# vFones/situation-recognition

Hardware: NVIDIA B200
Metric: ggnn_images_per_sec_fwd_bwd (higher is better)
Workload: dtype bf16

## Files before the change

include/srggnn.h:

```cpp
#ifndef SRGGNN_H_
#define SRGGNN_H_

#include <stddef.h>
#include <stdint.h>

#ifdef __cplusplus
extern "C" {
#endif

typedef struct srg_handle srg_handle;

enum { SRG_DT_F32 = 1, SRG_DT_BF16 = 2 };
enum { SRG_PREC_BF16 = 0, SRG_PREC_FP32 = 1 };
enum { SRG_MODE_NOUN = 0, SRG_MODE_VERB = 1 };

const char* srg_last_error(void);
int srg_version(void);

int srg_create(srg_handle** out, int device, int D, int R, int T, int n_verbs, int n_roles, int n_labels);
int srg_destroy(srg_handle* h);
int srg_set_cta_group(srg_handle* h, int cta_group);

int srg_set_compact_rows(srg_handle* h, int on);

int srg_set_tables(srg_handle* h, const int32_t* verb2roles, const int32_t* role_count);

int srg_gather_mask(srg_handle* h, const int64_t* verb, int B, int64_t* role_idx, float* mask, int* bad_verb,
                    void* stream);

int srg_check_verbs(srg_handle* h, void* stream);

typedef struct srg_params {
  const float *W_p, *b_p;
  const float *W_z, *b_Wz, *U_z, *b_Uz;
  const float *W_r, *b_Wr, *U_r, *b_Ur;
  const float *W_h, *b_Wh, *U_h, *b_Uh;
  const float *Wc_verb, *bc_verb;
  const float *Wc_noun, *bc_noun;
} srg_params;

typedef struct srg_grads {
  float *W_p, *b_p;
  float *W_z, *b_Wz, *U_z, *b_Uz;
  float *W_r, *b_Wr, *U_r, *b_Ur;
  float *W_h, *b_Wh, *U_h, *b_Uh;
  float *Wc_verb, *bc_verb;
  float *Wc_noun, *bc_noun;
  float *role_emb;
  float *verb_emb;
} srg_grads;

int srg_pack_weights(srg_handle* h, const srg_params* p, int precision, void* stream);

size_t srg_workspace_bytes(srg_handle* h, int mode, int B, int precision, int save_for_backward);

int srg_nouns_forward(srg_handle* h, const float* feat, const int64_t* verb, int B, const float* role_emb,
                      const float* verb_emb, const uint8_t* keep, float drop_p, const int64_t* drop_seed,
                      int64_t drop_stream, float* logits, int64_t ldl, int precision, int save_for_backward,
                      void* workspace, size_t workspace_bytes, void* stream);

int srg_verb_forward(srg_handle* h, const float* feat, int B, const uint8_t* keep, float drop_p,
                     const int64_t* drop_seed, int64_t drop_stream, float* logits, int64_t ldl, int precision,
                     int save_for_backward, void* workspace, size_t workspace_bytes, void* stream);

int srg_topk_logsoftmax(const float* logits, int64_t ldl, int rows, int n, int k, int64_t* idx, float* logp,
                        void* stream);

size_t srg_situation_workspace_bytes(srg_handle* h, int B, int k, int precision);
int srg_situation_nouns(srg_handle* h, const float* feat, const int64_t* verbs, int B, int k, const float* role_emb,
                        const float* verb_emb, const float* verb_logp, int64_t* labels, float* label_logp,
                        float* score, int precision, void* workspace, size_t workspace_bytes, void* stream);

int srg_dropout_mask(const int64_t* drop_seed, int64_t drop_stream, float drop_p, int64_t rows, int D, uint8_t* keep,
                     void* stream);

int srg_ggnn_forward(srg_handle* h, int mode, float* hidden, const float* mask, int B, int precision,
                     int save_for_backward, void* workspace, size_t workspace_bytes, void* stream);

int srg_ggnn_backward(srg_handle* h, int mode, const float* dhidden_out, const float* mask, float* dmask,
                      float* dhidden_in, int B, const srg_grads* g, void* workspace, size_t workspace_bytes,
                      void* stream);

int srg_count_targets(srg_handle* h, const int64_t* gt_nouns, int B, float* counts, void* stream);
int srg_nouns_loss(srg_handle* h, const float* logits, int64_t ldl, const int64_t* gt_nouns, int B,
                   const float* counts, float* loss, float* dlogits, float grad_scale, const float* stats,
                   void* stream);

int srg_verb_loss(srg_handle* h, const float* logits, int64_t ldl, const int64_t* gt_verb, int B, float inv_batch,
                  const float* batch_total, float* loss, float* dlogits, float grad_scale, const float* stats,
                  void* stream);

int srg_nouns_loss_backward(srg_handle* h, const float* logits, int64_t ldl, const int64_t* gt_nouns, int B,
                            const float* counts, const float* grad_out, float grad_scale, float* dlogits,
                            void* dlogits_bf16, int accumulate, const float* stats, void* stream);
int srg_verb_loss_backward(srg_handle* h, const float* logits, int64_t ldl, const int64_t* gt_verb, int B,
                           float inv_batch, const float* batch_total, const float* grad_out, float grad_scale,
                           float* dlogits, void* dlogits_bf16, int accumulate, const float* stats, void* stream);
size_t srg_workspace_dlogits_offset(srg_handle* h, int mode, int B, const void* workspace);

size_t srg_workspace_stats_offset(srg_handle* h, int mode, int B, int precision, int save_for_backward,
                                  const void* workspace);

int srg_nouns_backward(srg_handle* h, const float* dlogits, int64_t ldl, int dlogits_in_workspace, const float* feat,
                       const int64_t* verb, int B, const float* role_emb, const float* verb_emb, const uint8_t* keep,
                       float drop_p, const int64_t* drop_seed, int64_t drop_stream, const srg_grads* g, void* workspace,
                       size_t workspace_bytes, void* stream);
int srg_verb_backward(srg_handle* h, const float* dlogits, int64_t ldl, int dlogits_in_workspace, int B,
                      const uint8_t* keep, float drop_p, const int64_t* drop_seed, int64_t drop_stream,
                      const srg_grads* g, void* workspace, size_t workspace_bytes, void* stream);

int srg_nouns_backward_feat(srg_handle* h, const float* dlogits, int64_t ldl, int dlogits_in_workspace,
                            const float* feat, const int64_t* verb, int B, const float* role_emb, const float* verb_emb,
                            const uint8_t* keep, float drop_p, const int64_t* drop_seed, int64_t drop_stream,
                            const srg_grads* g, float* dfeat, void* workspace, size_t workspace_bytes, void* stream);
int srg_verb_backward_feat(srg_handle* h, const float* dlogits, int64_t ldl, int dlogits_in_workspace, int B,
                           const uint8_t* keep, float drop_p, const int64_t* drop_seed, int64_t drop_stream,
                           const srg_grads* g, float* dfeat, void* workspace, size_t workspace_bytes, void* stream);

int srg_set_deferred_chain(srg_handle* h, int on, void* stream);
int srg_chain_finalize(srg_handle* h, const srg_grads* g, void* stream);

int srg_clip_adamax(float* params, float* grads, float* exp_avg, float* exp_inf, int64_t n, float lr, float beta1,
                    float beta2, float eps, float max_norm, float* scratch, void* stream);

int srg_sumsq(const float* x, int64_t n, float* out, void* stream);
int srg_adamax_step(float* params, float* grads, float* exp_avg, float* exp_inf, int64_t n, float lr, float beta1,
                    float beta2, float eps, float max_norm, const float* norm_sq, float* step, void* stream);

int srg_gemm_bf16(const void* A, int64_t lda, int a_mn, const void* B, int64_t ldb, int b_mn, void* C, int64_t ldc,
                  int c_dtype, int M, int N, int K, const float* bias, float alpha, int cta_group, int k_splits,
                  int reduce, void* stream);

long long srg_launch_count(void);
int srg_profile_begin(void);
int srg_profile_end(int max_kinds, double* ms, double* flops, long long* launches);
const char* srg_profile_kind_name(int kind);

#ifdef __cplusplus
}
#endif
#endif
```

situation_recognition_b200/_lib.py:

```python
import ctypes
import os

_HERE = os.path.dirname(os.path.abspath(__file__))
LIB_PATH = os.environ.get("SRG_LIB_PATH") or os.path.join(_HERE, "libsrggnn.so")

SRG_DT_F32, SRG_DT_BF16 = 1, 2
SRG_PREC_BF16, SRG_PREC_FP32 = 0, 1
SRG_MODE_NOUN, SRG_MODE_VERB = 0, 1

_c = ctypes
_vp, _i, _i64, _f, _sz = _c.c_void_p, _c.c_int, _c.c_int64, _c.c_float, _c.c_size_t

_PARAM_FIELDS = ["W_p", "b_p", "W_z", "b_Wz", "U_z", "b_Uz", "W_r", "b_Wr", "U_r", "b_Ur", "W_h", "b_Wh", "U_h",
                 "b_Uh", "Wc_verb", "bc_verb", "Wc_noun", "bc_noun"]


class SrgParams(_c.Structure):
    _fields_ = [(n, _vp) for n in _PARAM_FIELDS]


class SrgGrads(_c.Structure):
    _fields_ = [(n, _vp) for n in _PARAM_FIELDS + ["role_emb", "verb_emb"]]


SIGNATURES = {
    "srg_last_error": (_c.c_char_p, []),
    "srg_version": (_i, []),
    "srg_create": (_i, [_c.POINTER(_vp), _i, _i, _i, _i, _i, _i, _i]),
    "srg_destroy": (_i, [_vp]),
    "srg_set_cta_group": (_i, [_vp, _i]),
    "srg_set_compact_rows": (_i, [_vp, _i]),
    "srg_set_tables": (_i, [_vp, _vp, _vp]),
    "srg_check_verbs": (_i, [_vp, _vp]),
    "srg_gather_mask": (_i, [_vp, _vp, _i, _vp, _vp, _vp, _vp]),
    "srg_pack_weights": (_i, [_vp, _c.POINTER(SrgParams), _i, _vp]),
    "srg_workspace_bytes": (_sz, [_vp, _i, _i, _i, _i]),
    "srg_nouns_forward": (_i, [_vp, _vp, _vp, _i, _vp, _vp, _vp, _f, _vp, _i64, _vp, _i64, _i, _i, _vp, _sz, _vp]),
    "srg_verb_forward": (_i, [_vp, _vp, _i, _vp, _f, _vp, _i64, _vp, _i64, _i, _i, _vp, _sz, _vp]),
    "srg_topk_logsoftmax": (_i, [_vp, _i64, _i, _i, _i, _vp, _vp, _vp]),
    "srg_situation_workspace_bytes": (_sz, [_vp, _i, _i, _i]),
    "srg_situation_nouns": (_i, [_vp, _vp, _vp, _i, _i, _vp, _vp, _vp, _vp, _vp, _vp, _i, _vp, _sz, _vp]),
    "srg_dropout_mask": (_i, [_vp, _i64, _f, _i64, _i, _vp, _vp]),
    "srg_ggnn_forward": (_i, [_vp, _i, _vp, _vp, _i, _i, _i, _vp, _sz, _vp]),
    "srg_count_targets": (_i, [_vp, _vp, _i, _vp, _vp]),
    "srg_nouns_loss": (_i, [_vp, _vp, _i64, _vp, _i, _vp, _vp, _vp, _f, _vp, _vp]),
    "srg_verb_loss": (_i, [_vp, _vp, _i64, _vp, _i, _f, _vp, _vp, _vp, _f, _vp, _vp]),
    "srg_nouns_loss_backward": (_i, [_vp, _vp, _i64, _vp, _i, _vp, _vp, _f, _vp, _vp, _i, _vp, _vp]),
    "srg_verb_loss_backward": (_i, [_vp, _vp, _i64, _vp, _i, _f, _vp, _vp, _f, _vp, _vp, _i, _vp, _vp]),
    "srg_workspace_stats_offset": (_sz, [_vp, _i, _i, _i, _i, _vp]),
    "srg_workspace_dlogits_offset": (_sz, [_vp, _i, _i, _vp]),
    "srg_nouns_backward": (_i, [_vp, _vp, _i64, _i, _vp, _vp, _i, _vp, _vp, _vp, _f, _vp, _i64, _c.POINTER(SrgGrads),
                                _vp, _sz, _vp]),
    "srg_verb_backward": (_i, [_vp, _vp, _i64, _i, _i, _vp, _f, _vp, _i64, _c.POINTER(SrgGrads), _vp, _sz, _vp]),
    "srg_nouns_backward_feat": (_i, [_vp, _vp, _i64, _i, _vp, _vp, _i, _vp, _vp, _vp, _f, _vp, _i64,
                                     _c.POINTER(SrgGrads), _vp, _vp, _sz, _vp]),
    "srg_verb_backward_feat": (_i, [_vp, _vp, _i64, _i, _i, _vp, _f, _vp, _i64, _c.POINTER(SrgGrads), _vp, _vp, _sz,
                                    _vp]),
    "srg_ggnn_backward": (_i, [_vp, _i, _vp, _vp, _vp, _vp, _i, _c.POINTER(SrgGrads), _vp, _sz, _vp]),
    "srg_set_deferred_chain": (_i, [_vp, _i, _vp]),
    "srg_chain_finalize": (_i, [_vp, _c.POINTER(SrgGrads), _vp]),
    "srg_clip_adamax": (_i, [_vp, _vp, _vp, _vp, _i64, _f, _f, _f, _f, _f, _vp, _vp]),
    "srg_sumsq": (_i, [_vp, _i64, _vp, _vp]),
    "srg_adamax_step": (_i, [_vp, _vp, _vp, _vp, _i64, _f, _f, _f, _f, _f, _vp, _vp, _vp]),
    "srg_launch_count": (_c.c_longlong, []),
    "srg_profile_begin": (_i, []),
    "srg_profile_end": (_i, [_i, _vp, _vp, _vp]),
    "srg_profile_kind_name": (_c.c_char_p, [_i]),
    "srg_gemm_bf16": (_i, [_vp, _i64, _i, _vp, _i64, _i, _vp, _i64, _i, _i, _i, _i, _vp, _f, _i, _i, _i, _vp]),
}

_lib = None


class SrgError(RuntimeError):
    pass


def load():
    global _lib
    if _lib is not None:
        return _lib
    if not os.path.exists(LIB_PATH):
        raise SrgError(
            f"{LIB_PATH} not found: build it with `python -c 'import __graft_entry__ as g; g.build()'` "
            "(there is no CPU/PyTorch fallback for the GGNN stage)")
    lib = ctypes.CDLL(LIB_PATH)
    for name, (res, args) in SIGNATURES.items():
        fn = getattr(lib, name)
        fn.restype = res
        fn.argtypes = args
    _lib = lib
    return lib


def check(rc):
    if rc != 0:
        msg = load().srg_last_error()
        raise SrgError(f"libsrggnn call failed (code {rc}): {msg.decode() if msg else '?'}")


def ptr(t):
    return None if t is None else ctypes.c_void_p(t.data_ptr())


def stream_ptr(device=None):
    import torch
    return ctypes.c_void_p(torch.cuda.current_stream(device).cuda_stream)
```

situation_recognition_b200/csrc/capi_ggnn.cu:

```cuda
#include <new>
#include <vector>
#include "elementwise.cuh"
#include "host.cuh"
#include "../../include/srggnn.h"

using namespace srg;

namespace srg {
int query_device(DeviceInfo* d);
}

namespace {
constexpr int kMaxT = 8;
inline int round_up(int x, int m) { return (x + m - 1) / m * m; }
}

struct srg_handle {
  int device = 0, D = 0, R = 0, T = 0, V = 0, n_roles = 0, L = 0;
  int Vpad = 0, Lpad = 0;
  int cg = 2;
  int compact = 1;
  DeviceInfo dev;
  int32_t* d_verb2roles = nullptr;
  int32_t* d_role_count = nullptr;
  bool tables_set = false;
  int* d_bad = nullptr;
  int packed_prec = -1;
  int alloc_split = 0;
  srg_params params;
  bf16 *Wzr = nullptr;
  bf16 *Wh = nullptr;
  bf16 *Wcn = nullptr, *Wcv = nullptr;
  bf16 *Wm_hi = nullptr, *Wm_mid = nullptr, *Wm_lo = nullptr;
  bf16 *Wp6 = nullptr;
  bf16 *P_hi = nullptr, *P_mid = nullptr, *P_lo = nullptr;
  bf16 *U_stack = nullptr, *Uh = nullptr;
  float *wb = nullptr;
  float *bzr[2] = {nullptr, nullptr};
  float *bh[2] = {nullptr, nullptr};
  float *bcn = nullptr, *bcv = nullptr;
  bool defer_chain = false;
  float* acc_GP = nullptr;
  bf16* acc_GPb = nullptr;
  float* acc_s = nullptr;
};

namespace {

struct StepBufs {
  bf16 *a_hi = nullptr, *a_mid = nullptr, *a_lo = nullptr, *rh_hi = nullptr, *rh_mid = nullptr, *rh_lo = nullptr;
  bf16 *r = nullptr, *hc = nullptr;
  void* z = nullptr;
};

struct PathBufs {
  int M = 0;
  int Mfull = 0;
  RowMap rm;
  float* h32 = nullptr;
  bf16* hb_hi[kMaxT + 1] = {};
  bf16* hb_mid[kMaxT + 1] = {};
  bf16* hb_lo[kMaxT + 1] = {};
  StepBufs st[kMaxT];
  bf16 *xd_hi = nullptr, *xd_mid = nullptr, *xd_lo = nullptr;
  float* stats = nullptr;
  float *dh = nullptr, *dh_acc = nullptr, *dx = nullptr;
  bf16* dpre_all = nullptr;
  bf16 *da = nullptr, *ada = nullptr, *e = nullptr, *dlb = nullptr;
  float* G_P = nullptr;
  bf16* G_Pb = nullptr;
  float* s_all = nullptr;
  size_t bytes = 0;
};

struct Bump {
  uint8_t* base;
  size_t off = 0;
  explicit Bump(void* b) : base(static_cast<uint8_t*>(b)) {
    if (base) off = (1024 - (reinterpret_cast<uintptr_t>(base) & 1023)) & 1023;
  }
  template <typename T>
  T* take(size_t n) {
    T* p = base ? reinterpret_cast<T*>(base + off) : nullptr;
    off += (n * sizeof(T) + 1023) & ~static_cast<size_t>(1023);
    return p;
  }
};

inline bool base_is_null(const void* ws) { return ws == nullptr; }

PathBufs carve(const srg_handle* h, int mode, int B, int prec, int save, void* ws, bool rowmap) {
  PathBufs pb;
  const int D = h->D, T = h->T;
  const int Mfull = (mode == SRG_MODE_NOUN) ? B * h->R : B;
  const int M = rowmap ? round_up(Mfull + 1, 256) : Mfull;
  const size_t MD = static_cast<size_t>(M) * D;
  const size_t MfD = static_cast<size_t>(Mfull) * D;
  const bool f32 = (prec == SRG_PREC_FP32);
  const int npad = (mode == SRG_MODE_NOUN) ? h->Lpad : h->Vpad;
  Bump bump(ws);
  pb.M = M;
  pb.Mfull = Mfull;
  if (rowmap) {
    pb.rm.cnt = bump.take<int>(B);
    pb.rm.off = bump.take<int>(static_cast<size_t>(B) + 1);
    pb.rm.meta = bump.take<int>(4);
    pb.rm.compact = h->compact;
  }
  pb.h32 = bump.take<float>(MD);
  const int n_hb = save ? T + 1 : 2;
  bf16* hb_all = bump.take<bf16>(static_cast<size_t>(n_hb) * MD);
  bf16* hb_mid_all = f32 ? bump.take<bf16>(static_cast<size_t>(n_hb) * MD) : nullptr;
  bf16* hb_lo_all = f32 ? bump.take<bf16>(static_cast<size_t>(n_hb) * MD) : nullptr;
  for (int t = 0; t <= T; ++t) {
    const size_t off = static_cast<size_t>(save ? t : (t & 1)) * MD;
    pb.hb_hi[t] = hb_all ? hb_all + off : nullptr;
    pb.hb_mid[t] = hb_mid_all ? hb_mid_all + off : nullptr;
    pb.hb_lo[t] = hb_lo_all ? hb_lo_all + off : nullptr;
  }
  const int n_st = save ? T : 1;
  const size_t n_all = static_cast<size_t>(n_st) * MD;
  bf16* a_all = (mode == SRG_MODE_NOUN) ? bump.take<bf16>(n_all) : nullptr;
  bf16* a_mid_all = (mode == SRG_MODE_NOUN && f32) ? bump.take<bf16>(n_all) : nullptr;
  bf16* a_lo_all = (mode == SRG_MODE_NOUN && f32) ? bump.take<bf16>(n_all) : nullptr;
  bf16* rh_all = bump.take<bf16>(n_all);
  bf16* rh_mid_all = f32 ? bump.take<bf16>(n_all) : nullptr;
  bf16* rh_lo_all = f32 ? bump.take<bf16>(n_all) : nullptr;
  uint8_t* z_all = f32 ? reinterpret_cast<uint8_t*>(bump.take<float>(n_all)) : reinterpret_cast<uint8_t*>(bump.take<bf16>(n_all));
  bf16* r_all = save ? bump.take<bf16>(n_all) : nullptr;
  bf16* hc_all = save ? bump.take<bf16>(n_all) : nullptr;
  for (int t = 0; t < T; ++t) {
    const size_t off = (save ? static_cast<size_t>(t) : 0) * MD;
    StepBufs& st = pb.st[t];
    st.a_hi = a_all ? a_all + off : nullptr;
    st.a_mid = a_mid_all ? a_mid_all + off : nullptr;
    st.a_lo = a_lo_all ? a_lo_all + off : nullptr;
    st.rh_hi = rh_all + off;
    st.rh_mid = rh_mid_all ? rh_mid_all + off : nullptr;
    st.rh_lo = rh_lo_all ? rh_lo_all + off : nullptr;
    st.z = (base_is_null(ws)) ? nullptr : static_cast<void*>(z_all + off * (f32 ? 4 : 2));
    st.r = r_all ? r_all + off : nullptr;
    st.hc = hc_all ? hc_all + off : nullptr;
  }
  pb.xd_hi = bump.take<bf16>(MfD);
  pb.xd_mid = f32 ? bump.take<bf16>(MfD) : nullptr;
  pb.xd_lo = f32 ? bump.take<bf16>(MfD) : nullptr;
  pb.stats = bump.take<float>(static_cast<size_t>(Mfull) * (npad / 128) * 2);
  if (save) {
    pb.dh = bump.take<float>(MD);
    pb.dh_acc = bump.take<float>(MD);
    pb.dx = bump.take<float>(MfD);
    pb.dpre_all = bump.take<bf16>(static_cast<size_t>(T) * 3 * MD);
    pb.da = bump.take<bf16>(MD);
    pb.ada = bump.take<bf16>(MD);
    pb.e = bump.take<bf16>(MD);
    pb.dlb = bump.take<bf16>(static_cast<size_t>(Mfull) * npad);
    pb.G_P = bump.take<float>(static_cast<size_t>(3) * D * D);
    pb.G_Pb = bump.take<bf16>(static_cast<size_t>(3) * D * D);
    pb.s_all = bump.take<float>(static_cast<size_t>(3) * D);
  }
  pb.bytes = bump.off + 1024;
  return pb;
}

int check_ws(const srg_handle* h, int mode, int B, int prec, int save, void* ws, size_t ws_bytes, PathBufs* out,
             bool rowmap) {
  SRG_CHECK(h != nullptr, "null handle");
  SRG_CHECK(B > 0, "batch must be positive (got %d)", B);
  SRG_CHECK(prec == SRG_PREC_BF16 || prec == SRG_PREC_FP32, "bad precision %d", prec);
  SRG_CHECK(!(save && prec != SRG_PREC_BF16), "save_for_backward requires SRG_PREC_BF16 (the fp32 mode is forward-only)");
  SRG_CHECK(ws != nullptr, "null workspace");
  SRG_CHECK((reinterpret_cast<uintptr_t>(ws) & 15) == 0, "workspace must be 16-byte aligned");
  *out = carve(h, mode, B, prec, save, ws, rowmap);
  const size_t need = carve(h, mode, B, prec, save, nullptr, rowmap).bytes;
  if (need > ws_bytes)
    return set_error(SRG_ERR_WORKSPACE, "workspace too small: need %zu bytes, got %zu", need, ws_bytes);
  return SRG_OK;
}

GemmProblem base_problem(const srg_handle* h, int M, int N) {
  GemmProblem p;
  p.cg = h->cg;
  p.M = M;
  p.N = N;
  return p;
}

GemmProblem path_problem(const srg_handle* h, const PathBufs& pb, int N) {
  GemmProblem p = base_problem(h, pb.M, N);
  p.m_dev = pb.rm.meta;
  return p;
}

void add_seg_ld(GemmProblem& p, const bf16* a, int64_t rows, int64_t cols, int64_t ld, int k_off, int k_len) {
  GemmSeg& s = p.seg[p.nseg++];
  s.a = mat(a, rows, cols, ld, DT_BF16);
  s.k_off = k_off;
  s.k_len = k_len;
}
void add_seg(GemmProblem& p, const bf16* a, int64_t rows, int64_t cols, int k_off, int k_len) {
  add_seg_ld(p, a, rows, cols, cols, k_off, k_len);
}

constexpr int kSplitTerms = 6;
constexpr int kPartA[kSplitTerms] = {0, 0, 1, 0, 2, 1};
constexpr int kPartB[kSplitTerms] = {0, 1, 0, 2, 0, 1};

struct Split3 {
  const bf16* part[3];
};

void add_split_segs(GemmProblem& p, int M, int D, bool f32, const Split3* x, int n) {
  const int terms = f32 ? kSplitTerms : 1;
  for (int b = 0; b < terms; ++b)
    for (int i = 0; i < n; ++i) add_seg(p, x[i].part[kPartA[b]], M, D, 0, D);
  if (f32) p.corr_seg_begin = n;
}

int wgrad_splits(const srg_handle* h, int out_rows, int out_cols, int K) {
  const int bn = (h->cg == 2) ? 256 : 128;
  const int tiles = ((out_rows + 128 * h->cg - 1) / (128 * h->cg)) * (out_cols / bn);
  const int clusters = h->dev.num_sms / h->cg;
  int s = (clusters * 7 + tiles - 1) / tiles;
  const int kb = (K + kBlockK - 1) / kBlockK;
  if (s > kb) s = kb;
  if (s > 64) s = 64;
  if (s < 1) s = 1;
  return s;
}

int wgrad(const srg_handle* h, const bf16* dY, int64_t dy_ld, int out_rows, const bf16* X, int in_cols, int nseg,
          int seg_rows, int64_t seg_stride, const int* k_dev, float* dW, cudaStream_t s) {
  if (dW == nullptr) return SRG_OK;
  const int64_t phys_rows = static_cast<int64_t>(nseg - 1) * seg_stride + seg_rows;
  GemmProblem p = base_problem(h, out_rows, in_cols);
  p.a_mn = true;
  p.b_mn = true;
  p.epi = EPI_STORE_F32;
  p.flags = FLAG_REDUCE;
  if (nseg > 1 && seg_stride == seg_rows && k_dev == nullptr) {
    nseg = 1;
    seg_rows = static_cast<int>(phys_rows);
  }
  SRG_CHECK(nseg >= 1 && nseg <= kMaxSeg, "wgrad: bad segment count %d", nseg);
  p.nseg = nseg;
  for (int t = 0; t < nseg; ++t) {
    p.seg[t].a = mat(dY, phys_rows, out_rows, dy_ld, DT_BF16);
    p.seg[t].k_off = static_cast<int>(t * seg_stride);
    p.seg[t].k_len = seg_rows;
  }
  if (nseg > 1 || k_dev != nullptr) p.flags |= FLAG_BK_A;
  p.k_dev = k_dev;
  p.b = mat(X, phys_rows, in_cols, in_cols, DT_BF16);
  p.io[0] = mat(dW, out_rows, in_cols, in_cols, DT_F32);
  const int64_t k_expect = static_cast<int64_t>(nseg) * seg_rows * ((k_dev != nullptr && h->compact) ? 3 : 5) / 5;
  p.k_splits = wgrad_splits(h, out_rows, in_cols, static_cast<int>(k_expect));
  return run_gemm(p, h->dev, s);
}

int ggnn_steps(srg_handle* h, int mode, PathBufs& pb, float* h32, const float* mask, int B, int prec, int save,
               cudaStream_t s) {
  const int D = h->D, T = h->T, M = pb.M;
  const bool f32 = (prec == SRG_PREC_FP32);
  const int kmul = f32 ? kSplitTerms : 1;
  const int mi = (mode == SRG_MODE_NOUN) ? 0 : 1;
  for (int t = 0; t < T; ++t) {
    StepBufs& st = pb.st[t];
    const Split3 hcur = {{pb.hb_hi[t], pb.hb_mid[t], pb.hb_lo[t]}};
    Split3 a = hcur;
    if (mode == SRG_MODE_NOUN) {
      if (pb.rm.meta != nullptr) SRG_TRY(launch_aggregate_rows(h32, pb.rm, B, h->R, D, st.a_hi, st.a_mid, st.a_lo, s));
      else SRG_TRY(launch_aggregate(h32, mask, B, h->R, D, st.a_hi, st.a_mid, st.a_lo, s));
      a = Split3{{st.a_hi, st.a_mid, st.a_lo}};
    }
    const Split3 rh = {{st.rh_hi, st.rh_mid, st.rh_lo}};
    {
      GemmProblem p = path_problem(h, pb, 2 * D);
      const Split3 ops[2] = {a, hcur};
      add_split_segs(p, M, D, f32, ops, 2);
      p.b = mat(h->Wzr, 2 * D, static_cast<int64_t>(2 * D) * kmul, static_cast<int64_t>(2 * D) * kmul, DT_BF16);
      p.epi = EPI_ZR;
      p.f32 = f32;
      p.bias = h->bzr[mi];
      p.n_split = D;
      p.flags = (f32 ? FLAG_LO : 0) | (save ? FLAG_STASH : 0);
      p.io[0] = mat(st.z, M, D, D, f32 ? DT_F32 : DT_BF16);
      p.io[1] = mat(h32, M, D, D, DT_F32);
      p.io[2] = mat(st.rh_hi, M, D, D, DT_BF16);
      if (f32) {
        p.io[3] = mat(st.rh_mid, M, D, D, DT_BF16);
        p.io[5] = mat(st.rh_lo, M, D, D, DT_BF16);
      }
      if (save) p.io[4] = mat(st.r, M, D, D, DT_BF16);
      SRG_TRY(run_gemm(p, h->dev, s));
    }
    {
      GemmProblem p = path_problem(h, pb, D);
      const Split3 ops[2] = {a, rh};
      add_split_segs(p, M, D, f32, ops, 2);
      p.b = mat(h->Wh, D, static_cast<int64_t>(2 * D) * kmul, static_cast<int64_t>(2 * D) * kmul, DT_BF16);
      p.epi = EPI_H;
      p.f32 = f32;
      p.bias = h->bh[mi];
      p.flags = save ? FLAG_STASH : 0;
      p.io[0] = mat(h32, M, D, D, DT_F32);
      p.io[1] = mat(st.z, M, D, D, f32 ? DT_F32 : DT_BF16);
      p.io[2] = mat(pb.hb_hi[t + 1], M, D, D, DT_BF16);
      if (f32) {
        p.io[3] = mat(pb.hb_mid[t + 1], M, D, D, DT_BF16);
        p.io[5] = mat(pb.hb_lo[t + 1], M, D, D, DT_BF16);
      }
      if (save) p.io[4] = mat(st.hc, M, D, D, DT_BF16);
      SRG_TRY(run_gemm(p, h->dev, s));
    }
  }
  return SRG_OK;
}

int make_drop(const uint8_t* keep, float drop_p, const int64_t* seed, int64_t stream_id, DropSpec* ds) {
  SRG_CHECK(drop_p >= 0.f && drop_p < 1.f, "dropout probability %f out of range", drop_p);
  *ds = DropSpec();
  if (drop_p > 0.f && (keep != nullptr || seed != nullptr)) {
    ds->keep = keep;
    ds->seed = (keep == nullptr) ? reinterpret_cast<const long long*>(seed) : nullptr;
    ds->stream = stream_id;
    ds->thresh = static_cast<uint32_t>((1.0 - static_cast<double>(drop_p)) * 65536.0 + 0.5);
    ds->scale = 1.0f / (1.0f - drop_p);
  }
  return SRG_OK;
}

int classifier_forward(srg_handle* h, int mode, PathBufs& pb, const float* h32, const DropSpec& ds, float* logits,
                       int64_t ldl, int prec, cudaStream_t s) {
  const int D = h->D, M = pb.Mfull;
  const bool f32 = (prec == SRG_PREC_FP32);
  const int kmul = f32 ? kSplitTerms : 1;
  const int ncls = (mode == SRG_MODE_NOUN) ? h->L : h->V;
  const int npad = (mode == SRG_MODE_NOUN) ? h->Lpad : h->Vpad;
  SRG_CHECK(ldl >= ncls && (ldl % 4) == 0, "logits leading dimension %lld must be >= %d and a multiple of 4",
            (long long)ldl, ncls);
  Split3 x = {{pb.hb_hi[h->T], pb.hb_mid[h->T], pb.hb_lo[h->T]}};
  const bool use_drop = (ds.keep != nullptr || ds.seed != nullptr);
  if (use_drop || pb.rm.meta != nullptr) {
    SRG_TRY(launch_classifier_input(h32, pb.rm, h->R, M, D, ds, pb.xd_hi, pb.xd_mid, pb.xd_lo, s));
    x = Split3{{pb.xd_hi, pb.xd_mid, pb.xd_lo}};
  }
  GemmProblem p = base_problem(h, M, npad);
  add_split_segs(p, M, D, f32, &x, 1);
  const bf16* W = (mode == SRG_MODE_NOUN) ? h->Wcn : h->Wcv;
  p.b = mat(W, npad, static_cast<int64_t>(D) * kmul, static_cast<int64_t>(D) * kmul, DT_BF16);
  p.epi = EPI_LOGITS;
  p.f32 = f32;
  p.bias = (mode == SRG_MODE_NOUN) ? h->bcn : h->bcv;
  p.n_valid = ncls;
  p.stats = pb.stats;
  p.io[0] = mat(logits, M, ldl < npad ? ldl : npad, ldl, DT_F32);
  return run_gemm(p, h->dev, s);
}

int chain_rule(srg_handle* h, const float* G_P, bf16* G_Pb, const float* s_all, const srg_grads* g, bool shared_dst,
               cudaStream_t s) {
  const int D = h->D;
  SRG_TRY(launch_split_cast(G_P, static_cast<int64_t>(3) * D * D, G_Pb, nullptr, nullptr, s));
  float* gW[3] = {g->W_h, g->W_z, g->W_r};
  const float* W32[3] = {h->params.W_h, h->params.W_z, h->params.W_r};
  for (int x3 = 0; x3 < 3; ++x3) {
    if (gW[x3] == nullptr) continue;
    GemmProblem p = base_problem(h, D, D);
    add_seg(p, G_Pb + static_cast<size_t>(x3) * D * D, D, D, 0, D);
    p.b = mat(h->Wp6, D, D, D, DT_BF16);
    p.epi = EPI_STORE_F32;
    p.flags = FLAG_REDUCE;
    p.io[0] = mat(gW[x3], D, D, D, DT_F32);
    SRG_TRY(run_gemm(p, h->dev, s));
  }
  SRG_TRY(launch_outer_acc3(s_all, h->params.b_p, D, D, gW, shared_dst, s));
  if (g->b_p != nullptr) SRG_TRY(launch_matvec_t_acc3(W32, s_all, D, D, g->b_p, s));
  if (g->W_p != nullptr) {
    GemmProblem p = base_problem(h, D, D);
    p.a_mn = true;
    p.b_mn = true;
    p.nseg = 1;
    p.seg[0].a = mat(h->Wm_hi, 3 * D, D, D, DT_BF16);
    p.seg[0].k_off = 0;
    p.seg[0].k_len = 3 * D;
    p.b = mat(G_Pb, 3 * D, D, D, DT_BF16);
    p.epi = EPI_STORE_F32;
    p.flags = FLAG_REDUCE;
    p.io[0] = mat(g->W_p, D, D, D, DT_F32);
    p.k_splits = wgrad_splits(h, D, D, 3 * D);
    SRG_TRY(run_gemm(p, h->dev, s));
  }
  return SRG_OK;
}

int chain_acc(srg_handle* h, PathBufs& pb, float** G_P, float** s_all, cudaStream_t s) {
  const int D = h->D;
  *G_P = h->defer_chain ? h->acc_GP : pb.G_P;
  *s_all = h->defer_chain ? h->acc_s : pb.s_all;
  if (!h->defer_chain) {
    SRG_CUDA(cudaMemsetAsync(*G_P, 0, sizeof(float) * 3 * D * D, s));
    SRG_CUDA(cudaMemsetAsync(*s_all, 0, sizeof(float) * 3 * D, s));
  }
  return SRG_OK;
}

int ggnn_backward(srg_handle* h, int mode, PathBufs& pb, int B, const float* dh_T, const float* mask, float* dmask,
                  float* G_P, float* s_all, const srg_grads* g, cudaStream_t s) {
  const int D = h->D, T = h->T, M = pb.M, R = h->R;
  const int64_t ld3 = 3 * static_cast<int64_t>(D);
  const float cmul = (mode == SRG_MODE_NOUN) ? static_cast<float>(R) : 1.f;
  const bool mapped = (pb.rm.meta != nullptr);
  const int* m_dev = mapped ? pb.rm.meta : nullptr;

  float* dh_acc = pb.dh_acc;
  auto dpre_of = [&](int t) { return pb.dpre_all + static_cast<size_t>(t) * M * ld3; };
  if (dh_T != nullptr)
    SRG_TRY(launch_gru_bwd_pre_ld(dh_T, static_cast<const bf16*>(pb.st[T - 1].z), pb.st[T - 1].hc, pb.hb_hi[T - 1], M,
                                  nullptr, nullptr, D, dpre_of(T - 1) + D, dpre_of(T - 1), ld3, dh_acc, s));
  for (int t = T - 1; t >= 0; --t) {
    StepBufs& st = pb.st[t];
    bf16* dp = dpre_of(t);
    bf16* dpre_r = dp + 2 * D;
    {
      GemmProblem p = path_problem(h, pb, D);
      add_seg_ld(p, dp, M, ld3, ld3, 0, D);
      p.b_mn = true;
      p.b = mat(h->Uh, D, D, D, DT_BF16);
      p.epi = EPI_DRH;
      p.io[0] = mat(pb.hb_hi[t], M, D, D, DT_BF16);
      p.io[1] = mat(st.r, M, D, D, DT_BF16);
      p.io[2] = mat(dpre_r, M, D, ld3, DT_BF16);
      p.io[3] = mat(pb.e, M, D, D, DT_BF16);
      SRG_TRY(run_gemm(p, h->dev, s));
    }
    {
      GemmProblem p = path_problem(h, pb, D);
      add_seg_ld(p, dp, M, ld3, ld3, 0, 3 * D);
      p.b_mn = true;
      p.b = mat(h->P_hi, 3 * D, D, D, DT_BF16);
      p.epi = EPI_STORE_BF16;
      p.io[0] = mat(pb.da, M, D, D, DT_BF16);
      SRG_TRY(run_gemm(p, h->dev, s));
    }
    if (mask != nullptr) SRG_TRY(launch_aggregate_t(pb.da, pb.e, mask, pb.hb_hi[t], B, R, D, pb.ada, dmask, s));
    else SRG_TRY(launch_aggregate_t_rows(pb.da, pb.e, pb.rm, mapped ? B : M, R, D, pb.ada, s));
    const bf16* ada = pb.ada;
    {
      GemmProblem p = path_problem(h, pb, D);
      add_seg_ld(p, dp, M, ld3, ld3, D, 2 * D);
      p.b_mn = true;
      p.b = mat(h->U_stack, 2 * D, D, D, DT_BF16);
      p.epi = EPI_DH;
      p.flags = FLAG_ADD;
      p.io[0] = mat(dh_acc, M, D, D, DT_F32);
      p.io[6] = mat(ada, M, D, D, DT_BF16);
      if (t > 0) {
        bf16* dn = dpre_of(t - 1);
        p.flags |= FLAG_NEXT;
        p.io[1] = mat(pb.st[t - 1].z, M, D, D, DT_BF16);
        p.io[2] = mat(pb.st[t - 1].hc, M, D, D, DT_BF16);
        p.io[3] = mat(pb.hb_hi[t - 1], M, D, D, DT_BF16);
        p.io[4] = mat(dn + D, M, D, ld3, DT_BF16);
        p.io[5] = mat(dn, M, D, ld3, DT_BF16);
      }
      SRG_TRY(run_gemm(p, h->dev, s));
    }
  }
  {
    bf16* dp = pb.dpre_all;
    const bf16* a_all = (mode == SRG_MODE_NOUN) ? pb.st[0].a_hi : pb.hb_hi[0];
    SRG_TRY(wgrad(h, dp, ld3, 3 * D, a_all, D, T, M, M, m_dev, G_P, s));
    SRG_TRY(wgrad(h, dp + D, ld3, D, pb.hb_hi[0], D, T, M, M, m_dev, g->U_z, s));
    SRG_TRY(wgrad(h, dp + 2 * D, ld3, D, pb.hb_hi[0], D, T, M, M, m_dev, g->U_r, s));
    SRG_TRY(wgrad(h, dp, ld3, D, pb.st[0].rh_hi, D, T, M, M, m_dev, g->U_h, s));
    ColsumJob jobs[3] = {{dp, g->b_Wh, g->b_Uh, 1.f, s_all, cmul},
                         {dp + D, g->b_Wz, g->b_Uz, 1.f, s_all + D, cmul},
                         {dp + 2 * D, g->b_Wr, g->b_Ur, 1.f, s_all + 2 * D, cmul}};
    if (mapped) SRG_TRY(launch_colsum_multi(jobs, 3, ld3, M, m_dev, T, M, D, s));
    else SRG_TRY(launch_colsum_multi(jobs, 3, ld3, T * M, nullptr, 1, 0, D, s));
  }
  pb.dh = dh_acc;

  if (h->defer_chain) return SRG_OK;
  return chain_rule(h, G_P, pb.G_Pb, s_all, g, true, s);
}

int path_backward(srg_handle* h, int mode, PathBufs& pb, const float* dlogits, int64_t ldl, int dlb_ready, int B,
                  const DropSpec& ds, const srg_grads* g, cudaStream_t s) {
  const int D = h->D, T = h->T, Mf = pb.Mfull, R = h->R;
  const int ncls = (mode == SRG_MODE_NOUN) ? h->L : h->V;
  const int npad = (mode == SRG_MODE_NOUN) ? h->Lpad : h->Vpad;
  const bf16* Wc = (mode == SRG_MODE_NOUN) ? h->Wcn : h->Wcv;
  float* gWc = (mode == SRG_MODE_NOUN) ? g->Wc_noun : g->Wc_verb;
  float* gbc = (mode == SRG_MODE_NOUN) ? g->bc_noun : g->bc_verb;
  const int64_t ld3 = 3 * static_cast<int64_t>(D);
  const bool use_drop = (ds.keep != nullptr || ds.seed != nullptr);
  const bool mapped = (pb.rm.meta != nullptr);
  const bool gathered = use_drop || mapped;
  const bf16* x = gathered ? pb.xd_hi : pb.hb_hi[T];
  const int* rows_dev = mapped ? pb.rm.meta + 2 : nullptr;

  float *G_P = nullptr, *s_all = nullptr;
  SRG_TRY(chain_acc(h, pb, &G_P, &s_all, s));

  SRG_CHECK(dlogits != nullptr || dlb_ready, "backward: no gradient of the logits was given");
  if (dlogits != nullptr) SRG_TRY(launch_cast_pad(dlogits, ldl, Mf, ncls, npad, pb.dlb, dlb_ready ? 1 : 0, s));
  SRG_TRY(launch_colsum(pb.dlb, npad, Mf, ncls, gbc, 1.f, nullptr, 0.f, s));
  SRG_TRY(wgrad(h, pb.dlb, npad, ncls, x, D, 1, Mf, Mf, nullptr, gWc, s));
  {
    GemmProblem p = base_problem(h, Mf, D);
    add_seg(p, pb.dlb, Mf, npad, 0, npad);
    p.b_mn = true;
    p.b = mat(Wc, npad, D, D, DT_BF16);
    p.epi = EPI_STORE_F32;
    p.io[0] = mat(gathered ? pb.dx : pb.dh, Mf, D, D, DT_F32);
    SRG_TRY(run_gemm(p, h->dev, s));
  }
  if (gathered) {
    bf16* dp = pb.dpre_all + static_cast<size_t>(T - 1) * pb.M * ld3;
    GruPre gp;
    gp.z = static_cast<const bf16*>(pb.st[T - 1].z);
    gp.hc = pb.st[T - 1].hc;
    gp.h = pb.hb_hi[T - 1];
    gp.dpre_z = dp + D;
    gp.dpre_h = dp;
    gp.ld_out = ld3;
    gp.dh_acc = pb.dh_acc;
    SRG_TRY(launch_classifier_input_bwd(pb.dx, pb.rm, (mode == SRG_MODE_NOUN) ? B : Mf, (mode == SRG_MODE_NOUN) ? R : 1,
                                        D, ds, pb.dh, gp, s));
    if (mapped)
      SRG_TRY(launch_gru_bwd_pre_ld(pb.dh, gp.z, gp.hc, gp.h, 256, rows_dev, pb.rm.meta + 1, D, gp.dpre_z, gp.dpre_h,
                                    ld3, pb.dh_acc, s));
  }
  return ggnn_backward(h, mode, pb, B, gathered ? nullptr : pb.dh, nullptr, nullptr, G_P, s_all, g, s);
}

int ensure_pack_buffers(srg_handle* h, int split) {
  const size_t D = h->D;
  auto re = [&](bf16** p, size_t n) -> int {
    if (*p) cudaFree(*p);
    *p = nullptr;
    SRG_CUDA(cudaMalloc(reinterpret_cast<void**>(p), n * sizeof(bf16)));
    return SRG_OK;
  };
  auto f32buf = [&](float** p, size_t n) -> int {
    SRG_CUDA(cudaMalloc(reinterpret_cast<void**>(p), n * sizeof(float)));
    return SRG_OK;
  };
  if (!h->Wm_hi) {
    SRG_TRY(re(&h->Wm_hi, 3 * D * D));
    SRG_TRY(re(&h->Wm_mid, 3 * D * D));
    SRG_TRY(re(&h->Wm_lo, 3 * D * D));
    SRG_TRY(re(&h->Wp6, 6 * D * D));
    SRG_TRY(re(&h->P_hi, 3 * D * D));
    SRG_TRY(re(&h->P_mid, 3 * D * D));
    SRG_TRY(re(&h->P_lo, 3 * D * D));
    SRG_TRY(re(&h->U_stack, 2 * D * D));
    SRG_TRY(re(&h->Uh, D * D));
    SRG_TRY(f32buf(&h->wb, 3 * D));
    for (int i = 0; i < 2; ++i) {
      SRG_TRY(f32buf(&h->bzr[i], 2 * D));
      SRG_TRY(f32buf(&h->bh[i], D));
    }
    SRG_TRY(f32buf(&h->bcn, h->Lpad));
    SRG_TRY(f32buf(&h->bcv, h->Vpad));
  }
  if (h->alloc_split >= split) return SRG_OK;
  SRG_TRY(re(&h->Wzr, 2 * D * 2 * D * split));
  SRG_TRY(re(&h->Wh, D * 2 * D * split));
  SRG_TRY(re(&h->Wcn, static_cast<size_t>(h->Lpad) * D * split));
  SRG_TRY(re(&h->Wcv, static_cast<size_t>(h->Vpad) * D * split));
  h->alloc_split = split;
  return SRG_OK;
}

int copy_block(bf16* dst, int64_t ld, int64_t row_off, int64_t col_off, const bf16* src, int D, cudaStream_t s) {
  SRG_CUDA(cudaMemcpy2DAsync(dst + row_off * ld + col_off, ld * sizeof(bf16), src, D * sizeof(bf16), D * sizeof(bf16), D,
                             cudaMemcpyDeviceToDevice, s));
  return SRG_OK;
}

}

extern "C" {

int srg_version(void) { return 100; }

int srg_create(srg_handle** out, int device, int D, int R, int T, int n_verbs, int n_roles, int n_labels) {
  SRG_CHECK(out != nullptr, "srg_create: null output pointer");
  SRG_CHECK(D > 0 && D % 256 == 0, "hidden size D=%d must be a positive multiple of 256", D);
  SRG_CHECK(R >= 1 && R <= 8, "max role count R=%d must be in [1, 8]", R);
  SRG_CHECK(T >= 1 && T <= kMaxT, "propagation steps T=%d must be in [1, %d]", T, kMaxT);
  SRG_CHECK(n_verbs > 0 && n_roles > 0 && n_labels > 0, "vocabulary sizes must be positive");
  SRG_CUDA(cudaSetDevice(device));
  srg_handle* h = new (std::nothrow) srg_handle();
  SRG_CHECK(h != nullptr, "out of host memory");
  h->device = device;
  h->D = D; h->R = R; h->T = T; h->V = n_verbs; h->n_roles = n_roles; h->L = n_labels;
  h->Vpad = round_up(n_verbs, 256);
  h->Lpad = round_up(n_labels, 256);
  int rc = query_device(&h->dev);
  if (rc != SRG_OK) { delete h; return rc; }
  cudaError_t e = cudaMalloc(reinterpret_cast<void**>(&h->d_verb2roles), sizeof(int32_t) * n_verbs * R);
  if (e == cudaSuccess) e = cudaMalloc(reinterpret_cast<void**>(&h->d_role_count), sizeof(int32_t) * n_verbs);
  if (e == cudaSuccess) e = cudaMalloc(reinterpret_cast<void**>(&h->d_bad), sizeof(int));
  if (e == cudaSuccess) e = cudaMemset(h->d_bad, 0, sizeof(int));
  if (e != cudaSuccess) {
    delete h;
    return set_error(SRG_ERR_CUDA, "srg_create: cudaMalloc failed: %s", cudaGetErrorString(e));
  }
  *out = h;
  return SRG_OK;
}

int srg_destroy(srg_handle* h) {
  if (!h) return SRG_OK;
  DeviceGuard guard_(h->device);
  void* ptrs[] = {h->d_verb2roles, h->d_role_count, h->d_bad, h->Wzr, h->Wh, h->Wcn, h->Wcv, h->Wm_hi, h->Wm_mid, h->Wm_lo, h->Wp6,
                  h->P_hi, h->P_mid, h->P_lo, h->U_stack, h->Uh, h->wb, h->bzr[0], h->bzr[1], h->bh[0], h->bh[1], h->bcn, h->bcv,
                  h->acc_GP, h->acc_GPb, h->acc_s};
  for (void* p : ptrs)
    if (p) cudaFree(p);
  delete h;
  return SRG_OK;
}

int srg_set_cta_group(srg_handle* h, int cta_group) {
  SRG_CHECK(h != nullptr, "null handle");
  SRG_CHECK(cta_group == 1 || cta_group == 2, "cta_group must be 1 or 2");
  h->cg = cta_group;
  return SRG_OK;
}

int srg_set_compact_rows(srg_handle* h, int on) {
  SRG_CHECK(h != nullptr, "null handle");
  h->compact = (on != 0);
  return SRG_OK;
}

int srg_set_tables(srg_handle* h, const int32_t* verb2roles, const int32_t* role_count) {
  SRG_CHECK(h != nullptr, "srg_set_tables: null handle");
  DeviceGuard guard_(h->device);
  SRG_CHECK(h && verb2roles && role_count, "srg_set_tables: null argument");
  for (int v = 0; v < h->V; ++v) {
    SRG_CHECK(role_count[v] >= 0 && role_count[v] <= h->R, "role_count[%d]=%d outside [0,%d]", v, role_count[v], h->R);
    for (int r = 0; r < h->R; ++r) {
      const int id = verb2roles[v * h->R + r];
      SRG_CHECK(id >= 0 && id <= h->n_roles, "verb2roles[%d,%d]=%d outside [0,%d]", v, r, id, h->n_roles);
    }
  }
  SRG_CUDA(cudaMemcpy(h->d_verb2roles, verb2roles, sizeof(int32_t) * h->V * h->R, cudaMemcpyHostToDevice));
  SRG_CUDA(cudaMemcpy(h->d_role_count, role_count, sizeof(int32_t) * h->V, cudaMemcpyHostToDevice));
  h->tables_set = true;
  return SRG_OK;
}

int srg_gather_mask(srg_handle* h, const int64_t* verb, int B, int64_t* role_idx, float* mask, int* bad_verb,
                    void* stream) {
  SRG_CHECK(h != nullptr, "srg_gather_mask: null handle");
  DeviceGuard guard_(h->device);
  SRG_CHECK(h != nullptr && h->tables_set, "srg_gather_mask: call srg_set_tables first");
  SRG_CHECK(B >= 0, "negative batch");
  if (B == 0) return SRG_OK;
  SRG_CHECK(verb != nullptr, "null verb pointer");
  return launch_gather_mask(h->d_verb2roles, h->d_role_count, h->V, h->R, verb, B, role_idx, mask, bad_verb,
                            static_cast<cudaStream_t>(stream));
}

int srg_check_verbs(srg_handle* h, void* stream) {
  SRG_CHECK(h != nullptr, "srg_check_verbs: null handle");
  DeviceGuard guard_(h->device);
  cudaStream_t s = static_cast<cudaStream_t>(stream);
  int bad = 0;
  SRG_CUDA(cudaMemcpyAsync(&bad, h->d_bad, sizeof(int), cudaMemcpyDeviceToHost, s));
  SRG_CUDA(cudaMemsetAsync(h->d_bad, 0, sizeof(int), s));
  SRG_CUDA(cudaStreamSynchronize(s));
  if (bad) return set_error(SRG_ERR_ARG, "a verb id outside [0, %d) was passed to srg_nouns_forward (it was computed as verb 0)", h->V);
  return SRG_OK;
}

int srg_pack_weights(srg_handle* h, const srg_params* p, int precision, void* stream) {
  SRG_CHECK(h != nullptr, "srg_pack_weights: null handle");
  DeviceGuard guard_(h->device);
  SRG_CHECK(h && p, "srg_pack_weights: null argument");
  SRG_CHECK(precision == SRG_PREC_BF16 || precision == SRG_PREC_FP32, "bad precision %d", precision);
  cudaStream_t s = static_cast<cudaStream_t>(stream);
  const int D = h->D;
  const int split = (precision == SRG_PREC_FP32) ? kSplitTerms : 1;
  SRG_TRY(ensure_pack_buffers(h, split));
  h->params = *p;
  const size_t DD = static_cast<size_t>(D) * D;

  std::vector<PackJob> jobs;
  auto queue = [&](const float* src, int rows, int rows_pad, bf16* dst, int64_t ld, int64_t col_off, int part) {
    PackJob j;
    j.src = src; j.dst = dst; j.ld_dst = ld; j.col_off = col_off; j.rows = rows; j.rows_pad = rows_pad; j.part = part;
    jobs.push_back(j);
  };
  const bool f32 = (precision == SRG_PREC_FP32);

  const float* Wm32[3] = {p->W_h, p->W_z, p->W_r};
  bf16* Wm_part[3] = {h->Wm_hi, h->Wm_mid, h->Wm_lo};
  const int p_terms = f32 ? kSplitTerms : 1;
  for (int x = 0; x < 3; ++x)
    for (int part = 0; part < (f32 ? 3 : 1); ++part) queue(Wm32[x], D, D, Wm_part[part] + x * DD, D, 0, part);
  for (int b = 0; b < p_terms; ++b) queue(p->W_p, D, D, h->Wp6 + b * DD, D, 0, kPartB[b]);
  SRG_TRY(launch_pack_weight_multi(jobs.data(), static_cast<int>(jobs.size()), D, s));
  jobs.clear();

  {
    GemmProblem g = base_problem(h, 3 * D, D);
    for (int b = 0; b < p_terms; ++b) add_seg(g, Wm_part[kPartA[b]], 3 * D, D, 0, D);
    if (f32) g.corr_seg_begin = 1;
    g.b_mn = true;
    g.b = mat(h->Wp6, static_cast<int64_t>(p_terms) * D, D, D, DT_BF16);
    g.epi = EPI_STORE_BF16;
    g.f32 = f32;
    g.flags = f32 ? FLAG_LO : 0;
    g.io[0] = mat(h->P_hi, 3 * D, D, D, DT_BF16);
    if (f32) {
      g.io[1] = mat(h->P_mid, 3 * D, D, D, DT_BF16);
      g.io[2] = mat(h->P_lo, 3 * D, D, D, DT_BF16);
    }
    SRG_TRY(run_gemm(g, h->dev, s));
  }

  const int64_t ld1 = static_cast<int64_t>(D) * split, ld2 = static_cast<int64_t>(2 * D) * split;
  const bf16* P_part[3] = {h->P_hi, h->P_mid, h->P_lo};
  auto pack_u = [&](const float* src, int rows, int rows_pad, bf16* dst, int64_t ld, int64_t row_off, int block_cols,
                    int col_in_block) {
    bf16* d = dst + row_off * ld;
    for (int b = 0; b < split; ++b)
      queue(src, rows, rows_pad, d, ld, static_cast<int64_t>(b) * block_cols + col_in_block, kPartB[b]);
  };
  auto pack_p = [&](int x, bf16* dst, int64_t row_off) -> int {
    for (int b = 0; b < split; ++b)
      SRG_TRY(copy_block(dst, ld2, row_off, static_cast<int64_t>(b) * 2 * D, P_part[kPartB[b]] + x * DD, D, s));
    return SRG_OK;
  };
  SRG_TRY(pack_p(1, h->Wzr, 0));
  pack_u(p->U_z, D, D, h->Wzr, ld2, 0, 2 * D, D);
  SRG_TRY(pack_p(2, h->Wzr, D));
  pack_u(p->U_r, D, D, h->Wzr, ld2, D, 2 * D, D);
  SRG_TRY(pack_p(0, h->Wh, 0));
  pack_u(p->U_h, D, D, h->Wh, ld2, 0, 2 * D, D);
  pack_u(p->Wc_noun, h->L, h->Lpad, h->Wcn, ld1, 0, D, 0);
  pack_u(p->Wc_verb, h->V, h->Vpad, h->Wcv, ld1, 0, D, 0);
  if (!f32) {
    queue(p->U_z, D, D, h->U_stack, D, 0, 0);
    queue(p->U_r, D, D, h->U_stack + DD, D, 0, 0);
    queue(p->U_h, D, D, h->Uh, D, 0, 0);
  }
  SRG_TRY(launch_pack_weight_multi(jobs.data(), static_cast<int>(jobs.size()), D, s));

  for (int x = 0; x < 3; ++x) SRG_TRY(launch_matvec(Wm32[x], p->b_p, D, D, h->wb + x * D, s));
  for (int mi = 0; mi < 2; ++mi) {
    const float c = (mi == 0) ? static_cast<float>(h->R) : 1.f;
    SRG_TRY(launch_pack_bias3(p->b_Wz, p->b_Uz, h->wb + D, c, D, D, h->bzr[mi], s));
    SRG_TRY(launch_pack_bias3(p->b_Wr, p->b_Ur, h->wb + 2 * D, c, D, D, h->bzr[mi] + D, s));
    SRG_TRY(launch_pack_bias3(p->b_Wh, p->b_Uh, h->wb, c, D, D, h->bh[mi], s));
  }
  SRG_TRY(launch_pack_bias(p->bc_noun, nullptr, h->L, h->Lpad, h->bcn, s));
  SRG_TRY(launch_pack_bias(p->bc_verb, nullptr, h->V, h->Vpad, h->bcv, s));
  h->packed_prec = precision;
  return SRG_OK;
}

size_t srg_workspace_stats_offset(srg_handle* h, int mode, int B, int precision, int save_for_backward,
                                  const void* workspace) {
  if (!h || B <= 0 || !workspace) return 0;
  PathBufs pb = carve(h, mode, B, precision, save_for_backward, const_cast<void*>(workspace), mode == SRG_MODE_NOUN);
  return static_cast<size_t>(reinterpret_cast<const uint8_t*>(pb.stats) - static_cast<const uint8_t*>(workspace));
}

size_t srg_workspace_dlogits_offset(srg_handle* h, int mode, int B, const void* workspace) {
  if (!h || B <= 0 || !workspace) return 0;
  PathBufs pb = carve(h, mode, B, SRG_PREC_BF16, 1, const_cast<void*>(workspace), mode == SRG_MODE_NOUN);
  return static_cast<size_t>(reinterpret_cast<const uint8_t*>(pb.dlb) - static_cast<const uint8_t*>(workspace));
}

size_t srg_workspace_bytes(srg_handle* h, int mode, int B, int precision, int save_for_backward) {
  if (!h || B <= 0) return 0;
  return carve(h, mode, B, precision, save_for_backward, nullptr, mode == SRG_MODE_NOUN).bytes;
}

}

namespace {
int nouns_forward_body(srg_handle* h, PathBufs& pb, const float* feat, int feat_rep, const int64_t* verb, int B,
                       const float* role_emb, const float* verb_emb, const DropSpec& ds, float* logits, int64_t ldl,
                       int precision, int save_for_backward, cudaStream_t s) {
  SRG_TRY(launch_prep_rows(h->d_role_count, h->V, h->R, verb, B, h->compact, pb.rm, h->d_bad, s));
  SRG_TRY(launch_node_init_noun(feat, role_emb, verb_emb, verb, h->d_verb2roles, h->V, B, h->R, h->D, pb.rm, feat_rep,
                                pb.h32, pb.hb_hi[0], pb.hb_mid[0], pb.hb_lo[0], s));
  SRG_TRY(ggnn_steps(h, SRG_MODE_NOUN, pb, pb.h32, nullptr, B, precision, save_for_backward, s));
  return classifier_forward(h, SRG_MODE_NOUN, pb, pb.h32, ds, logits, ldl, precision, s);
}

size_t situation_layout(const srg_handle* h, int B, int k, int prec, void* ws, PathBufs* pb, float** logits) {
  const int n = B * k;
  const size_t logit_bytes = static_cast<size_t>(n) * h->R * h->Lpad * sizeof(float);
  if (ws != nullptr) {
    const PathBufs p = carve(h, SRG_MODE_NOUN, n, prec, 0, ws, true);
    if (pb) *pb = p;
    if (logits) *logits = reinterpret_cast<float*>(static_cast<uint8_t*>(ws) + p.bytes - 1024);
  }
  return carve(h, SRG_MODE_NOUN, n, prec, 0, nullptr, true).bytes + logit_bytes;
}
}

extern "C" {

int srg_nouns_forward(srg_handle* h, const float* feat, const int64_t* verb, int B, const float* role_emb,
                      const float* verb_emb, const uint8_t* keep, float drop_p, const int64_t* drop_seed,
                      int64_t drop_stream, float* logits, int64_t ldl, int precision, int save_for_backward,
                      void* workspace, size_t workspace_bytes, void* stream) {
  SRG_CHECK(h != nullptr, "srg_nouns_forward: null handle");
  DeviceGuard guard_(h->device);
  PathBufs pb;
  SRG_TRY(check_ws(h, SRG_MODE_NOUN, B, precision, save_for_backward, workspace, workspace_bytes, &pb, true));
  SRG_CHECK(h->tables_set, "srg_nouns_forward: call srg_set_tables first");
  SRG_CHECK(h->packed_prec == precision, "srg_nouns_forward: weights are not packed for precision %d", precision);
  SRG_CHECK(feat && verb && role_emb && verb_emb && logits, "srg_nouns_forward: null argument");
  DropSpec ds;
  SRG_TRY(make_drop(keep, drop_p, drop_seed, drop_stream, &ds));
  return nouns_forward_body(h, pb, feat, 1, verb, B, role_emb, verb_emb, ds, logits, ldl, precision, save_for_backward,
                            static_cast<cudaStream_t>(stream));
}

int srg_topk_logsoftmax(const float* logits, int64_t ldl, int rows, int n, int k, int64_t* idx, float* logp,
                        void* stream) {
  SRG_CHECK(rows >= 0, "srg_topk_logsoftmax: negative row count %d", rows);
  SRG_CHECK(rows == 0 || (logits && idx && logp), "srg_topk_logsoftmax: null argument");
  return launch_row_topk_logsoftmax(logits, ldl, rows, n, k, idx, logp, static_cast<cudaStream_t>(stream));
}

size_t srg_situation_workspace_bytes(srg_handle* h, int B, int k, int precision) {
  if (!h || B <= 0 || k < 1 || k > 16) return 0;
  return situation_layout(h, B, k, precision, nullptr, nullptr, nullptr);
}

int srg_situation_nouns(srg_handle* h, const float* feat, const int64_t* verbs, int B, int k, const float* role_emb,
                        const float* verb_emb, const float* verb_logp, int64_t* labels, float* label_logp,
                        float* score, int precision, void* workspace, size_t workspace_bytes, void* stream) {
  SRG_CHECK(h != nullptr, "srg_situation_nouns: null handle");
  DeviceGuard guard_(h->device);
  SRG_CHECK(k >= 1 && k <= 16 && k <= h->V, "srg_situation_nouns: k=%d must be in [1, min(16, n_verbs=%d)]", k, h->V);
  SRG_CHECK(B > 0 && static_cast<int64_t>(B) * k * h->R <= (1 << 30), "srg_situation_nouns: bad batch %d", B);
  PathBufs pb;
  SRG_TRY(check_ws(h, SRG_MODE_NOUN, B * k, precision, 0, workspace, workspace_bytes, &pb, true));
  float* nl = nullptr;
  const size_t need = situation_layout(h, B, k, precision, workspace, &pb, &nl);
  if (need > workspace_bytes)
    return set_error(SRG_ERR_WORKSPACE, "workspace too small: need %zu bytes, got %zu", need, workspace_bytes);
  SRG_CHECK(h->tables_set, "srg_situation_nouns: call srg_set_tables first");
  SRG_CHECK(h->packed_prec == precision, "srg_situation_nouns: weights are not packed for precision %d", precision);
  SRG_CHECK(feat && verbs && role_emb && verb_emb && labels && label_logp && score, "srg_situation_nouns: null argument");
  cudaStream_t s = static_cast<cudaStream_t>(stream);
  const int n = B * k;
  SRG_TRY(nouns_forward_body(h, pb, feat, k, verbs, n, role_emb, verb_emb, DropSpec(), nl, h->Lpad, precision, 0, s));
  SRG_TRY(launch_row_topk_logsoftmax(nl, h->Lpad, n * h->R, h->L, 1, labels, label_logp, s));
  return launch_situation_finish(verbs, h->d_role_count, h->V, h->R, n, verb_logp, labels, label_logp, score, s);
}

int srg_verb_forward(srg_handle* h, const float* feat, int B, const uint8_t* keep, float drop_p,
                     const int64_t* drop_seed, int64_t drop_stream, float* logits, int64_t ldl, int precision,
// ... 239 lines not shown
```

situation_recognition_b200/csrc/elementwise.cuh:

```cuda
#pragma once
#include <cstdint>
#include <cuda_runtime.h>
#include <cuda_bf16.h>

namespace srg {

typedef __nv_bfloat16 bf16;

struct RowMap {
  const int* cnt = nullptr;
  const int* off = nullptr;
  const int* meta = nullptr;
  int compact = 0;
};

struct DropSpec {
  const uint8_t* keep = nullptr;
  const long long* seed = nullptr;
  long long stream = 0;
  uint32_t thresh = 65536;
  float scale = 1.f;
};

int launch_gather_mask(const int32_t* verb2roles, const int32_t* role_count, int n_verbs, int R, const int64_t* verb,
                       int B, int64_t* role_idx, float* mask, int* bad, cudaStream_t s);

int launch_prep_rows(const int32_t* role_count, int n_verbs, int R, const int64_t* verb, int B, int compact, RowMap rm,
                     int* bad, cudaStream_t s);
int launch_node_init_noun(const float* feat, const float* role_emb, const float* verb_emb, const int64_t* verb,
                          const int32_t* verb2roles, int n_verbs, int B, int R, int D, RowMap rm, int feat_rep,
                          float* h32, bf16* hb_hi, bf16* hb_mid, bf16* hb_lo, cudaStream_t s);
int launch_aggregate_rows(const float* h32, RowMap rm, int B, int R, int D, bf16* a_hi, bf16* a_mid, bf16* a_lo,
                          cudaStream_t s);
int launch_aggregate_t_rows(const bf16* da, const bf16* e, RowMap rm, int B, int R, int D, bf16* ada, cudaStream_t s);
int launch_aggregate_t(const bf16* da, const bf16* e, const float* mask, const bf16* h, int B, int R, int D,
                       bf16* ada, float* dmask, cudaStream_t s);
int launch_classifier_input(const float* h32, RowMap rm, int R, int64_t rows, int D, DropSpec ds, bf16* x_hi,
                            bf16* x_mid, bf16* x_lo, cudaStream_t s);
struct GruPre {
  const bf16* z = nullptr;
  const bf16* hc = nullptr;
  const bf16* h = nullptr;
  bf16* dpre_z = nullptr;
  bf16* dpre_h = nullptr;
  int64_t ld_out = 0;
  float* dh_acc = nullptr;
};
int launch_classifier_input_bwd(const float* dx, RowMap rm, int B, int R, int D, DropSpec ds, float* dh, GruPre gp,
                                cudaStream_t s);
int launch_dropout_mask(DropSpec ds, int64_t rows, int D, uint8_t* out, cudaStream_t s);
int launch_node_init_verb(const float* feat, int B, int D, float* h32, bf16* hb_hi, bf16* hb_mid, bf16* hb_lo,
                          cudaStream_t s);
int launch_split_cast(const float* x, int64_t n, bf16* hi, bf16* mid, bf16* lo, cudaStream_t s);

int launch_aggregate(const float* h32, const float* mask, int B, int R, int D, bf16* a_hi, bf16* a_mid, bf16* a_lo,
                     cudaStream_t s);

struct PackJob {
  const float* src;
  bf16* dst;
  int64_t ld_dst;
  int64_t col_off;
  int rows, rows_pad, part;
};
constexpr int kMaxPackJobs = 48;
int launch_pack_weight_multi(const PackJob* jobs, int n_jobs, int cols, cudaStream_t s);
int launch_pack_bias(const float* a, const float* b, int n, int n_pad, float* dst, cudaStream_t s);

int launch_count_targets(const int64_t* gt, int B, int R, int ignore_index, float* counts, cudaStream_t s);
int launch_nouns_ce(const float* logits, int64_t ldl, int n_labels, const int64_t* gt, int B, int R,
                    const float* counts, float* loss, float* dlogits, float grad_scale, const float* gscale_dev,
                    const float* stats, int stats_tiles, bf16* dlb, int n_pad, int accumulate, cudaStream_t s);
int launch_verb_ce(const float* logits, int64_t ldl, int n_verbs, const int64_t* gt, int B, float inv_batch,
                   float* loss, float* dlogits, float grad_scale, const float* gscale_dev, const float* stats,
                   int stats_tiles, const float* batch_total, bf16* dlb, int n_pad, int accumulate, cudaStream_t s);
int launch_row_topk_logsoftmax(const float* x, int64_t ldl, int rows, int n, int k, int64_t* idx, float* logp,
                               cudaStream_t s);
int launch_situation_finish(const int64_t* verb, const int32_t* role_count, int n_verbs, int R, int n_cand,
                            const float* verb_logp, int64_t* labels, float* label_logp, float* score, cudaStream_t s);
int launch_cast_pad(const float* src, int64_t ld, int rows, int n_valid, int n_pad, bf16* dst, int accumulate,
                    cudaStream_t s);

int launch_colsum(const bf16* X, int64_t ld, int rows, int n_cols, float* out1, float scale1, float* out2,
                  float scale2, cudaStream_t s);
int launch_node_init_bwd(const float* dh0, const bf16* h0b, const float* feat, const float* role_emb,
                         const float* verb_emb, const int64_t* verb, const int32_t* verb2roles, int n_verbs,
                         int n_roles, int B, int R, int D, RowMap rm, float* d_role_emb, float* d_verb_emb,
                         float* dfeat, cudaStream_t s);
int launch_node_init_verb_bwd(const float* dh0, const bf16* h0b, int B, int D, float* dfeat, cudaStream_t s);

struct ColsumJob {
  const bf16* X;
  float* out1;
  float* out2;
  float scale;
  float* out3;
  float scale3;
};
int launch_colsum_multi(const ColsumJob* jobs, int n_jobs, int64_t ld, int rows, const int* rows_dev, int nseg,
                        int64_t seg_stride, int n_cols, cudaStream_t s);


int launch_sumsq(const float* x, int64_t n, float* out, cudaStream_t s);
int launch_adamax_step(float* params, float* grads, float* exp_avg, float* exp_inf, int64_t n, float lr, float beta1,
                       float beta2, float eps, float max_norm, const float* norm_sq, float* step, cudaStream_t s);
int launch_clip_adamax(float* params, float* grads, float* exp_avg, float* exp_inf, int64_t n, float lr, float beta1,
                       float beta2, float eps, float max_norm, float* norm_sq, float* step, cudaStream_t s);

int launch_gru_bwd_pre_ld(const float* dh, const bf16* z, const bf16* hc, const bf16* h, int rows, const int* rows_dev,
                          const int* row0_dev, int D, bf16* dpre_z, bf16* dpre_h, int64_t ld_out, float* dh_acc,
                          cudaStream_t s);
int launch_matvec(const float* W, const float* x, int rows, int cols, float* y, cudaStream_t s);
int launch_matvec_t_acc3(const float* const W[3], const float* sv, int rows, int cols, float* y, cudaStream_t s);
int launch_outer_acc3(const float* sv, const float* b, int rows, int cols, float* const dW[3], bool atomic,
                      cudaStream_t s);
int launch_pack_bias3(const float* a, const float* b, const float* c, float scale, int n, int n_pad, float* dst,
                      cudaStream_t s);

}
```

situation_recognition_b200/csrc/epilogue_pipe.cuh:

```cuda
#pragma once

namespace srg {

__device__ __forceinline__ uint32_t u64_addr(uint32_t base, int r, int c) {
  return base + r * 64 + ((c ^ ((r >> 1) & 3)) << 4);
}
__device__ __forceinline__ void u64_ld_bf16x8(uint32_t base, int lane, int c, float (&v)[8]) {
  uint32_t u[4];
  lds128(u64_addr(base, lane, c), u[0], u[1], u[2], u[3]);
#pragma unroll
  for (int i = 0; i < 4; ++i) {
    v[2 * i] = bf16_lo_f(u[i]);
    v[2 * i + 1] = bf16_hi_f(u[i]);
  }
}
__device__ __forceinline__ void u64_st_bf16x8(uint32_t base, int lane, int c, const float (&v)[8]) {
  sts128(u64_addr(base, lane, c), pack_bf16(v[0], v[1]), pack_bf16(v[2], v[3]), pack_bf16(v[4], v[5]),
         pack_bf16(v[6], v[7]));
}

constexpr int kF32Box = 16384;
constexpr int kB16Box = 8192;
constexpr int kF32Warp = 4096;
constexpr int kB16Warp = 2048;

template <int EPI>
struct PipeTraits {
  static constexpr int kSetBytes = (EPI == EPI_ZR)   ? kF32Box + 2 * kB16Box
                                   : (EPI == EPI_H)  ? kF32Box + 2 * kB16Box
                                   : (EPI == EPI_DH) ? kF32Box + 4 * kB16Box
                                                     : 2 * kB16Box;
};
constexpr int kRegB0 = kF32Box;
constexpr int kRegB1 = kF32Box + kB16Box;
constexpr int kRegB2 = kF32Box + 2 * kB16Box;
constexpr int kRegB3 = kF32Box + 3 * kB16Box;

struct PipeCtx {
  const GemmMaps* maps;
  const GemmArgs* args;
  int lane;
  int ew;
};

template <int EPI>
__device__ __forceinline__ void pipe_issue(const PipeCtx& c, uint8_t* sp, uint64_t* bar, int n0, int cc, int row0) {
  const GemmMaps& m = *c.maps;
  const GemmArgs& a = *c.args;
  const int gcol = n0 + cc * 32;
  if constexpr (EPI == EPI_ZR) {
    ptx::mbar_arrive_expect_tx(bar, kF32Box);
    ptx::tma_load_2d(&m.io[1], bar, sp, gcol - a.n_split, row0);
  } else if constexpr (EPI == EPI_H) {
    ptx::mbar_arrive_expect_tx(bar, kF32Box + kB16Box);
    ptx::tma_load_2d(&m.io[0], bar, sp, gcol, row0);
    ptx::tma_load_2d(&m.io[1], bar, sp + kRegB0, gcol, row0);
  } else if constexpr (EPI == EPI_DH) {
    const bool next = (a.flags & FLAG_NEXT) != 0, has_add = (a.flags & FLAG_ADD) != 0;
    ptx::mbar_arrive_expect_tx(bar, kF32Box + (next ? 3 : 0) * kB16Box + (has_add ? kB16Box : 0));
    ptx::tma_load_2d(&m.io[0], bar, sp, gcol, row0);
    if (next) {
      ptx::tma_load_2d(&m.io[1], bar, sp + kRegB0, gcol, row0);
      ptx::tma_load_2d(&m.io[2], bar, sp + kRegB1, gcol, row0);
      ptx::tma_load_2d(&m.io[3], bar, sp + kRegB2, gcol, row0);
    }
    if (has_add) ptx::tma_load_2d(&m.io[6], bar, sp + kRegB3, gcol, row0);
  } else {
    ptx::mbar_arrive_expect_tx(bar, 2 * kB16Box);
    ptx::tma_load_2d(&m.io[0], bar, sp, gcol, row0);
    ptx::tma_load_2d(&m.io[1], bar, sp + kB16Box, gcol, row0);
  }
}

template <int EPI>
__device__ __forceinline__ void pipe_compute(const PipeCtx& c, uint32_t s, const float (&acc)[32],
                                             const float (&breg)[8], int cc, bool r_tile) {
  const GemmArgs& a = *c.args;
  const int lane = c.lane;
  const uint32_t sf = s + c.ew * kF32Warp;
  auto sb = [&](int region_off) -> uint32_t { return s + region_off + c.ew * kB16Warp; };
  if constexpr (EPI == EPI_ZR) {
    float b[4][8];
#pragma unroll
    for (int g = 0; g < 4; ++g)
#pragma unroll
      for (int i = 0; i < 8; ++i) b[g][i] = __shfl_sync(0xffffffffu, breg[i], cc * 4 + g);
    if (!r_tile) {
#pragma unroll
      for (int g = 0; g < 4; ++g) {
        float z[8];
#pragma unroll
        for (int i = 0; i < 8; ++i) z[i] = act_sigmoid<false>(acc[g * 8 + i] + b[g][i]);
        u64_st_bf16x8(s + c.ew * kB16Warp, lane, g, z);
      }
    } else {
      float h[4][8];
#pragma unroll
      for (int g = 0; g < 4; ++g) slot_ld_f32x8(sf, lane, g, h[g]);
#pragma unroll
      for (int g = 0; g < 4; ++g) {
        float r[8], rh[8];
#pragma unroll
        for (int i = 0; i < 8; ++i) {
          r[i] = act_sigmoid<false>(acc[g * 8 + i] + b[g][i]);
          rh[i] = r[i] * h[g][i];
        }
        u64_st_bf16x8(sb(kRegB0), lane, g, rh);
        if (a.flags & FLAG_STASH) u64_st_bf16x8(sb(kRegB1), lane, g, r);
      }
    }
  } else if constexpr (EPI == EPI_H) {
    float h[4][8], z[4][8];
#pragma unroll
    for (int g = 0; g < 4; ++g) {
      slot_ld_f32x8(sf, lane, g, h[g]);
      u64_ld_bf16x8(sb(kRegB0), lane, g, z[g]);
    }
#pragma unroll
    for (int g = 0; g < 4; ++g) {
      float hc[8], hn[8];
#pragma unroll
      for (int i = 0; i < 8; ++i) {
        const float bi = __shfl_sync(0xffffffffu, breg[i], cc * 4 + g);
        hc[i] = act_tanh<false>(acc[g * 8 + i] + bi);
        hn[i] = fmaf(z[g][i], hc[i] - h[g][i], h[g][i]);
      }
      slot_st_f32x8(sf, lane, g, hn);
      u64_st_bf16x8(sb(kRegB1), lane, g, hn);
      if (a.flags & FLAG_STASH) u64_st_bf16x8(sb(kRegB0), lane, g, hc);
    }
  } else if constexpr (EPI == EPI_DH) {
    const bool next = (a.flags & FLAG_NEXT) != 0, has_add = (a.flags & FLAG_ADD) != 0;
#pragma unroll
    for (int g0 = 0; g0 < 4; g0 += 2) {
      float dh[2][8], ad[2][8], z[2][8], hc[2][8], h[2][8];
#pragma unroll
      for (int j = 0; j < 2; ++j) {
        slot_ld_f32x8(sf, lane, g0 + j, dh[j]);
        if (has_add) u64_ld_bf16x8(sb(kRegB3), lane, g0 + j, ad[j]);
        if (next) {
          u64_ld_bf16x8(sb(kRegB0), lane, g0 + j, z[j]);
          u64_ld_bf16x8(sb(kRegB1), lane, g0 + j, hc[j]);
          u64_ld_bf16x8(sb(kRegB2), lane, g0 + j, h[j]);
        }
      }
#pragma unroll
      for (int j = 0; j < 2; ++j) {
        const int g = g0 + j;
#pragma unroll
        for (int i = 0; i < 8; ++i) dh[j][i] += acc[g * 8 + i];
        if (has_add) {
#pragma unroll
          for (int i = 0; i < 8; ++i) dh[j][i] += ad[j][i];
        }
        if (next) {
          float dz[8], dc[8];
#pragma unroll
          for (int i = 0; i < 8; ++i) {
            dz[i] = dh[j][i] * (hc[j][i] - h[j][i]) * z[j][i] * (1.0f - z[j][i]);
            dc[i] = dh[j][i] * z[j][i] * (1.0f - hc[j][i] * hc[j][i]);
            dh[j][i] = dh[j][i] * (1.0f - z[j][i]);
          }
          u64_st_bf16x8(sb(kRegB0), lane, g, dz);
          u64_st_bf16x8(sb(kRegB1), lane, g, dc);
        }
        slot_st_f32x8(sf, lane, g, dh[j]);
      }
    }
  } else {
    const uint32_t s0 = s + c.ew * kB16Warp, s1 = s + kB16Box + c.ew * kB16Warp;
    float h[4][8], r[4][8];
#pragma unroll
    for (int g = 0; g < 4; ++g) {
      u64_ld_bf16x8(s0, lane, g, h[g]);
      u64_ld_bf16x8(s1, lane, g, r[g]);
    }
#pragma unroll
    for (int g = 0; g < 4; ++g) {
      float e[8], dp[8];
#pragma unroll
      for (int i = 0; i < 8; ++i) {
        const float d = acc[g * 8 + i];
        dp[i] = d * h[g][i] * r[g][i] * (1.0f - r[g][i]);
        e[i] = d * r[g][i];
      }
      u64_st_bf16x8(s0, lane, g, dp);
      u64_st_bf16x8(s1, lane, g, e);
    }
  }
}

template <int EPI>
__device__ __forceinline__ void pipe_store(const PipeCtx& c, uint8_t* sp, int n0, int cc, int row0, bool r_tile) {
  const GemmMaps& m = *c.maps;
  const GemmArgs& a = *c.args;
  const int gcol = n0 + cc * 32;
  if constexpr (EPI == EPI_ZR) {
    if (!r_tile) {
      ptx::tma_store_2d(&m.io[0], sp, gcol, row0);
    } else {
      ptx::tma_store_2d(&m.io[2], sp + kRegB0, gcol - a.n_split, row0);
      if (a.flags & FLAG_STASH) ptx::tma_store_2d(&m.io[4], sp + kRegB1, gcol - a.n_split, row0);
    }
  } else if constexpr (EPI == EPI_H) {
    ptx::tma_store_2d(&m.io[0], sp, gcol, row0);
    ptx::tma_store_2d(&m.io[2], sp + kRegB1, gcol, row0);
    if (a.flags & FLAG_STASH) ptx::tma_store_2d(&m.io[4], sp + kRegB0, gcol, row0);
  } else if constexpr (EPI == EPI_DH) {
    ptx::tma_store_2d(&m.io[0], sp, gcol, row0);
    if (a.flags & FLAG_NEXT) {
      ptx::tma_store_2d(&m.io[4], sp + kRegB0, gcol, row0);
      ptx::tma_store_2d(&m.io[5], sp + kRegB1, gcol, row0);
    }
  } else {
    ptx::tma_store_2d(&m.io[2], sp, gcol, row0);
    ptx::tma_store_2d(&m.io[3], sp + kB16Box, gcol, row0);
  }
}

}
```

situation_recognition_b200/csrc/gemm.cuh:

```cuda
#pragma once
#include "ptx.cuh"

namespace srg {

constexpr int kBlockK = 64;
constexpr int kUmmaK = 16;
constexpr int kTileM = 128;
constexpr int kNumThreads = 256;
constexpr int kEpiWarp0 = 4;
constexpr int kSlotBytes = 4096;
constexpr int kMaxSeg = 12;
constexpr int kMaxAMaps = 6;
constexpr int kMaxIoMaps = 7;

enum EpiKind : int {
  EPI_STORE_BF16 = 0,
  EPI_STORE_F32 = 1,
  EPI_ZR = 2,
  EPI_H = 3,
  EPI_LOGITS = 4,
  EPI_DRH = 5,
  EPI_DH = 6,
};

enum : int { FLAG_LO = 1, FLAG_STASH = 2, FLAG_REDUCE = 4, FLAG_NEXT = 8, FLAG_ADD = 16, FLAG_BK_A = 32 };

struct GemmMaps {
  CUtensorMap a[kMaxAMaps];
  CUtensorMap b;
  CUtensorMap io[kMaxIoMaps];
};

struct GemmArgs {
  int M, N;
  const int* m_dev;
  const int* k_dev;
  int nseg;
  int seg_map[kMaxSeg];
  int seg_acol[kMaxSeg];
  int seg_kb[kMaxSeg];
  int total_kb;
  int corr_kb_begin;
  int k_splits;
  float alpha;
  const float* bias;
  float bias_scale;
  int n_split;
  int n_valid;
  float* stats;
  int flags;
  unsigned long long b_hint;
#ifdef SRG_EPI_TIMING
  unsigned long long* epi_t;
#endif
};

template <int EPI, bool F32>
struct EpiTraits {
  static constexpr int kSlots = (EPI == EPI_STORE_BF16) ? (F32 ? 6 : 2)
                                : (EPI == EPI_STORE_F32) ? 4
                                : (EPI == EPI_ZR)        ? (F32 ? 6 : 4)
                                : (EPI == EPI_H)         ? (F32 ? 7 : 4)
                                : (EPI == EPI_LOGITS)    ? 4
                                : (EPI == EPI_DH)        ? 6
                                                         : 2;
  static constexpr bool kPipe = !F32 && (EPI == EPI_ZR || EPI == EPI_H || EPI == EPI_DH || EPI == EPI_DRH);
};

template <int CG, int BLOCK_N, int EPI, bool F32>
struct GemmCfg {
  static constexpr int kABytes = kTileM * kBlockK * 2;
  static constexpr int kBBytes = (BLOCK_N / CG) * kBlockK * 2;
  static constexpr int kStageBytes = kABytes + kBBytes;
  static constexpr int kEpiBytes = 4 * EpiTraits<EPI, F32>::kSlots * kSlotBytes;
  static constexpr int kBarBytes = 1024;
  static constexpr int kSmemBudget = 232448 - 1024;
  static constexpr int kStagesRaw = (kSmemBudget - kEpiBytes - kBarBytes) / kStageBytes;
  static constexpr int kStages = kStagesRaw > 8 ? 8 : kStagesRaw;
  static constexpr int kSmemBytes = kStages * kStageBytes + kEpiBytes + kBarBytes + 1024;
  static constexpr int kTmemCols = 2 * BLOCK_N;
  static_assert(kStages >= 3, "not enough shared memory for the main loop");
  static_assert(kTmemCols <= 512, "accumulators do not fit TMEM");
};

template <bool F32>
__device__ __forceinline__ float act_sigmoid(float x) {
  if constexpr (F32) {
    return 1.0f / (1.0f + expf(-x));
  } else {
    float t;
    asm("tanh.approx.f32 %0, %1;" : "=f"(t) : "f"(0.5f * x));
    return fmaf(0.5f, t, 0.5f);
  }
}
template <bool F32>
__device__ __forceinline__ float act_tanh(float x) {
  if constexpr (F32) {
    return tanhf(x);
  } else {
    float y;
    asm("tanh.approx.f32 %0, %1;" : "=f"(y) : "f"(x));
    return y;
  }
}

__device__ __forceinline__ uint32_t pack_bf16(float a, float b) {
  __nv_bfloat162 v = __floats2bfloat162_rn(a, b);
  return *reinterpret_cast<uint32_t*>(&v);
}
__device__ __forceinline__ float bf16_lo_f(uint32_t p) { return __uint_as_float(p << 16); }
__device__ __forceinline__ float bf16_hi_f(uint32_t p) { return __uint_as_float(p & 0xFFFF0000u); }

__device__ __forceinline__ uint32_t slot_addr(uint32_t slot_base, int r, int c) {
  return slot_base + r * 128 + ((c ^ (r & 7)) << 4);
}
__device__ __forceinline__ void sts128(uint32_t addr, uint32_t a, uint32_t b, uint32_t c, uint32_t d) {
  asm volatile("st.shared.v4.b32 [%0], {%1, %2, %3, %4};" ::"r"(addr), "r"(a), "r"(b), "r"(c), "r"(d) : "memory");
}
__device__ __forceinline__ void lds128(uint32_t addr, uint32_t& a, uint32_t& b, uint32_t& c, uint32_t& d) {
  asm volatile("ld.shared.v4.b32 {%0, %1, %2, %3}, [%4];" : "=r"(a), "=r"(b), "=r"(c), "=r"(d) : "r"(addr) : "memory");
}

__device__ __forceinline__ void slot_ld_f32x8(uint32_t slot, int lane, int g, float (&v)[8]) {
  uint32_t* u = reinterpret_cast<uint32_t*>(v);
  lds128(slot_addr(slot, lane, 2 * g), u[0], u[1], u[2], u[3]);
  lds128(slot_addr(slot, lane, 2 * g + 1), u[4], u[5], u[6], u[7]);
}
__device__ __forceinline__ void slot_st_f32x8(uint32_t slot, int lane, int g, const float (&v)[8]) {
  const uint32_t* u = reinterpret_cast<const uint32_t*>(v);
  sts128(slot_addr(slot, lane, 2 * g), u[0], u[1], u[2], u[3]);
  sts128(slot_addr(slot, lane, 2 * g + 1), u[4], u[5], u[6], u[7]);
}
// ... 215 lines not shown
        ptx::tcgen05_fence_after();
        const uint32_t tmem_main = tmem_base + acc * BLOCK_N;
        for (int kb = kb_begin; kb < kb_end; ++kb) {
          const bool corr = F32 && kb >= args.corr_kb_begin;
          const uint32_t tmem_d = corr ? tmem_base + BLOCK_N : tmem_main;
          const int first_kb = corr ? args.corr_kb_begin : kb_begin;
          ptx::mbar_wait(&full_bar[stage], phase);
          ptx::tcgen05_fence_after();
          const uint32_t sa = ptx::smem_u32(smem_a + stage * A_BYTES);
          const uint32_t sb = ptx::smem_u32(smem_b + stage * B_BYTES);
#pragma unroll
          for (int k = 0; k < kBlockK / kUmmaK; ++k) {
            const uint64_t da = ptx::make_smem_desc(sa + k * A_KSTEP, A_LBO, 1024);
            const uint64_t db = ptx::make_smem_desc(sb + k * B_KSTEP, B_LBO, 1024);
            ptx::umma_bf16<CG>(tmem_d, da, db, idesc, (kb > first_kb || k > 0) ? 1u : 0u);
          }
          ptx::umma_commit<CG>(&empty_bar[stage]);
          if (kb == kb_end - 1) ptx::umma_commit<CG>(&tmem_full_bar[acc]);
          if (++stage == STAGES) { stage = 0; phase ^= 1u; }
        }
      }
    }
    __syncwarp();
  } else if (warp >= kEpiWarp0) {
    const int ew = warp - kEpiWarp0;
    const uint32_t slot0 = ptx::smem_u32(smem_epi + ew * SLOTS * kSlotBytes);
    auto slot = [&](int i) -> uint32_t { return slot0 + i * kSlotBytes; };
    auto slot_ptr = [&](int i) -> void* { return smem_epi + (ew * SLOTS + i) * kSlotBytes; };
    uint64_t* in_bar = &epi_in_bar[ew * 2];
    uint32_t in_phase = 0;
    int iter = 0;
    int store_set = 0;
    (void)in_bar; (void)in_phase; (void)store_set;

    if constexpr (EpiTraits<EPI, F32>::kPipe) {
      constexpr int NCH = BLOCK_N / 32;
      constexpr int SETB = PipeTraits<EPI>::kSetBytes;
      static_assert(NCH % 2 == 0, "ping-pong sets assume an even number of chunks per tile");
      static_assert(2 * SETB <= Cfg::kEpiBytes, "epilogue sets do not fit their shared-memory region");
      uint8_t* wsm = smem_epi;
      uint64_t* bar2 = &epi_in_bar[0];
      const PipeCtx ctx{&maps, &args, lane, ew};
      const bool leader = (ew == 0 && lane == 0);
      auto epi_sync = [&]() { ptx::named_bar_sync(1, 128); };
      auto row_of = [&](int w_) {
        return ((w_ % tiles_mn) / num_n_tiles) * kTileM * CG + static_cast<int>(cta_rank) * kTileM;
      };
      auto n0_of = [&](int w_) { return ((w_ % tiles_mn) % num_n_tiles) * BLOCK_N; };
      auto needs_in = [&](int n0_) { return EPI != EPI_ZR || n0_ >= args.n_split; };
      int set = 0;
      uint32_t ph = 0;
      bool issued = false;
#ifdef SRG_EPI_TIMING
      unsigned long long tacc_[8] = {0, 0, 0, 0, 0, 0, 0, 0};
#endif
      for (int w = cluster_id; w < total_work; w += num_clusters, ++iter) {
        const int row0 = row_of(w), n0 = n0_of(w);
        const int acc = iter & 1;
        const uint32_t acc_phase = (iter >> 1) & 1;
        const bool active = row0 < M_rt;
        const bool tin = needs_in(n0);
        const bool r_tile = (EPI == EPI_ZR) && tin;
        const uint32_t tacc = tmem_base + (static_cast<uint32_t>(ew * 32) << 16) + acc * BLOCK_N;
        float breg[8] = {0.f, 0.f, 0.f, 0.f, 0.f, 0.f, 0.f, 0.f};
        if constexpr (EPI == EPI_ZR || EPI == EPI_H) {
          if (active && lane * 8 < BLOCK_N) load_bias8(args.bias, n0 + lane * 8, 1.0f, breg);
        }
        SRG_T(tile_t0);
        if (!active) {
          ptx::mbar_wait(&tmem_full_bar[acc], acc_phase);
        } else {
#pragma unroll 1
          for (int cc = 0; cc < NCH; ++cc) {
            uint8_t* sp = wsm + set * SETB;
            int nw = w, ncc = cc + 1;
            bool nvalid = true;
            if (ncc == NCH) {
              nw = w + num_clusters;
              ncc = 0;
              nvalid = (nw < total_work) && (row_of(nw) < M_rt);
            }
            const bool pre = nvalid && needs_in(n0_of(nw));
            SRG_T(c0);
            if (leader && tin && !issued) {
              ptx::tma_wait_group_read<0>();
              pipe_issue<EPI>(ctx, sp, &bar2[set], n0, cc, row0);
            }
            SRG_T(c1);
            if (cc == 0) {
              ptx::mbar_wait(&tmem_full_bar[acc], acc_phase);
              ptx::tcgen05_fence_after();
            }
            SRG_T(c2);
            if (tin) {
              ptx::mbar_wait(&bar2[set], (ph >> set) & 1u);
              ph ^= (1u << set);
            }
            SRG_T(c3);
            if (leader) {
              if (pre) {
                ptx::tma_wait_group_read<0>();
                pipe_issue<EPI>(ctx, wsm + (set ^ 1) * SETB, &bar2[set ^ 1], n0_of(nw), ncc, row_of(nw));
              } else {
                ptx::tma_wait_group_read<1>();
              }
            }
            issued = pre;
            if (!tin) epi_sync();
            SRG_T(c4);
            float accv[32];
            ptx::tmem_ld_32x32(tacc + cc * 32, accv);
            ptx::tmem_ld_wait();
            pipe_compute<EPI>(ctx, ptx::smem_u32(sp), accv, breg, cc, r_tile);
            ptx::fence_proxy_async_smem();
            epi_sync();
            SRG_T(c5);
            if (leader) {
              pipe_store<EPI>(ctx, sp, n0, cc, row0, r_tile);
              ptx::tma_commit_group();
            }
            SRG_T(c6);
            SRG_TACC(1, 0, 1);
            SRG_TACC(3, c1, c2);
            SRG_TACC(4, c2, c3);
            SRG_TACC(5, c0, c1);
            SRG_TACC(5, c3, c4);
            SRG_TACC(6, c4, c5);
            SRG_TACC(7, c5, c6);
            set ^= 1;
          }
        }
        ptx::tcgen05_fence_before();
        if constexpr (CG == 2) ptx::mbar_arrive_cluster(&tmem_empty_bar[acc], 0);
        else ptx::mbar_arrive(&tmem_empty_bar[acc]);
        SRG_T(tile_t1);
        SRG_TACC(0, 0, 1);
        SRG_TACC(2, tile_t0, tile_t1);
      }
#ifdef SRG_EPI_TIMING
      if (lane == 0 && args.epi_t != nullptr)
        for (int i = 0; i < 8; ++i) atomicAdd(&args.epi_t[EPI * 8 + i], tacc_[i]);
#endif
      if (leader) ptx::tma_wait_group<0>();
      __syncwarp();
    } else
    for (int w = cluster_id; w < total_work; w += num_clusters, ++iter) {
      const int nt = (w % tiles_mn) % num_n_tiles;
      const int mt = (w % tiles_mn) / num_n_tiles;
      const int cta_row0 = mt * kTileM * CG + static_cast<int>(cta_rank) * kTileM;
      const int row0 = cta_row0 + ew * 32;
      const int n0 = nt * BLOCK_N;
      const int acc = F32 ? 0 : (iter & 1);
      const uint32_t acc_phase = F32 ? (iter & 1) : ((iter >> 1) & 1);
      const bool warp_active = (args.m_dev != nullptr) ? (cta_row0 < M_rt) : (row0 < M_rt);

      ptx::mbar_wait(&tmem_full_bar[acc], acc_phase);
      ptx::tcgen05_fence_after();
      const uint32_t tacc = tmem_base + (static_cast<uint32_t>(ew * 32) << 16) + acc * BLOCK_N;
      const bool has_corr = F32 && args.corr_kb_begin < total_kb;
      auto load_acc = [&](int col, float (&v)[32]) {
        ptx::tmem_ld_32x32(tacc + col, v);
        ptx::tmem_ld_wait();
        if constexpr (F32) {
          if (has_corr) {
            float c2[32];
            ptx::tmem_ld_32x32(tacc + BLOCK_N + col, c2);
            ptx::tmem_ld_wait();
#pragma unroll
            for (int i = 0; i < 32; ++i) v[i] += c2[i];
          }
        }
      };

      float st_max = -INFINITY, st_sum = 0.f;
      (void)st_max; (void)st_sum;

#pragma unroll 1
      for (int cc = 0; warp_active && cc < BLOCK_N / 64; ++cc) {
        const int gcol = n0 + cc * 64;
        float accv[32];

        if constexpr (EPI == EPI_STORE_BF16) {
          constexpr int kPer = F32 ? 3 : 1;
          const int s_hi = store_set * kPer, s_mid = s_hi + (F32 ? 1 : 0), s_lo = s_hi + (F32 ? 2 : 0);
          if (lane == 0) ptx::tma_wait_group_read<1>();
          __syncwarp();
#pragma unroll
          for (int half = 0; half < 2; ++half) {
            load_acc(cc * 64 + half * 32, accv);
#pragma unroll
            for (int g = 0; g < 4; ++g) {
              float b[8], v[8];
              load_bias8(args.bias, gcol + half * 32 + g * 8, args.bias_scale, b);
#pragma unroll
              for (int i = 0; i < 8; ++i) v[i] = fmaf(accv[g * 8 + i], args.alpha, b[i]);
              if (F32 && (args.flags & FLAG_LO)) slot_st_bf16x8_split(slot(s_hi), slot(s_mid), slot(s_lo), lane, half * 4 + g, v);
// ... 236 lines not shown
```

situation_recognition_b200/csrc/gemm_launch.cuh:

```cuda
#pragma once
#include <algorithm>
#include <cstdlib>
#include "host.cuh"

namespace srg {

template <int CG, int BLOCK_N, bool A_MN, bool B_MN, int EPI, bool F32>
inline int launch_gemm_inst(const GemmProblem& p, const GemmMaps& maps, const GemmArgs& args, const DeviceInfo& dev,
                            cudaStream_t stream) {
  using Cfg = GemmCfg<CG, BLOCK_N, EPI, F32>;
  auto kern = gemm_kernel<CG, BLOCK_N, A_MN, B_MN, EPI, F32>;
  static bool attr_done[kMaxDevices] = {};
  SRG_CHECK(dev.device >= 0 && dev.device < kMaxDevices, "device index %d out of range", dev.device);
  if (!attr_done[dev.device]) {
    SRG_CUDA(cudaFuncSetAttribute(kern, cudaFuncAttributeMaxDynamicSharedMemorySize, Cfg::kSmemBytes));
    attr_done[dev.device] = true;
  }
  const int num_m_tiles = (p.M + kTileM * CG - 1) / (kTileM * CG);
  const int total_work = num_m_tiles * (p.N / BLOCK_N) * args.k_splits;
  int clusters = dev.num_sms / CG;
  if (p.max_clusters > 0 && p.max_clusters < clusters) clusters = p.max_clusters;
  if (total_work < clusters) clusters = total_work;
  if (clusters <= 0) return SRG_OK;

// ... 99 lines not shown
    SRG_CHECK(p.a_mn && p.b_mn, "gemm: FLAG_BK_A is for MN-major operands (weight gradients)");
    for (int s = 0; s < p.nseg; ++s)
      SRG_CHECK(p.seg[s].a.ptr == p.seg[0].a.ptr, "gemm: FLAG_BK_A needs every segment in the same A matrix");
  }

  const void* aptr[kMaxAMaps];
  int n_amaps = 0;
  int ktot = 0;
  args.corr_kb_begin = 1 << 30;
  for (int s = 0; s < p.nseg; ++s) {
    const GemmSeg& sg = p.seg[s];
    SRG_CHECK(sg.k_len > 0 && (sg.k_len % kBlockK == 0 || s == p.nseg - 1), "gemm: segment %d K=%d not a multiple of 64",
              s, sg.k_len);
    SRG_CHECK(sg.a.dtype == DT_BF16, "gemm: A must be bf16");
    int mi = -1;
    for (int j = 0; j < n_amaps; ++j)
      if (aptr[j] == sg.a.ptr) mi = j;
    if (mi < 0) {
      SRG_CHECK(n_amaps < kMaxAMaps, "gemm: more than %d distinct A matrices", kMaxAMaps);
      mi = n_amaps++;
      aptr[mi] = sg.a.ptr;
      if (!p.a_mn) {
        SRG_CHECK(sg.a.rows >= p.M, "gemm: A segment %d has %lld rows < M=%d", s, (long long)sg.a.rows, p.M);
        SRG_TRY(make_tmap(&maps.a[mi], sg.a.ptr, DT_BF16, p.M, sg.a.cols, sg.a.ld, kTileM, kBlockK));
      } else {
        SRG_CHECK(sg.a.cols >= p.M, "gemm: MN-major A segment %d has %lld cols < M=%d", s, (long long)sg.a.cols, p.M);
        SRG_TRY(make_tmap(&maps.a[mi], sg.a.ptr, DT_BF16, sg.a.rows, p.M, sg.a.ld, kBlockK, 64));
      }
    }
    const int64_t kext = p.a_mn ? sg.a.rows : sg.a.cols;
    SRG_CHECK(sg.k_off >= 0 && sg.k_off + sg.k_len <= kext, "gemm: segment %d K range [%d,%d) outside A (%lld)", s,
              sg.k_off, sg.k_off + sg.k_len, (long long)kext);
    if (s == p.corr_seg_begin) args.corr_kb_begin = ktot / kBlockK;
    args.seg_map[s] = mi;
    args.seg_acol[s] = sg.k_off;
    args.seg_kb[s] = (sg.k_len + kBlockK - 1) / kBlockK;
    ktot += sg.k_len;
    if (sg.k_len % kBlockK != 0)
      SRG_CHECK(sg.k_off + sg.k_len == kext, "gemm: a K tail must end at the tensor extent (zero fill)");
  }
  for (int j = n_amaps; j < kMaxAMaps; ++j) maps.a[j] = maps.a[0];
  args.total_kb = (ktot + kBlockK - 1) / kBlockK;
  int k_splits = p.k_splits < args.total_kb ? p.k_splits : args.total_kb;
  {
    const int per = (args.total_kb + k_splits - 1) / k_splits;
    k_splits = (args.total_kb + per - 1) / per;
  }

  SRG_CHECK(p.b.dtype == DT_BF16, "gemm: B must be bf16");
  if (!p.b_mn) {
    SRG_CHECK(p.b.rows >= p.N && p.b.cols >= ktot, "gemm: B [%lld,%lld] smaller than [N=%d,K=%d]",
              (long long)p.b.rows, (long long)p.b.cols, p.N, ktot);
    SRG_CHECK(ktot % kBlockK == 0 || p.b.cols == ktot, "gemm: K tail needs B cols == K");
    SRG_TRY(make_tmap(&maps.b, p.b.ptr, DT_BF16, p.N, ktot, p.b.ld, block_n / p.cg, kBlockK));
  } else if (p.flags & FLAG_BK_A) {
    int64_t kmax = 0;
    for (int s = 0; s < p.nseg; ++s) kmax = std::max<int64_t>(kmax, p.seg[s].k_off + p.seg[s].k_len);
    SRG_CHECK(p.b.rows >= kmax && p.b.cols >= p.N, "gemm: MN-major B [%lld,%lld] smaller than [K=%lld,N=%d]",
              (long long)p.b.rows, (long long)p.b.cols, (long long)kmax, p.N);
    SRG_TRY(make_tmap(&maps.b, p.b.ptr, DT_BF16, p.b.rows, p.N, p.b.ld, kBlockK, 64));
  } else {
    SRG_CHECK(p.b.rows >= ktot && p.b.cols >= p.N, "gemm: MN-major B [%lld,%lld] smaller than [K=%d,N=%d]",
              (long long)p.b.rows, (long long)p.b.cols, ktot, p.N);
    SRG_CHECK(ktot % kBlockK == 0 || p.b.rows == ktot, "gemm: K tail needs B rows == K");
    SRG_TRY(make_tmap(&maps.b, p.b.ptr, DT_BF16, ktot, p.N, p.b.ld, kBlockK, 64));
  }
  bool have_io0 = false;
  for (int i = 0; i < kMaxIoMaps; ++i) {
    if (p.io[i].dtype == DT_NONE || p.io[i].ptr == nullptr) continue;
    const bool pipe = !p.f32 && (p.epi == EPI_ZR || p.epi == EPI_H || p.epi == EPI_DH || p.epi == EPI_DRH);
    SRG_TRY(make_tmap(&maps.io[i], p.io[i].ptr, p.io[i].dtype, p.io[i].rows, p.io[i].cols, p.io[i].ld,
                      pipe ? kTileM : 32, pipe ? 32 : io_box_cols(p.io[i].dtype)));
    if (i == 0) have_io0 = true;
  }
  (void)have_io0;

  args.k_splits = k_splits;
  args.alpha = p.alpha;
  args.bias = p.bias;
  args.bias_scale = p.bias_scale;
  args.n_split = p.n_split;
  args.n_valid = p.n_valid;
  args.stats = p.stats;
  args.flags = p.flags;
  static const bool b_evict_last = [] { const char* v = getenv("SRG_B_EVICT_LAST"); return !(v && v[0] == '0'); }();
  args.b_hint = (b_evict_last && !(p.a_mn && p.b_mn)) ? 0x14F0000000000000ull : 0ull;
#ifdef SRG_EPI_TIMING
  if (g_epi_t_dev == nullptr) {
    SRG_CUDA(cudaMalloc(reinterpret_cast<void**>(&g_epi_t_dev), 64 * sizeof(unsigned long long)));
    SRG_CUDA(cudaMemset(g_epi_t_dev, 0, 64 * sizeof(unsigned long long)));
  }
  args.epi_t = g_epi_t_dev;
#endif

  if (p.cg == 2) return dispatch_gemm<2, 256>(p, maps, args, dev, stream);
  return dispatch_gemm<1, 128>(p, maps, args, dev, stream);
}

}
```

situation_recognition_b200/csrc/host.cuh:

```cuda
#pragma once
#include <cstdarg>
#include <cstdio>
#include <cstring>
#include <atomic>
#include <string>
#include "gemm.cuh"

namespace srg {

inline thread_local char g_last_error[512] = "";

inline int set_error(int code, const char* fmt, ...) {
  va_list ap;
  va_start(ap, fmt);
  vsnprintf(g_last_error, sizeof(g_last_error), fmt, ap);
  va_end(ap);
  return code;
}

enum : int {
  SRG_OK = 0,
  SRG_ERR_ARG = 1,
  SRG_ERR_CUDA = 2,
  SRG_ERR_UNSUPPORTED = 3,
// ... 50 lines not shown
  int m_host[kProfMaxRecords], nseg[kProfMaxRecords], kb_host[kProfMaxRecords];
};
inline ProfState g_prof;
#ifdef SRG_EPI_TIMING
inline unsigned long long* g_epi_t_dev = nullptr;
#endif
inline int prof_kind(int epi, bool a_mn, bool b_mn) { return epi * 4 + (a_mn ? 2 : 0) + (b_mn ? 1 : 0); }

typedef CUresult (*PFN_encodeTiled)(CUtensorMap*, CUtensorMapDataType, cuuint32_t, void*, const cuuint64_t*,
                                    const cuuint64_t*, const cuuint32_t*, const cuuint32_t*, CUtensorMapInterleave,
                                    CUtensorMapSwizzle, CUtensorMapL2promotion, CUtensorMapFloatOOBfill);

inline PFN_encodeTiled get_encode_fn() {
  static PFN_encodeTiled fn = nullptr;
  if (fn) return fn;
  void* p = nullptr;
  cudaDriverEntryPointQueryResult qres;
  if (cudaGetDriverEntryPoint("cuTensorMapEncodeTiled", &p, cudaEnableDefault, &qres) != cudaSuccess ||
      qres != cudaDriverEntryPointSuccess)
    return nullptr;
  fn = reinterpret_cast<PFN_encodeTiled>(p);
  return fn;
}

enum DType : int { DT_NONE = 0, DT_F32 = 1, DT_BF16 = 2 };

inline int make_tmap(CUtensorMap* out, const void* ptr, int dtype, int64_t rows, int64_t cols, int64_t ld,
                     int box_rows, int box_cols) {
  PFN_encodeTiled enc = get_encode_fn();
  if (!enc) return set_error(SRG_ERR_CUDA, "cuTensorMapEncodeTiled entry point not available");
  const int es = (dtype == DT_F32) ? 4 : 2;
  SRG_CHECK(box_cols * es == 128 || box_cols * es == 64, "TMA box must span 128 or 64 bytes (got %d)", box_cols * es);
  const CUtensorMapSwizzle swz = (box_cols * es == 128) ? CU_TENSOR_MAP_SWIZZLE_128B : CU_TENSOR_MAP_SWIZZLE_64B;
  SRG_CHECK((reinterpret_cast<uintptr_t>(ptr) & 15) == 0, "TMA base pointer must be 16-byte aligned");
  SRG_CHECK(((ld * es) & 15) == 0, "TMA row pitch must be a multiple of 16 bytes (ld=%lld)", (long long)ld);
  SRG_CHECK(rows > 0 && cols > 0, "empty tensor for TMA (%lld x %lld)", (long long)rows, (long long)cols);
  cuuint64_t gdim[2] = {static_cast<cuuint64_t>(cols), static_cast<cuuint64_t>(rows)};
  cuuint64_t gstride[1] = {static_cast<cuuint64_t>(ld) * es};
  cuuint32_t box[2] = {static_cast<cuuint32_t>(box_cols), static_cast<cuuint32_t>(box_rows)};
  cuuint32_t estr[2] = {1, 1};
  CUresult r = enc(out, dtype == DT_F32 ? CU_TENSOR_MAP_DATA_TYPE_FLOAT32 : CU_TENSOR_MAP_DATA_TYPE_BFLOAT16, 2,
                   const_cast<void*>(ptr), gdim, gstride, box, estr, CU_TENSOR_MAP_INTERLEAVE_NONE,
                   swz, CU_TENSOR_MAP_L2_PROMOTION_L2_256B, CU_TENSOR_MAP_FLOAT_OOB_FILL_NONE);
  if (r != CUDA_SUCCESS)
    return set_error(SRG_ERR_CUDA, "cuTensorMapEncodeTiled failed (%d) rows=%lld cols=%lld ld=%lld box=%dx%d", (int)r,
                     (long long)rows, (long long)cols, (long long)ld, box_rows, box_cols);
  return SRG_OK;
}

struct Mat {
  const void* ptr = nullptr;
  int64_t rows = 0, cols = 0, ld = 0;
  int dtype = DT_NONE;
};
inline Mat mat(const void* p, int64_t rows, int64_t cols, int64_t ld, int dtype) {
  Mat m;
  m.ptr = p; m.rows = rows; m.cols = cols; m.ld = ld; m.dtype = dtype;
  return m;
}

struct GemmSeg {
  Mat a;
  int k_off;
  int k_len;
};

struct GemmProblem {
  int cg = 2;
  bool a_mn = false, b_mn = false;
  int epi = EPI_STORE_F32;
  bool f32 = false;
  int M = 0, N = 0;
  const int* m_dev = nullptr;
  const int* k_dev = nullptr;
  int nseg = 0;
  GemmSeg seg[kMaxSeg];
  Mat b;
  Mat io[kMaxIoMaps];
  float alpha = 1.f;
  const float* bias = nullptr;
  float bias_scale = 1.f;
  int n_split = 0, n_valid = 0;
  float* stats = nullptr;
  int flags = 0;
  int k_splits = 1;
  int corr_seg_begin = -1;
  int max_clusters = 0;
};

struct DeviceInfo {
  int device = -1;
  int num_sms = 0;
};

int run_gemm(const GemmProblem& p, const DeviceInfo& dev, cudaStream_t stream);

}
```

situation_recognition_b200/csrc/kernels_elementwise.cu:

```cuda
#include "elementwise.cuh"
#include "host.cuh"

namespace srg {

namespace {

constexpr int kMaxR = 8;
constexpr int kThreads = 256;

inline int grid_for(int64_t work, int threads = kThreads, int max_blocks = 148 * 16) {
  int64_t b = (work + threads - 1) / threads;
  if (b < 1) b = 1;
  if (b > max_blocks) b = max_blocks;
  return static_cast<int>(b);
}

__device__ __forceinline__ uint2 pack4_bf16(float a, float b, float c, float d) {
  __nv_bfloat162 lo = __floats2bfloat162_rn(a, b), hi = __floats2bfloat162_rn(c, d);
  uint2 r;
  r.x = *reinterpret_cast<uint32_t*>(&lo);
  r.y = *reinterpret_cast<uint32_t*>(&hi);
  return r;
}
__device__ __forceinline__ float bf16_round(float x) { return __bfloat162float(__float2bfloat16_rn(x)); }
// ... 7 lines not shown
  if (parts.mid != nullptr) {
    const float4 r1 = make_float4(v.x - bf16_round(v.x), v.y - bf16_round(v.y), v.z - bf16_round(v.z),
                                  v.w - bf16_round(v.w));
    *reinterpret_cast<uint2*>(parts.mid + idx) = pack4_bf16(r1.x, r1.y, r1.z, r1.w);
    *reinterpret_cast<uint2*>(parts.lo + idx) = pack4_bf16(r1.x - bf16_round(r1.x), r1.y - bf16_round(r1.y),
                                                           r1.z - bf16_round(r1.z), r1.w - bf16_round(r1.w));
  }
}

__global__ void k_gather_mask(const int32_t* __restrict__ verb2roles, const int32_t* __restrict__ role_count,
                              int n_verbs, int R, const int64_t* __restrict__ verb, int B,
                              int64_t* __restrict__ role_idx, float* __restrict__ mask, int* __restrict__ bad) {
  const int64_t total = static_cast<int64_t>(B) * R * R;
  for (int64_t t = blockIdx.x * static_cast<int64_t>(blockDim.x) + threadIdx.x; t < total;
       t += static_cast<int64_t>(gridDim.x) * blockDim.x) {
    const int b = static_cast<int>(t / (R * R));
    const int ij = static_cast<int>(t % (R * R));
    const int i = ij / R, j = ij % R;
    int64_t v = verb[b];
    const bool ok = (v >= 0 && v < n_verbs);
    if (!ok) {
      if (bad != nullptr) *bad = 1;
      v = 0;
    }
    const int n = role_count[v];
    if (mask != nullptr) {
      const bool on = (i < n && j < n && i != j) || (i >= n && i == j);
      mask[t] = on ? 1.0f : 0.0f;
    }
    if (role_idx != nullptr && i == 0) role_idx[static_cast<int64_t>(b) * R + j] = verb2roles[v * R + j];
  }
}

__global__ void k_node_init_verb(const float* __restrict__ feat, int64_t n4, float* __restrict__ h32,
                                 bf16* __restrict__ hb_hi, Parts hb_lo) {
  for (int64_t t = blockIdx.x * static_cast<int64_t>(blockDim.x) + threadIdx.x; t < n4;
       t += static_cast<int64_t>(gridDim.x) * blockDim.x) {
    float4 f = *reinterpret_cast<const float4*>(feat + t * 4);
    f.x = fmaxf(f.x, 0.f); f.y = fmaxf(f.y, 0.f); f.z = fmaxf(f.z, 0.f); f.w = fmaxf(f.w, 0.f);
    *reinterpret_cast<float4*>(h32 + t * 4) = f;
    store4_split(hb_hi, hb_lo, t * 4, f);
  }
}

__global__ void k_split_cast(const float* __restrict__ x, int64_t n4, bf16* __restrict__ hi, Parts lo) {
  for (int64_t t = blockIdx.x * static_cast<int64_t>(blockDim.x) + threadIdx.x; t < n4;
       t += static_cast<int64_t>(gridDim.x) * blockDim.x) {
    const float4 f = *reinterpret_cast<const float4*>(x + t * 4);
    store4_split(hi, lo, t * 4, f);
  }
}

__global__ void k_aggregate(const float* __restrict__ h32, const float* __restrict__ mask, int B, int R, int D,
                            bf16* __restrict__ a_hi, Parts a_lo) {
  const int D4 = D / 4;
  const int64_t total = static_cast<int64_t>(B) * D4;
  for (int64_t t = blockIdx.x * static_cast<int64_t>(blockDim.x) + threadIdx.x; t < total;
       t += static_cast<int64_t>(gridDim.x) * blockDim.x) {
    const int b = static_cast<int>(t / D4);
    const int d = static_cast<int>(t % D4) * 4;
    float4 h[kMaxR];
#pragma unroll
    for (int j = 0; j < kMaxR; ++j)
      if (j < R) h[j] = *reinterpret_cast<const float4*>(h32 + (static_cast<int64_t>(b) * R + j) * D + d);
    const float* mb = mask + static_cast<int64_t>(b) * R * R;
#pragma unroll
    for (int i = 0; i < kMaxR; ++i) {
      if (i < R) {
        float4 a = make_float4(0.f, 0.f, 0.f, 0.f);
#pragma unroll
        for (int j = 0; j < kMaxR; ++j) {
          if (j < R) {
            const float m = __ldg(mb + i * R + j);
            a.x = fmaf(m, h[j].x, a.x); a.y = fmaf(m, h[j].y, a.y);
            a.z = fmaf(m, h[j].z, a.z); a.w = fmaf(m, h[j].w, a.w);
          }
        }
        store4_split(a_hi, a_lo, (static_cast<int64_t>(b) * R + i) * D + d, a);
      }
    }
  }
}

__global__ void __launch_bounds__(1024)
k_prep_rows(const int32_t* __restrict__ role_count, int n_verbs, int R, const int64_t* __restrict__ verb, int B,
            int compact, int* __restrict__ cnt, int* __restrict__ off, int* __restrict__ meta, int* __restrict__ bad) {
  __shared__ int s_part[1024];
  const int tid = threadIdx.x;
  const int per = (B + 1023) / 1024;
  const int b0 = min(B, tid * per), b1 = min(B, b0 + per);
  int sum = 0;
  for (int b = b0; b < b1; ++b) {
    int64_t v = verb[b];
    if (v < 0 || v >= n_verbs) {
      if (bad != nullptr) *bad = 1;
      v = 0;
    }
    const int n = role_count[v];
    cnt[b] = n;
    sum += compact ? n : R;
  }
  s_part[tid] = sum;
  __syncthreads();
  for (int o = 1; o < 1024; o <<= 1) {
    const int v = (tid >= o) ? s_part[tid - o] : 0;
    __syncthreads();
    s_part[tid] += v;
    __syncthreads();
  }
  int run = s_part[tid] - sum;
  for (int b = b0; b < b1; ++b) {
    off[b] = run;
    run += compact ? cnt[b] : R;
  }
  if (tid == 1023) {
    const int n_real = s_part[1023];
    off[B] = n_real;
    meta[0] = n_real + 1;
    meta[1] = n_real;
    meta[2] = (n_real + 1 + 255) / 256 * 256;
    meta[3] = 0;
  }
}

constexpr int kSelfRows = 256;

__device__ __forceinline__ void store8_split(bf16* hi, Parts parts, int64_t idx, float4 a, float4 b) {
  store4_split(hi, parts, idx, a);
  store4_split(hi, parts, idx + 4, b);
}

__global__ void k_node_init_noun(const float* __restrict__ feat, const float* __restrict__ role_emb,
                                 const float* __restrict__ verb_emb, const int64_t* __restrict__ verb,
                                 const int32_t* __restrict__ verb2roles, int n_verbs, int B, int R, int D, RowMap rm,
                                 int feat_rep, float* __restrict__ h32, bf16* __restrict__ hb_hi, Parts hb_lo) {
  const int D4 = D / 4;
  const int64_t total = static_cast<int64_t>(B + kSelfRows) * D4;
  for (int64_t t = blockIdx.x * static_cast<int64_t>(blockDim.x) + threadIdx.x; t < total;
       t += static_cast<int64_t>(gridDim.x) * blockDim.x) {
    const int u = static_cast<int>(t / D4);
    const int d = static_cast<int>(t % D4) * 4;
    if (u >= B) {
      const int row = rm.meta[1] + (u - B);
      if (row < rm.meta[2]) {
        const int64_t off = static_cast<int64_t>(row) * D + d;
        const float4 z = make_float4(0.f, 0.f, 0.f, 0.f);
        *reinterpret_cast<float4*>(h32 + off) = z;
        store4_split(hb_hi, hb_lo, off, z);
      }
      continue;
    }
    const int b = u;
    int64_t v = verb[b];
    if (v < 0 || v >= n_verbs) v = 0;
    const float4 f = *reinterpret_cast<const float4*>(feat + static_cast<int64_t>(b / feat_rep) * D + d);
    const float4 ve = *reinterpret_cast<const float4*>(verb_emb + v * D + d);
    const int L = rm.compact ? rm.cnt[b] : R;
    const int base = rm.off[b];
    for (int r = 0; r < L; ++r) {
      const int idx = verb2roles[v * R + r];
      const float4 re = *reinterpret_cast<const float4*>(role_emb + static_cast<int64_t>(idx) * D + d);
      float4 o;
      o.x = fmaxf((f.x * re.x) * ve.x, 0.f);
      o.y = fmaxf((f.y * re.y) * ve.y, 0.f);
      o.z = fmaxf((f.z * re.z) * ve.z, 0.f);
      o.w = fmaxf((f.w * re.w) * ve.w, 0.f);
      const int64_t off = (static_cast<int64_t>(base) + r) * D + d;
      *reinterpret_cast<float4*>(h32 + off) = o;
      store4_split(hb_hi, hb_lo, off, o);
    }
  }
}

__global__ void k_aggregate_rows(const float* __restrict__ h32, RowMap rm, int B, int R, int D, bf16* __restrict__ a_hi,
                                 Parts a_lo) {
  const int D4 = D / 4;
  const int64_t total = static_cast<int64_t>(B + kSelfRows) * D4;
  for (int64_t t = blockIdx.x * static_cast<int64_t>(blockDim.x) + threadIdx.x; t < total;
       t += static_cast<int64_t>(gridDim.x) * blockDim.x) {
    const int u = static_cast<int>(t / D4);
    const int d = static_cast<int>(t % D4) * 4;
    if (u >= B) {
      const int row = rm.meta[1] + (u - B);
      if (row < rm.meta[2]) {
        const int64_t off = static_cast<int64_t>(row) * D + d;
        store4_split(a_hi, a_lo, off, *reinterpret_cast<const float4*>(h32 + off));
      }
      continue;
    }
    const int n = rm.cnt[u];
    const int L = rm.compact ? n : R;
    const int64_t base = static_cast<int64_t>(rm.off[u]) * D + d;
    float4 h[kMaxR];
#pragma unroll
    for (int j = 0; j < kMaxR; ++j)
      if (j < L) h[j] = *reinterpret_cast<const float4*>(h32 + base + static_cast<int64_t>(j) * D);
#pragma unroll
    for (int i = 0; i < kMaxR; ++i) {
      if (i < L) {
        float4 a = make_float4(0.f, 0.f, 0.f, 0.f);
        if (i < n) {
#pragma unroll
          for (int j = 0; j < kMaxR; ++j) {
            if (j < n && j != i) {
              a.x += h[j].x; a.y += h[j].y; a.z += h[j].z; a.w += h[j].w;
            }
          }
        } else {
          a = h[i];
        }
        store4_split(a_hi, a_lo, base + static_cast<int64_t>(i) * D, a);
      }
    }
  }
}

__device__ __forceinline__ uint4 philox4x32_10(uint4 c, uint2 k) {
#pragma unroll
  for (int i = 0; i < 10; ++i) {
    const uint32_t hi0 = __umulhi(0xD2511F53u, c.x), lo0 = 0xD2511F53u * c.x;
    const uint32_t hi1 = __umulhi(0xCD9E8D57u, c.z), lo1 = 0xCD9E8D57u * c.z;
    c = make_uint4(hi1 ^ c.y ^ k.x, lo1, hi0 ^ c.w ^ k.y, lo0);
    k.x += 0x9E3779B9u;
    k.y += 0xBB67AE85u;
  }
  return c;
}

__device__ __forceinline__ uint32_t keep_bits8(const DropSpec& ds, int64_t row, int col8, int64_t ld_keep) {
  if (ds.keep != nullptr) {
    const uint2 k = *reinterpret_cast<const uint2*>(ds.keep + row * ld_keep + static_cast<int64_t>(col8) * 8);
    uint32_t m = 0;
#pragma unroll
    for (int i = 0; i < 4; ++i) {
      m |= (((k.x >> (8 * i)) & 0xFFu) ? 1u : 0u) << i;
      m |= (((k.y >> (8 * i)) & 0xFFu) ? 1u : 0u) << (4 + i);
    }
    return m;
  }
  if (ds.seed == nullptr) return 0xFFu;
  const unsigned long long seed = static_cast<unsigned long long>(*ds.seed);
  const uint4 r = philox4x32_10(make_uint4(static_cast<uint32_t>(row), static_cast<uint32_t>(col8),
                                           static_cast<uint32_t>(ds.stream), static_cast<uint32_t>(row >> 32)),
                                make_uint2(static_cast<uint32_t>(seed), static_cast<uint32_t>(seed >> 32)));
  const uint32_t w[4] = {r.x, r.y, r.z, r.w};
  uint32_t m = 0;
#pragma unroll
  for (int i = 0; i < 4; ++i) {
    m |= ((w[i] & 0xFFFFu) < ds.thresh ? 1u : 0u) << (2 * i);
    m |= ((w[i] >> 16) < ds.thresh ? 1u : 0u) << (2 * i + 1);
  }
  return m;
}

__global__ void k_dropout_mask(DropSpec ds, int64_t rows, int D, uint8_t* __restrict__ out) {
  const int D8 = D / 8;
  const int64_t total = rows * D8;
  for (int64_t t = blockIdx.x * static_cast<int64_t>(blockDim.x) + threadIdx.x; t < total;
       t += static_cast<int64_t>(gridDim.x) * blockDim.x) {
    const int64_t row = t / D8;
    const int c8 = static_cast<int>(t % D8);
    const uint32_t m = keep_bits8(ds, row, c8, D);
    uint2 o;
    o.x = (m & 1u) | ((m >> 1 & 1u) << 8) | ((m >> 2 & 1u) << 16) | ((m >> 3 & 1u) << 24);
    o.y = (m >> 4 & 1u) | ((m >> 5 & 1u) << 8) | ((m >> 6 & 1u) << 16) | ((m >> 7 & 1u) << 24);
    *reinterpret_cast<uint2*>(out + row * D + static_cast<int64_t>(c8) * 8) = o;
  }
}

__global__ void k_classifier_input(const float* __restrict__ h32, RowMap rm, int R, int64_t rows, int D, DropSpec ds,
                                   bf16* __restrict__ x_hi, Parts x_lo) {
  const int D8 = D / 8;
  const int64_t total = rows * D8;
  for (int64_t t = blockIdx.x * static_cast<int64_t>(blockDim.x) + threadIdx.x; t < total;
       t += static_cast<int64_t>(gridDim.x) * blockDim.x) {
    const int64_t row = t / D8;
    const int c8 = static_cast<int>(t % D8);
    int64_t src = row;
    if (rm.cnt != nullptr) {
// ... 23 lines not shown
  for (int64_t t = blockIdx.x * static_cast<int64_t>(blockDim.x) + threadIdx.x; t < total;
       t += static_cast<int64_t>(gridDim.x) * blockDim.x) {
    const int row = rm.meta[1] + static_cast<int>(t / D4);
    if (row < rm.meta[2])
      *reinterpret_cast<float4*>(x + static_cast<int64_t>(row) * D + static_cast<int>(t % D4) * 4) =
          make_float4(0.f, 0.f, 0.f, 0.f);
  }
}

__global__ void k_classifier_input_bwd(const float* __restrict__ dx, RowMap rm, int B, int R, int D, DropSpec ds,
                                       float* __restrict__ dh, GruPre gp) {
  const int D8 = D / 8;
  const int c8 = blockIdx.x * blockDim.x + threadIdx.x;
  if (c8 >= D8) return;
  float acc[8] = {0.f, 0.f, 0.f, 0.f, 0.f, 0.f, 0.f, 0.f};
  bool any_pad = false;
  for (int b = blockIdx.y; b < B; b += gridDim.y) {
    const int L = (rm.cnt != nullptr) ? (rm.compact ? rm.cnt[b] : R) : R;
    const int64_t base = (rm.off != nullptr) ? rm.off[b] : static_cast<int64_t>(b) * R;
    for (int r = 0; r < R; ++r) {
      const int64_t row = static_cast<int64_t>(b) * R + r;
      const float* xp = dx + row * D + c8 * 8;
      const float4 a = *reinterpret_cast<const float4*>(xp), b4 = *reinterpret_cast<const float4*>(xp + 4);
      const uint32_t m = keep_bits8(ds, row, c8, D);
      const float sc = ds.scale;
      float v[8] = {a.x, a.y, a.z, a.w, b4.x, b4.y, b4.z, b4.w};
#pragma unroll
      for (int i = 0; i < 8; ++i) v[i] = ((m >> i) & 1u) ? v[i] * sc : 0.f;
      if (r < L && gp.z != nullptr) {
        const int64_t o = (base + r) * D + c8 * 8;
        const uint4 zz = *reinterpret_cast<const uint4*>(gp.z + o), cc = *reinterpret_cast<const uint4*>(gp.hc + o),
                    hh = *reinterpret_cast<const uint4*>(gp.h + o);
        const uint32_t zw[4] = {zz.x, zz.y, zz.z, zz.w}, cw[4] = {cc.x, cc.y, cc.z, cc.w}, hw[4] = {hh.x, hh.y, hh.z, hh.w};
        float dz[8], dc[8], da[8];
#pragma unroll
        for (int i = 0; i < 8; ++i) {
          const float zv = (i & 1) ? bf16_hi_f(zw[i >> 1]) : bf16_lo_f(zw[i >> 1]);
          const float cv = (i & 1) ? bf16_hi_f(cw[i >> 1]) : bf16_lo_f(cw[i >> 1]);
          const float hv = (i & 1) ? bf16_hi_f(hw[i >> 1]) : bf16_lo_f(hw[i >> 1]);
          dz[i] = v[i] * (cv - hv) * zv * (1.f - zv);
          dc[i] = v[i] * zv * (1.f - cv * cv);
          da[i] = v[i] * (1.f - zv);
        }
        const int64_t oo = (base + r) * gp.ld_out + c8 * 8;
        uint4 pz, ph;
        const uint2 z0 = pack4_bf16(dz[0], dz[1], dz[2], dz[3]), z1 = pack4_bf16(dz[4], dz[5], dz[6], dz[7]);
        const uint2 c0 = pack4_bf16(dc[0], dc[1], dc[2], dc[3]), c1 = pack4_bf16(dc[4], dc[5], dc[6], dc[7]);
        pz.x = z0.x; pz.y = z0.y; pz.z = z1.x; pz.w = z1.y;
        ph.x = c0.x; ph.y = c0.y; ph.z = c1.x; ph.w = c1.y;
        *reinterpret_cast<uint4*>(gp.dpre_z + oo) = pz;
        *reinterpret_cast<uint4*>(gp.dpre_h + oo) = ph;
        *reinterpret_cast<float4*>(gp.dh_acc + o) = make_float4(da[0], da[1], da[2], da[3]);
        *reinterpret_cast<float4*>(gp.dh_acc + o + 4) = make_float4(da[4], da[5], da[6], da[7]);
      } else if (r < L) {
        float* dp = dh + (base + r) * D + c8 * 8;
        *reinterpret_cast<float4*>(dp) = make_float4(v[0], v[1], v[2], v[3]);
        *reinterpret_cast<float4*>(dp + 4) = make_float4(v[4], v[5], v[6], v[7]);
      } else {
        any_pad = true;
#pragma unroll
        for (int i = 0; i < 8; ++i) acc[i] += v[i];
      }
    }
  }
  if (any_pad) {
    float* dp = dh + static_cast<int64_t>(rm.meta[1]) * D + c8 * 8;
    atomicAdd(reinterpret_cast<float4*>(dp), make_float4(acc[0], acc[1], acc[2], acc[3]));
    atomicAdd(reinterpret_cast<float4*>(dp + 4), make_float4(acc[4], acc[5], acc[6], acc[7]));
  }
}

struct PackJobs {
  PackJob j[kMaxPackJobs];
};
__global__ void k_pack_weight_multi(PackJobs jobs, int cols) {
  const PackJob job = jobs.j[blockIdx.y];
  const int c4 = cols / 4;
  const int64_t total = static_cast<int64_t>(job.rows_pad) * c4;
  for (int64_t t = blockIdx.x * static_cast<int64_t>(blockDim.x) + threadIdx.x; t < total;
       t += static_cast<int64_t>(gridDim.x) * blockDim.x) {
    const int r = static_cast<int>(t / c4);
    const int c = static_cast<int>(t % c4) * 4;
    float4 v = make_float4(0.f, 0.f, 0.f, 0.f);
    if (r < job.rows) v = *reinterpret_cast<const float4*>(job.src + static_cast<int64_t>(r) * cols + c);
    for (int k = 0; k < job.part; ++k) {
      v.x -= bf16_round(v.x); v.y -= bf16_round(v.y); v.z -= bf16_round(v.z); v.w -= bf16_round(v.w);
    }
    *reinterpret_cast<uint2*>(job.dst + static_cast<int64_t>(r) * job.ld_dst + job.col_off + c) =
        pack4_bf16(v.x, v.y, v.z, v.w);
  }
}

__global__ void k_pack_bias(const float* __restrict__ a, const float* __restrict__ b, int n, int n_pad,
                            float* __restrict__ dst) {
  for (int i = blockIdx.x * blockDim.x + threadIdx.x; i < n_pad; i += gridDim.x * blockDim.x) {
    float v = 0.f;
    if (i < n) v = a[i] + (b != nullptr ? b[i] : 0.f);
    dst[i] = v;
  }
}

__global__ void k_count_targets(const int64_t* __restrict__ gt, int B, int R, int ignore_index,
                                float* __restrict__ counts) {
  __shared__ int sc[3];
  if (threadIdx.x < 3) sc[threadIdx.x] = 0;
  __syncthreads();
  int local[3] = {0, 0, 0};
  const int64_t total = static_cast<int64_t>(B) * 3 * R;
  for (int64_t t = blockIdx.x * static_cast<int64_t>(blockDim.x) + threadIdx.x; t < total;
       t += static_cast<int64_t>(gridDim.x) * blockDim.x) {
    const int a = static_cast<int>((t / R) % 3);
    if (gt[t] != ignore_index) local[a]++;
  }
  for (int a = 0; a < 3; ++a)
    if (local[a]) atomicAdd(&sc[a], local[a]);
  __syncthreads();
  if (threadIdx.x < 3 && sc[threadIdx.x]) atomicAdd(&counts[threadIdx.x], static_cast<float>(sc[threadIdx.x]));
}

__device__ __forceinline__ float warp_max(float v) {
#pragma unroll
  for (int o = 16; o > 0; o >>= 1) v = fmaxf(v, __shfl_xor_sync(0xffffffffu, v, o));
  return v;
}
__device__ __forceinline__ float warp_sum(float v) {
#pragma unroll
  for (int o = 16; o > 0; o >>= 1) v += __shfl_xor_sync(0xffffffffu, v, o);
  return v;
}

template <int NT>
__global__ void k_cross_entropy(const float* __restrict__ logits, int64_t ldl, int n_classes, int rows,
                                const int64_t* __restrict__ gt, int R, int ignore_index,
                                const float* __restrict__ counts, float inv_fixed, float* __restrict__ loss,
                                float* __restrict__ dlogits, float grad_scale, const float* __restrict__ gscale_dev,
                                const float2* __restrict__ stats, int stats_tiles,
                                const float* __restrict__ total_dev, bf16* __restrict__ dlb, int64_t ld_b, int n_pad,
                                int accumulate) {
  __shared__ float s_loss[kThreads / 32];
  if (total_dev != nullptr) inv_fixed = 1.0f / fmaxf(__ldg(total_dev), 1.0f);
  if (gscale_dev != nullptr) grad_scale *= __ldg(gscale_dev);
  const int lane = threadIdx.x & 31, wib = threadIdx.x >> 5;
  const int warps_per_block = blockDim.x >> 5;
  float my_loss = 0.f;
  for (int row = blockIdx.x * warps_per_block + wib; row < rows; row += gridDim.x * warps_per_block) {
    const float* lr = logits + static_cast<int64_t>(row) * ldl;
    int64_t tgt[NT];
    float w[NT];
    float wsum = 0.f;
#pragma unroll
    for (int a = 0; a < NT; ++a) {
      if (NT == 3) {
        const int b = row / R, r = row % R;
        tgt[a] = gt[(static_cast<int64_t>(b) * 3 + a) * R + r];
        w[a] = (tgt[a] != ignore_index) ? 1.0f / counts[a] : 0.f;
      } else {
        tgt[a] = gt[row];
        w[a] = inv_fixed;
      }
      wsum += w[a];
    }
    if (wsum == 0.f && dlogits == nullptr && dlb == nullptr) continue;
    float mx = -INFINITY, se = 0.f;
    if (stats != nullptr) {
      float2 st = make_float2(-INFINITY, 0.f);
      if (lane < stats_tiles) st = stats[static_cast<int64_t>(row) * stats_tiles + lane];
      mx = warp_max(st.x);
// ... 146 lines not shown
    for (int i = 1; i < 8; ++i) {
      t.x += red[i][lane].x;
      t.y += red[i][lane].y;
    }
    if (out1 != nullptr) {
      atomicAdd(out1 + c, t.x * scale1);
      if (c + 1 < n_cols) atomicAdd(out1 + c + 1, t.y * scale1);
    }
    if (out2 != nullptr) {
      atomicAdd(out2 + c, t.x * scale2);
      if (c + 1 < n_cols) atomicAdd(out2 + c + 1, t.y * scale2);
    }
  }
}

template <bool kEmb, bool kFeat>
__global__ void k_node_init_bwd(const float* __restrict__ dh0, const bf16* __restrict__ h0b,
                                const float* __restrict__ feat, const float* __restrict__ role_emb,
                                const float* __restrict__ verb_emb, const int64_t* __restrict__ verb,
                                const int32_t* __restrict__ verb2roles, int n_verbs, int n_roles, int B, int R,
                                int D, RowMap rm, float* __restrict__ d_role_emb, float* __restrict__ d_verb_emb,
                                float* __restrict__ dfeat) {
  const int D4 = D / 4;
  const int64_t total = static_cast<int64_t>(B) * D4;
  for (int64_t t = blockIdx.x * static_cast<int64_t>(blockDim.x) + threadIdx.x; t < total;
       t += static_cast<int64_t>(gridDim.x) * blockDim.x) {
    const int b = static_cast<int>(t / D4);
    const int d = static_cast<int>(t % D4) * 4;
    int64_t v = verb[b];
    if (v < 0 || v >= n_verbs) v = 0;
    float4 f = make_float4(0.f, 0.f, 0.f, 0.f);
    if (kEmb) f = *reinterpret_cast<const float4*>(feat + static_cast<int64_t>(b) * D + d);
    const float4 ve = *reinterpret_cast<const float4*>(verb_emb + v * D + d);
    float4 accv = make_float4(0.f, 0.f, 0.f, 0.f);
    float4 accf = make_float4(0.f, 0.f, 0.f, 0.f);
    const int n = rm.cnt[b];
    const int64_t base = rm.off[b];
    for (int r = 0; r < n; ++r) {
      const int idx = verb2roles[v * R + r];
      if (idx == n_roles) continue;
      const int64_t off = (base + r) * D + d;
      float4 g = *reinterpret_cast<const float4*>(dh0 + off);
      const uint2 hb = *reinterpret_cast<const uint2*>(h0b + off);
      g.x = (bf16_lo_f(hb.x) > 0.f) ? g.x : 0.f;
      g.y = (bf16_hi_f(hb.x) > 0.f) ? g.y : 0.f;
      g.z = (bf16_lo_f(hb.y) > 0.f) ? g.z : 0.f;
      g.w = (bf16_hi_f(hb.y) > 0.f) ? g.w : 0.f;
      const float4 re = *reinterpret_cast<const float4*>(role_emb + static_cast<int64_t>(idx) * D + d);
      if (kEmb) {
        atomicAdd(reinterpret_cast<float4*>(d_role_emb + static_cast<int64_t>(idx) * D + d),
                  make_float4(g.x * f.x * ve.x, g.y * f.y * ve.y, g.z * f.z * ve.z, g.w * f.w * ve.w));
        accv.x = fmaf(g.x * f.x, re.x, accv.x);
        accv.y = fmaf(g.y * f.y, re.y, accv.y);
        accv.z = fmaf(g.z * f.z, re.z, accv.z);
        accv.w = fmaf(g.w * f.w, re.w, accv.w);
      }
      if (kFeat) {
        accf.x = fmaf(g.x * re.x, ve.x, accf.x);
        accf.y = fmaf(g.y * re.y, ve.y, accf.y);
        accf.z = fmaf(g.z * re.z, ve.z, accf.z);
        accf.w = fmaf(g.w * re.w, ve.w, accf.w);
      }
    }
    if (kEmb) atomicAdd(reinterpret_cast<float4*>(d_verb_emb + v * D + d), accv);
    if (kFeat) *reinterpret_cast<float4*>(dfeat + static_cast<int64_t>(b) * D + d) = accf;
  }
}

__global__ void k_node_init_verb_bwd(const float* __restrict__ dh0, const bf16* __restrict__ h0b, int64_t n4,
                                     float* __restrict__ dfeat) {
  for (int64_t t = blockIdx.x * static_cast<int64_t>(blockDim.x) + threadIdx.x; t < n4;
       t += static_cast<int64_t>(gridDim.x) * blockDim.x) {
    float4 g = *reinterpret_cast<const float4*>(dh0 + t * 4);
    const uint2 hb = *reinterpret_cast<const uint2*>(h0b + t * 4);
    g.x = (bf16_lo_f(hb.x) > 0.f) ? g.x : 0.f;
    g.y = (bf16_hi_f(hb.x) > 0.f) ? g.y : 0.f;
    g.z = (bf16_lo_f(hb.y) > 0.f) ? g.z : 0.f;
    g.w = (bf16_hi_f(hb.y) > 0.f) ? g.w : 0.f;
    *reinterpret_cast<float4*>(dfeat + t * 4) = g;
  }
}

__global__ void __launch_bounds__(kThreads, 4)
k_aggregate_t_rows(const bf16* __restrict__ da, const bf16* __restrict__ e, RowMap rm, int B, int R, int D,
                   bf16* __restrict__ ada) {
  const int D8 = D / 8;
  const bool rows_only = (rm.cnt == nullptr);
  const int64_t total = static_cast<int64_t>(rows_only ? B : B + kSelfRows) * D8;
  for (int64_t t = blockIdx.x * static_cast<int64_t>(blockDim.x) + threadIdx.x; t < total;
       t += static_cast<int64_t>(gridDim.x) * blockDim.x) {
    const int u = static_cast<int>(t / D8);
    const int d = static_cast<int>(t % D8) * 8;
    int n = 0, L = 1;
    int64_t base;
    if (rows_only) {
      base = static_cast<int64_t>(u) * D + d;
    } else if (u >= B) {
      const int row = rm.meta[1] + (u - B);
      if (row >= rm.meta[2]) continue;
      base = static_cast<int64_t>(row) * D + d;
    } else {
      n = rm.cnt[u];
      L = rm.compact ? n : R;
      base = static_cast<int64_t>(rm.off[u]) * D + d;
    }
    uint4 g[kMaxR];
#pragma unroll
    for (int i = 0; i < kMaxR; ++i)
      if (i < L) g[i] = *reinterpret_cast<const uint4*>(da + base + static_cast<int64_t>(i) * D);
#pragma unroll
    for (int j = 0; j < kMaxR; ++j) {
      if (j < L) {
        const uint4 ad = *reinterpret_cast<const uint4*>(e + base + static_cast<int64_t>(j) * D);
        float a[8] = {bf16_lo_f(ad.x), bf16_hi_f(ad.x), bf16_lo_f(ad.y), bf16_hi_f(ad.y),
                      bf16_lo_f(ad.z), bf16_hi_f(ad.z), bf16_lo_f(ad.w), bf16_hi_f(ad.w)};
#pragma unroll
        for (int i = 0; i < kMaxR; ++i) {
          const bool on = (j < n) ? (i < n && i != j) : (i == j);
          if (i < L && on) {
            a[0] += bf16_lo_f(g[i].x); a[1] += bf16_hi_f(g[i].x);
            a[2] += bf16_lo_f(g[i].y); a[3] += bf16_hi_f(g[i].y);
            a[4] += bf16_lo_f(g[i].z); a[5] += bf16_hi_f(g[i].z);
            a[6] += bf16_lo_f(g[i].w); a[7] += bf16_hi_f(g[i].w);
          }
        }
        uint4 o;
        const uint2 lo = pack4_bf16(a[0], a[1], a[2], a[3]), hi = pack4_bf16(a[4], a[5], a[6], a[7]);
        o.x = lo.x; o.y = lo.y; o.z = hi.x; o.w = hi.y;
        *reinterpret_cast<uint4*>(ada + base + static_cast<int64_t>(j) * D) = o;
      }
    }
  }
}

template <bool kGrad>
__device__ __forceinline__ void aggregate_t_chunk(const bf16* __restrict__ da, const bf16* __restrict__ e,
                                                  const float* __restrict__ mb, const bf16* __restrict__ h,
                                                  int64_t base, int R, int D, bf16* __restrict__ ada, float* acc) {
  uint4 g[kMaxR];
#pragma unroll
  for (int i = 0; i < kMaxR; ++i)
    if (i < R) g[i] = *reinterpret_cast<const uint4*>(da + base + static_cast<int64_t>(i) * D);
#pragma unroll
  for (int j = 0; j < kMaxR; ++j) {
    if (j < R) {
      const uint4 ad = *reinterpret_cast<const uint4*>(e + base + static_cast<int64_t>(j) * D);
      float a[8] = {bf16_lo_f(ad.x), bf16_hi_f(ad.x), bf16_lo_f(ad.y), bf16_hi_f(ad.y),
                    bf16_lo_f(ad.z), bf16_hi_f(ad.z), bf16_lo_f(ad.w), bf16_hi_f(ad.w)};
#pragma unroll
      for (int i = 0; i < kMaxR; ++i) {
        if (i < R) {
          const float m = __ldg(mb + i * R + j);
          a[0] = fmaf(m, bf16_lo_f(g[i].x), a[0]); a[1] = fmaf(m, bf16_hi_f(g[i].x), a[1]);
          a[2] = fmaf(m, bf16_lo_f(g[i].y), a[2]); a[3] = fmaf(m, bf16_hi_f(g[i].y), a[3]);
          a[4] = fmaf(m, bf16_lo_f(g[i].z), a[4]); a[5] = fmaf(m, bf16_hi_f(g[i].z), a[5]);
          a[6] = fmaf(m, bf16_lo_f(g[i].w), a[6]); a[7] = fmaf(m, bf16_hi_f(g[i].w), a[7]);
        }
      }
      uint4 o;
      const uint2 lo = pack4_bf16(a[0], a[1], a[2], a[3]), hi = pack4_bf16(a[4], a[5], a[6], a[7]);
      o.x = lo.x; o.y = lo.y; o.z = hi.x; o.w = hi.y;
      *reinterpret_cast<uint4*>(ada + base + static_cast<int64_t>(j) * D) = o;
      if constexpr (kGrad) {
        const uint4 hv = *reinterpret_cast<const uint4*>(h + base + static_cast<int64_t>(j) * D);
        const float hf[8] = {bf16_lo_f(hv.x), bf16_hi_f(hv.x), bf16_lo_f(hv.y), bf16_hi_f(hv.y),
                             bf16_lo_f(hv.z), bf16_hi_f(hv.z), bf16_lo_f(hv.w), bf16_hi_f(hv.w)};
#pragma unroll
        for (int i = 0; i < kMaxR; ++i) {
          if (i < R) {
            float s = acc[i * kMaxR + j];
            s = fmaf(bf16_lo_f(g[i].x), hf[0], s); s = fmaf(bf16_hi_f(g[i].x), hf[1], s);
            s = fmaf(bf16_lo_f(g[i].y), hf[2], s); s = fmaf(bf16_hi_f(g[i].y), hf[3], s);
            s = fmaf(bf16_lo_f(g[i].z), hf[4], s); s = fmaf(bf16_hi_f(g[i].z), hf[5], s);
            s = fmaf(bf16_lo_f(g[i].w), hf[6], s); s = fmaf(bf16_hi_f(g[i].w), hf[7], s);
            acc[i * kMaxR + j] = s;
          }
        }
      }
    }
  }
}

template <bool kGrad>
__global__ void __launch_bounds__(kGrad ? 128 : 256, kGrad ? 1 : 4)
k_aggregate_t(const bf16* __restrict__ da, const bf16* __restrict__ e, const float* __restrict__ mask,
              const bf16* __restrict__ h, int B, int R, int D, bf16* __restrict__ ada, float* __restrict__ dmask) {
  if constexpr (!kGrad) {
    const int D8 = D / 8;
    const int64_t total = static_cast<int64_t>(B) * D8;
    for (int64_t t = blockIdx.x * static_cast<int64_t>(blockDim.x) + threadIdx.x; t < total;
         t += static_cast<int64_t>(gridDim.x) * blockDim.x) {
      const int b = static_cast<int>(t / D8);
      const int d = static_cast<int>(t % D8) * 8;
      aggregate_t_chunk<false>(da, e, mask + static_cast<int64_t>(b) * R * R, nullptr,
                               static_cast<int64_t>(b) * R * D + d, R, D, ada, nullptr);
    }
  } else {
    constexpr int kAcc = kMaxR * kMaxR;
    __shared__ float red[4][kAcc];
    const int lane = threadIdx.x & 31, w = threadIdx.x >> 5;
    for (int b = blockIdx.x; b < B; b += gridDim.x) {
      const float* mb = mask + static_cast<int64_t>(b) * R * R;
      float acc[kAcc];
#pragma unroll
      for (int k = 0; k < kAcc; ++k) acc[k] = 0.f;
      for (int d = threadIdx.x * 8; d < D; d += blockDim.x * 8)
        aggregate_t_chunk<true>(da, e, mb, h, static_cast<int64_t>(b) * R * D + d, R, D, ada, acc);
#pragma unroll
      for (int i = 0; i < kMaxR; ++i) {
#pragma unroll
        for (int j = 0; j < kMaxR; ++j) {
          if (i < R && j < R) {
// ... 427 lines not shown
  return SRG_OK;
}

int launch_nouns_ce(const float* logits, int64_t ldl, int n_labels, const int64_t* gt, int B, int R,
                    const float* counts, float* loss, float* dlogits, float grad_scale, const float* gscale_dev,
                    const float* stats, int stats_tiles, bf16* dlb, int n_pad, int accumulate, cudaStream_t s) {
  const int rows = B * R;
  if (rows <= 0) return SRG_OK;
  int blocks = (rows + 7) / 8;
  if (blocks > 148 * 8) blocks = 148 * 8;
  if (stats_tiles > 32) stats = nullptr;
  k_cross_entropy<3><<<blocks, kThreads, 0, s>>>(logits, ldl, n_labels, rows, gt, R, n_labels, counts, 0.f, loss,
                                                dlogits, grad_scale, gscale_dev,
                                                reinterpret_cast<const float2*>(stats), stats_tiles, nullptr, dlb, n_pad,
                                                n_pad, accumulate);
  SRG_LAUNCH_CHECK();
  return SRG_OK;
}

int launch_verb_ce(const float* logits, int64_t ldl, int n_verbs, const int64_t* gt, int B, float inv_batch,
                   float* loss, float* dlogits, float grad_scale, const float* gscale_dev, const float* stats,
                   int stats_tiles, const float* batch_total, bf16* dlb, int n_pad, int accumulate, cudaStream_t s) {
  if (B <= 0) return SRG_OK;
  int blocks = (B + 7) / 8;
  if (blocks > 148 * 8) blocks = 148 * 8;
  if (stats_tiles > 32) stats = nullptr;
  k_cross_entropy<1><<<blocks, kThreads, 0, s>>>(logits, ldl, n_verbs, B, gt, 1, -100, nullptr, inv_batch, loss,
                                                dlogits, grad_scale, gscale_dev,
                                                reinterpret_cast<const float2*>(stats), stats_tiles, batch_total, dlb,
                                                n_pad, n_pad, accumulate);
  SRG_LAUNCH_CHECK();
  return SRG_OK;
}

int launch_row_topk_logsoftmax(const float* x, int64_t ldl, int rows, int n, int k, int64_t* idx, float* logp,
                               cudaStream_t s) {
  if (rows <= 0) return SRG_OK;
  if (k < 1 || k > 16 || n < k || ldl < n)
    return set_error(SRG_ERR_ARG, "topk_logsoftmax: need 1 <= k <= 16, k <= n <= ldl (k=%d, n=%d, ldl=%lld)", k, n,
                     (long long)ldl);
  const int blocks = grid_for(static_cast<int64_t>(rows) * 32);
  if (k == 1) k_row_topk_logsoftmax<1><<<blocks, kThreads, 0, s>>>(x, ldl, rows, n, k, idx, logp);
  else if (k <= 4) k_row_topk_logsoftmax<4><<<blocks, kThreads, 0, s>>>(x, ldl, rows, n, k, idx, logp);
  else if (k <= 8) k_row_topk_logsoftmax<8><<<blocks, kThreads, 0, s>>>(x, ldl, rows, n, k, idx, logp);
  else k_row_topk_logsoftmax<16><<<blocks, kThreads, 0, s>>>(x, ldl, rows, n, k, idx, logp);
  SRG_LAUNCH_CHECK();
  return SRG_OK;
}

int launch_situation_finish(const int64_t* verb, const int32_t* role_count, int n_verbs, int R, int n_cand,
                            const float* verb_logp, int64_t* labels, float* label_logp, float* score, cudaStream_t s) {
  if (n_cand <= 0) return SRG_OK;
  k_situation_finish<<<grid_for(n_cand), kThreads, 0, s>>>(verb, role_count, n_verbs, R, n_cand, verb_logp, labels,
                                                          label_logp, score);
  SRG_LAUNCH_CHECK();
  return SRG_OK;
}

int launch_cast_pad(const float* src, int64_t ld, int rows, int n_valid, int n_pad, bf16* dst, int accumulate,
                    cudaStream_t s) {
  if (rows <= 0) return SRG_OK;
  if (n_pad % 8 != 0) return set_error(SRG_ERR_ARG, "cast_pad: padded width %d must be a multiple of 8", n_pad);
  k_cast_pad<<<grid_for(static_cast<int64_t>(rows) * n_pad / 8), kThreads, 0, s>>>(src, ld, rows, n_valid, n_pad, dst,
                                                                                   accumulate);
  SRG_LAUNCH_CHECK();
  return SRG_OK;
}

int launch_colsum(const bf16* X, int64_t ld, int rows, int n_cols, float* out1, float scale1, float* out2,
                  float scale2, cudaStream_t s) {
  if (rows <= 0 || n_cols <= 0) return SRG_OK;
  int slabs = (rows + 255) / 256;
  if (slabs > 64) slabs = 64;
  dim3 grid((n_cols + 63) / 64, slabs);
  k_colsum<<<grid, kThreads, 0, s>>>(X, ld, rows, n_cols, out1, scale1, out2, scale2);
  SRG_LAUNCH_CHECK();
  return SRG_OK;
}

int launch_prep_rows(const int32_t* role_count, int n_verbs, int R, const int64_t* verb, int B, int compact,
                     RowMap rm, int* bad, cudaStream_t s) {
  if (B <= 0) return SRG_OK;
  k_prep_rows<<<1, 1024, 0, s>>>(role_count, n_verbs, R, verb, B, compact, const_cast<int*>(rm.cnt),
                                 const_cast<int*>(rm.off), const_cast<int*>(rm.meta), bad);
  SRG_LAUNCH_CHECK();
  return SRG_OK;
}

int launch_node_init_noun(const float* feat, const float* role_emb, const float* verb_emb, const int64_t* verb,
                          const int32_t* verb2roles, int n_verbs, int B, int R, int D, RowMap rm, int feat_rep,
                          float* h32, bf16* hb_hi, bf16* hb_mid, bf16* hb_lo, cudaStream_t s) {
  if (B <= 0) return SRG_OK;
  if (R > kMaxR) return set_error(SRG_ERR_UNSUPPORTED, "max_role_count %d > %d", R, kMaxR);
  if (feat_rep < 1) return set_error(SRG_ERR_ARG, "node_init_noun: feat_rep %d < 1", feat_rep);
  k_node_init_noun<<<grid_for(static_cast<int64_t>(B + kSelfRows) * D / 4), kThreads, 0, s>>>(
      feat, role_emb, verb_emb, verb, verb2roles, n_verbs, B, R, D, rm, feat_rep, h32, hb_hi, Parts{hb_mid, hb_lo});
  SRG_LAUNCH_CHECK();
  return SRG_OK;
}

int launch_aggregate_rows(const float* h32, RowMap rm, int B, int R, int D, bf16* a_hi, bf16* a_mid, bf16* a_lo,
                          cudaStream_t s) {
  if (B <= 0) return SRG_OK;
  if (R > kMaxR) return set_error(SRG_ERR_UNSUPPORTED, "max_role_count %d > %d", R, kMaxR);
  k_aggregate_rows<<<grid_for(static_cast<int64_t>(B + kSelfRows) * D / 4), kThreads, 0, s>>>(h32, rm, B, R, D, a_hi,
                                                                                            Parts{a_mid, a_lo});
  SRG_LAUNCH_CHECK();
  return SRG_OK;
}

int launch_aggregate_t_rows(const bf16* da, const bf16* e, RowMap rm, int B, int R, int D, bf16* ada, cudaStream_t s) {
  if (B <= 0) return SRG_OK;
  if (R > kMaxR) return set_error(SRG_ERR_UNSUPPORTED, "max_role_count %d > %d", R, kMaxR);
  const int64_t units = (rm.cnt == nullptr) ? B : B + kSelfRows;
  k_aggregate_t_rows<<<grid_for(units * D / 8), kThreads, 0, s>>>(da, e, rm, B, R, D, ada);
  SRG_LAUNCH_CHECK();
  return SRG_OK;
}

int launch_aggregate_t(const bf16* da, const bf16* e, const float* mask, const bf16* h, int B, int R, int D,
                       bf16* ada, float* dmask, cudaStream_t s) {
  if (B <= 0) return SRG_OK;
  if (R > kMaxR) return set_error(SRG_ERR_UNSUPPORTED, "max_role_count %d > %d", R, kMaxR);
  if (D % 256 != 0) return set_error(SRG_ERR_ARG, "aggregate_t: D=%d must be a multiple of 256", D);
  if (dmask != nullptr) {
    if (h == nullptr) return set_error(SRG_ERR_ARG, "aggregate_t: dmask needs the step's state operand");
    const int blocks = B < 148 * 16 ? B : 148 * 16;
    k_aggregate_t<true><<<blocks, D / 8 < 128 ? D / 8 : 128, 0, s>>>(da, e, mask, h, B, R, D, ada, dmask);
  } else {
    k_aggregate_t<false><<<grid_for(static_cast<int64_t>(B) * D / 8), kThreads, 0, s>>>(da, e, mask, nullptr, B, R, D,
                                                                                       ada, nullptr);
  }
  SRG_LAUNCH_CHECK();
  return SRG_OK;
}

int launch_classifier_input(const float* h32, RowMap rm, int R, int64_t rows, int D, DropSpec ds, bf16* x_hi,
                            bf16* x_mid, bf16* x_lo, cudaStream_t s) {
  if (rows <= 0) return SRG_OK;
  if (D % 8 != 0) return set_error(SRG_ERR_ARG, "classifier_input: D=%d must be a multiple of 8", D);
  k_classifier_input<<<grid_for(rows * D / 8), kThreads, 0, s>>>(h32, rm, R, rows, D, ds, x_hi, Parts{x_mid, x_lo});
  SRG_LAUNCH_CHECK();
  return SRG_OK;
}

int launch_classifier_input_bwd(const float* dx, RowMap rm, int B, int R, int D, DropSpec ds, float* dh, GruPre gp,
                                cudaStream_t s) {
  if (B <= 0) return SRG_OK;
  if (D % 8 != 0) return set_error(SRG_ERR_ARG, "classifier_input_bwd: D=%d must be a multiple of 8", D);
  if (rm.meta != nullptr) {
    k_zero_self_rows<<<grid_for(static_cast<int64_t>(kSelfRows) * D / 4), kThreads, 0, s>>>(dh, rm, D);
    SRG_LAUNCH_CHECK();
  }
  const int D8 = D / 8;
  const int threads = D8 < kThreads ? D8 : kThreads;
  const int chunks = (D8 + threads - 1) / threads;
  int slabs = (148 * 8) / chunks;
  if (slabs > B) slabs = B;
  if (slabs < 1) slabs = 1;
  dim3 grid(chunks, slabs);
  k_classifier_input_bwd<<<grid, threads, 0, s>>>(dx, rm, B, R, D, ds, dh, gp);
  SRG_LAUNCH_CHECK();
  return SRG_OK;
}

int launch_dropout_mask(DropSpec ds, int64_t rows, int D, uint8_t* out, cudaStream_t s) {
  if (rows <= 0) return SRG_OK;
  if (D % 8 != 0) return set_error(SRG_ERR_ARG, "dropout_mask: D=%d must be a multiple of 8", D);
  k_dropout_mask<<<grid_for(rows * D / 8), kThreads, 0, s>>>(ds, rows, D, out);
  SRG_LAUNCH_CHECK();
  return SRG_OK;
}

int launch_node_init_bwd(const float* dh0, const bf16* h0b, const float* feat, const float* role_emb,
                         const float* verb_emb, const int64_t* verb, const int32_t* verb2roles, int n_verbs,
                         int n_roles, int B, int R, int D, RowMap rm, float* d_role_emb, float* d_verb_emb,
                         float* dfeat, cudaStream_t s) {
  const bool emb = (d_role_emb != nullptr && d_verb_emb != nullptr);
  if (B <= 0 || (!emb && dfeat == nullptr)) return SRG_OK;
  auto kern = emb ? (dfeat ? k_node_init_bwd<true, true> : k_node_init_bwd<true, false>) : k_node_init_bwd<false, true>;
  kern<<<grid_for(static_cast<int64_t>(B) * D / 4), kThreads, 0, s>>>(
      dh0, h0b, feat, role_emb, verb_emb, verb, verb2roles, n_verbs, n_roles, B, R, D, rm, d_role_emb, d_verb_emb,
      dfeat);
  SRG_LAUNCH_CHECK();
  return SRG_OK;
}

int launch_node_init_verb_bwd(const float* dh0, const bf16* h0b, int B, int D, float* dfeat, cudaStream_t s) {
  if (B <= 0) return SRG_OK;
  const int64_t n4 = static_cast<int64_t>(B) * D / 4;
  k_node_init_verb_bwd<<<grid_for(n4), kThreads, 0, s>>>(dh0, h0b, n4, dfeat);
  SRG_LAUNCH_CHECK();
  return SRG_OK;
}

int launch_colsum_multi(const ColsumJob* jobs, int n_jobs, int64_t ld, int rows, const int* rows_dev, int nseg,
                        int64_t seg_stride, int n_cols, cudaStream_t s) {
  if (rows <= 0 || n_cols <= 0 || n_jobs <= 0 || nseg <= 0) return SRG_OK;
// ... 89 lines not shown
```

Measured before the change: 291,600.

## Factor GGNN aggregation through per-image row sums and folded weights

Message aggregation is rewritten as a per-image sum minus the self term. Both the forward z/r GEMM and the backward dh GEMM now multiply only a small per-image summed matrix by the weights and add the result back in the epilogue through a gather index (srow). Weights are prepacked with sign and offset folded in (Wdg_noun/Wdg_verb built from P32 and U). This removes the full-size aggregated operand and the per-row aggregate_t pass, at the cost of new precomputed weight buffers, an extra small GEMM and gathered loads in the epilogue. Precision shifts because the sums are rounded to bf16.

New measurement: 317,400 (median of 6 runs). +8.9%, better.

```diff
diff --git a/include/srggnn.h b/include/srggnn.h
--- a/include/srggnn.h
+++ b/include/srggnn.h
@@ -98,6 +98,8 @@
                            float* dlogits, void* dlogits_bf16, int accumulate, const float* stats, void* stream);
 size_t srg_workspace_dlogits_offset(srg_handle* h, int mode, int B, const void* workspace);
 
+int srg_packed_weights(srg_handle* h, int which, void* out, void* stream);
+
 size_t srg_workspace_stats_offset(srg_handle* h, int mode, int B, int precision, int save_for_backward,
                                   const void* workspace);
 
diff --git a/situation_recognition_b200/_lib.py b/situation_recognition_b200/_lib.py
--- a/situation_recognition_b200/_lib.py
+++ b/situation_recognition_b200/_lib.py
@@ -49,6 +49,7 @@
     "srg_verb_loss_backward": (_i, [_vp, _vp, _i64, _vp, _i, _f, _vp, _vp, _f, _vp, _vp, _i, _vp, _vp]),
     "srg_workspace_stats_offset": (_sz, [_vp, _i, _i, _i, _i, _vp]),
     "srg_workspace_dlogits_offset": (_sz, [_vp, _i, _i, _vp]),
+    "srg_packed_weights": (_i, [_vp, _i, _vp, _vp]),
     "srg_nouns_backward": (_i, [_vp, _vp, _i64, _i, _vp, _vp, _i, _vp, _vp, _vp, _f, _vp, _i64, _c.POINTER(SrgGrads),
                                 _vp, _sz, _vp]),
     "srg_verb_backward": (_i, [_vp, _vp, _i64, _i, _i, _vp, _f, _vp, _i64, _c.POINTER(SrgGrads), _vp, _sz, _vp]),
diff --git a/situation_recognition_b200/csrc/capi_ggnn.cu b/situation_recognition_b200/csrc/capi_ggnn.cu
--- a/situation_recognition_b200/csrc/capi_ggnn.cu
+++ b/situation_recognition_b200/csrc/capi_ggnn.cu
@@ -1,3 +1,4 @@
+#include <algorithm>
 #include <new>
 #include <vector>
 #include "elementwise.cuh"
@@ -34,7 +35,9 @@
   bf16 *Wm_hi = nullptr, *Wm_mid = nullptr, *Wm_lo = nullptr;
   bf16 *Wp6 = nullptr;
   bf16 *P_hi = nullptr, *P_mid = nullptr, *P_lo = nullptr;
+  float* P32 = nullptr;
   bf16 *U_stack = nullptr, *Uh = nullptr;
+  bf16 *Wdg_noun = nullptr, *Wdg_verb = nullptr;
   float *wb = nullptr;
   float *bzr[2] = {nullptr, nullptr};
   float *bh[2] = {nullptr, nullptr};
@@ -66,7 +69,11 @@
   float* stats = nullptr;
   float *dh = nullptr, *dh_acc = nullptr, *dx = nullptr;
   bf16* dpre_all = nullptr;
-  bf16 *da = nullptr, *ada = nullptr, *e = nullptr, *dlb = nullptr;
+  bf16 *e = nullptr, *dlb = nullptr;
+  bf16 *da = nullptr, *ada = nullptr;
+  bf16 *Sd = nullptr, *Gd = nullptr;
+  bf16 *S = nullptr, *Gzr = nullptr;
+  int S_rows = 0;
   float* G_P = nullptr;
   bf16* G_Pb = nullptr;
   float* s_all = nullptr;
@@ -105,7 +112,13 @@
     pb.rm.cnt = bump.take<int>(B);
     pb.rm.off = bump.take<int>(static_cast<size_t>(B) + 1);
     pb.rm.meta = bump.take<int>(4);
+    pb.rm.srow = bump.take<int>(M);
     pb.rm.compact = h->compact;
+    pb.S_rows = B + (h->compact ? 256 : M);
+    if (!f32) {
+      pb.S = bump.take<bf16>(static_cast<size_t>(pb.S_rows) * D);
+      pb.Gzr = bump.take<bf16>(static_cast<size_t>(pb.S_rows) * 2 * D);
+    }
   }
   pb.h32 = bump.take<float>(MD);
   const int n_hb = save ? T + 1 : 2;
@@ -151,8 +164,13 @@
     pb.dh_acc = bump.take<float>(MD);
     pb.dx = bump.take<float>(MfD);
     pb.dpre_all = bump.take<bf16>(static_cast<size_t>(T) * 3 * MD);
-    pb.da = bump.take<bf16>(MD);
-    pb.ada = bump.take<bf16>(MD);
+    if (rowmap) {
+      pb.Sd = bump.take<bf16>(static_cast<size_t>(pb.S_rows) * 3 * D);
+      pb.Gd = bump.take<bf16>(static_cast<size_t>(pb.S_rows) * D);
+    } else if (mode == SRG_MODE_NOUN) {
+      pb.da = bump.take<bf16>(MD);
+      pb.ada = bump.take<bf16>(MD);
+    }
     pb.e = bump.take<bf16>(MD);
     pb.dlb = bump.take<bf16>(static_cast<size_t>(Mfull) * npad);
     pb.G_P = bump.take<float>(static_cast<size_t>(3) * D * D);
@@ -268,22 +286,41 @@
     StepBufs& st = pb.st[t];
     const Split3 hcur = {{pb.hb_hi[t], pb.hb_mid[t], pb.hb_lo[t]}};
     Split3 a = hcur;
+    const bool sums = (pb.S != nullptr);
     if (mode == SRG_MODE_NOUN) {
-      if (pb.rm.meta != nullptr) SRG_TRY(launch_aggregate_rows(h32, pb.rm, B, h->R, D, st.a_hi, st.a_mid, st.a_lo, s));
+      if (pb.rm.meta != nullptr)
+        SRG_TRY(launch_aggregate_rows(h32, pb.rm, B, h->R, D, st.a_hi, st.a_mid, st.a_lo, pb.S, s));
       else SRG_TRY(launch_aggregate(h32, mask, B, h->R, D, st.a_hi, st.a_mid, st.a_lo, s));
       a = Split3{{st.a_hi, st.a_mid, st.a_lo}};
+    }
+    if (sums) {
+      GemmProblem q = base_problem(h, pb.S_rows, 2 * D);
+      q.m_dev = pb.rm.meta + 3;
+      add_seg(q, pb.S, pb.S_rows, D, 0, D);
+      q.b = mat(h->Wzr, 2 * D, D, 2 * D, DT_BF16);
+      q.epi = EPI_STORE_BF16;
+      q.io[0] = mat(pb.Gzr, pb.S_rows, 2 * D, 2 * D, DT_BF16);
+      SRG_TRY(run_gemm(q, h->dev, s));
     }
     const Split3 rh = {{st.rh_hi, st.rh_mid, st.rh_lo}};
     {
       GemmProblem p = path_problem(h, pb, 2 * D);
-      const Split3 ops[2] = {a, hcur};
-      add_split_segs(p, M, D, f32, ops, 2);
-      p.b = mat(h->Wzr, 2 * D, static_cast<int64_t>(2 * D) * kmul, static_cast<int64_t>(2 * D) * kmul, DT_BF16);
+      if (sums) {
+        add_seg(p, hcur.part[0], M, D, 0, D);
+        p.b = mat(h->Wdg_noun + static_cast<size_t>(D) * D, 2 * D, D, D, DT_BF16);
+        p.flags = FLAG_GSUM;
+        p.gsum = pb.Gzr;
+        p.gsum_row = pb.rm.srow;
+      } else {
+        const Split3 ops[2] = {a, hcur};
+        add_split_segs(p, M, D, f32, ops, 2);
+        p.b = mat(h->Wzr, 2 * D, static_cast<int64_t>(2 * D) * kmul, static_cast<int64_t>(2 * D) * kmul, DT_BF16);
+      }
       p.epi = EPI_ZR;
       p.f32 = f32;
       p.bias = h->bzr[mi];
       p.n_split = D;
-      p.flags = (f32 ? FLAG_LO : 0) | (save ? FLAG_STASH : 0);
+      p.flags |= (f32 ? FLAG_LO : 0) | (save ? FLAG_STASH : 0);
       p.io[0] = mat(st.z, M, D, D, f32 ? DT_F32 : DT_BF16);
       p.io[1] = mat(h32, M, D, D, DT_F32);
       p.io[2] = mat(st.rh_hi, M, D, D, DT_BF16);
@@ -436,25 +473,41 @@
     }
     {
       GemmProblem p = path_problem(h, pb, D);
-      add_seg_ld(p, dp, M, ld3, ld3, 0, 3 * D);
       p.b_mn = true;
-      p.b = mat(h->P_hi, 3 * D, D, D, DT_BF16);
-      p.epi = EPI_STORE_BF16;
-      p.io[0] = mat(pb.da, M, D, D, DT_BF16);
-      SRG_TRY(run_gemm(p, h->dev, s));
-    }
-    if (mask != nullptr) SRG_TRY(launch_aggregate_t(pb.da, pb.e, mask, pb.hb_hi[t], B, R, D, pb.ada, dmask, s));
-    else SRG_TRY(launch_aggregate_t_rows(pb.da, pb.e, pb.rm, mapped ? B : M, R, D, pb.ada, s));
-    const bf16* ada = pb.ada;
-    {
-      GemmProblem p = path_problem(h, pb, D);
-      add_seg_ld(p, dp, M, ld3, ld3, D, 2 * D);
-      p.b_mn = true;
-      p.b = mat(h->U_stack, 2 * D, D, D, DT_BF16);
       p.epi = EPI_DH;
       p.flags = FLAG_ADD;
       p.io[0] = mat(dh_acc, M, D, D, DT_F32);
-      p.io[6] = mat(ada, M, D, D, DT_BF16);
+      if (mask != nullptr) {
+        GemmProblem q = path_problem(h, pb, D);
+        add_seg_ld(q, dp, M, ld3, ld3, 0, 3 * D);
+        q.b_mn = true;
+        q.b = mat(h->P_hi, 3 * D, D, D, DT_BF16);
+        q.epi = EPI_STORE_BF16;
+        q.io[0] = mat(pb.da, M, D, D, DT_BF16);
+        SRG_TRY(run_gemm(q, h->dev, s));
+        SRG_TRY(launch_aggregate_t(pb.da, pb.e, mask, pb.hb_hi[t], B, R, D, pb.ada, dmask, s));
+        add_seg_ld(p, dp, M, ld3, ld3, D, 2 * D);
+        p.b = mat(h->U_stack, 2 * D, D, D, DT_BF16);
+        p.io[6] = mat(pb.ada, M, D, D, DT_BF16);
+      } else {
+        add_seg_ld(p, dp, M, ld3, ld3, 0, 3 * D);
+        p.b = mat(mapped ? h->Wdg_noun : h->Wdg_verb, 3 * D, D, D, DT_BF16);
+        p.io[6] = mat(pb.e, M, D, D, DT_BF16);
+        if (mapped) {
+          SRG_TRY(launch_row_sums(dp, ld3, pb.rm, B, R, 3 * D, pb.Sd, s));
+          GemmProblem q = base_problem(h, pb.S_rows, D);
+          q.m_dev = pb.rm.meta + 3;
+          add_seg(q, pb.Sd, pb.S_rows, 3 * D, 0, 3 * D);
+          q.b_mn = true;
+          q.b = mat(h->P_hi, 3 * D, D, D, DT_BF16);
+          q.epi = EPI_STORE_BF16;
+          q.io[0] = mat(pb.Gd, pb.S_rows, D, D, DT_BF16);
+          SRG_TRY(run_gemm(q, h->dev, s));
+          p.flags |= FLAG_GSUM;
+          p.gsum = pb.Gd;
+          p.gsum_row = pb.rm.srow;
+        }
+      }
       if (t > 0) {
         bf16* dn = dpre_of(t - 1);
         p.flags |= FLAG_NEXT;
@@ -558,6 +611,9 @@
     SRG_TRY(re(&h->P_lo, 3 * D * D));
     SRG_TRY(re(&h->U_stack, 2 * D * D));
     SRG_TRY(re(&h->Uh, D * D));
+    SRG_TRY(re(&h->Wdg_noun, 3 * D * D));
+    SRG_TRY(re(&h->Wdg_verb, 3 * D * D));
+    SRG_TRY(f32buf(&h->P32, 3 * D * D));
     SRG_TRY(f32buf(&h->wb, 3 * D));
     for (int i = 0; i < 2; ++i) {
       SRG_TRY(f32buf(&h->bzr[i], 2 * D));
@@ -618,8 +674,8 @@
   if (!h) return SRG_OK;
   DeviceGuard guard_(h->device);
   void* ptrs[] = {h->d_verb2roles, h->d_role_count, h->d_bad, h->Wzr, h->Wh, h->Wcn, h->Wcv, h->Wm_hi, h->Wm_mid, h->Wm_lo, h->Wp6,
-                  h->P_hi, h->P_mid, h->P_lo, h->U_stack, h->Uh, h->wb, h->bzr[0], h->bzr[1], h->bh[0], h->bh[1], h->bcn, h->bcv,
-                  h->acc_GP, h->acc_GPb, h->acc_s};
+                  h->P_hi, h->P_mid, h->P_lo, h->P32, h->U_stack, h->Uh, h->Wdg_noun, h->Wdg_verb, h->wb, h->bzr[0],
+                  h->bzr[1], h->bh[0], h->bh[1], h->bcn, h->bcv, h->acc_GP, h->acc_GPb, h->acc_s};
   for (void* p : ptrs)
     if (p) cudaFree(p);
   delete h;
@@ -715,15 +771,37 @@
     if (f32) g.corr_seg_begin = 1;
     g.b_mn = true;
     g.b = mat(h->Wp6, static_cast<int64_t>(p_terms) * D, D, D, DT_BF16);
-    g.epi = EPI_STORE_BF16;
-    g.f32 = f32;
-    g.flags = f32 ? FLAG_LO : 0;
-    g.io[0] = mat(h->P_hi, 3 * D, D, D, DT_BF16);
     if (f32) {
+      g.epi = EPI_STORE_BF16;
+      g.f32 = true;
+      g.flags = FLAG_LO;
+      g.io[0] = mat(h->P_hi, 3 * D, D, D, DT_BF16);
       g.io[1] = mat(h->P_mid, 3 * D, D, D, DT_BF16);
       g.io[2] = mat(h->P_lo, 3 * D, D, D, DT_BF16);
+    } else {
+      g.epi = EPI_STORE_F32;
+      g.io[0] = mat(h->P32, 3 * D, D, D, DT_F32);
     }
     SRG_TRY(run_gemm(g, h->dev, s));
+  }
+  if (!f32) {
+    const float* Ux[3] = {nullptr, p->U_z, p->U_r};
+    for (int x = 0; x < 3; ++x) {
+      const float* Px = h->P32 + x * DD;
+      queue(Px, D, D, h->P_hi + x * DD, D, 0, 0);
+      for (int v = 0; v < 2; ++v) {
+        const float sign = v ? 1.f : -1.f;
+        queue(x == 0 ? Px : Ux[x], D, D, (v ? h->Wdg_verb : h->Wdg_noun) + x * DD, D, 0, 0);
+        if (x == 0) {
+          jobs.back().scale = sign;
+        } else {
+          jobs.back().add = Px;
+          jobs.back().add_scale = sign;
+        }
+      }
+    }
+    SRG_TRY(launch_pack_weight_multi(jobs.data(), static_cast<int>(jobs.size()), D, s));
+    jobs.clear();
   }
 
   const int64_t ld1 = static_cast<int64_t>(D) * split, ld2 = static_cast<int64_t>(2 * D) * split;
@@ -780,9 +858,24 @@
   return static_cast<size_t>(reinterpret_cast<const uint8_t*>(pb.dlb) - static_cast<const uint8_t*>(workspace));
 }
 
+int srg_packed_weights(srg_handle* h, int which, void* out, void* stream) {
+  SRG_CHECK(h != nullptr, "srg_packed_weights: null handle");
+  DeviceGuard guard_(h->device);
+  SRG_CHECK(out != nullptr, "srg_packed_weights: null output");
+  SRG_CHECK(h->packed_prec == SRG_PREC_BF16, "srg_packed_weights: weights are not packed for bf16");
+  SRG_CHECK(which >= 0 && which <= 2, "srg_packed_weights: which=%d must be 0, 1 or 2", which);
+  const size_t n = static_cast<size_t>(3) * h->D * h->D;
+  const void* src = (which == 0) ? static_cast<const void*>(h->P32) : (which == 1) ? h->Wdg_noun : h->Wdg_verb;
+  SRG_CUDA(cudaMemcpyAsync(out, src, n * (which == 0 ? sizeof(float) : sizeof(bf16)), cudaMemcpyDeviceToDevice,
+                           static_cast<cudaStream_t>(stream)));
+  return SRG_OK;
+}
+
 size_t srg_workspace_bytes(srg_handle* h, int mode, int B, int precision, int save_for_backward) {
   if (!h || B <= 0) return 0;
-  return carve(h, mode, B, precision, save_for_backward, nullptr, mode == SRG_MODE_NOUN).bytes;
+  const size_t dense = carve(h, mode, B, precision, save_for_backward, nullptr, false).bytes;
+  if (mode != SRG_MODE_NOUN) return dense;
+  return std::max(dense, carve(h, mode, B, precision, save_for_backward, nullptr, true).bytes);
 }
 
 }
diff --git a/situation_recognition_b200/csrc/elementwise.cuh b/situation_recognition_b200/csrc/elementwise.cuh
--- a/situation_recognition_b200/csrc/elementwise.cuh
+++ b/situation_recognition_b200/csrc/elementwise.cuh
@@ -11,6 +11,7 @@
   const int* cnt = nullptr;
   const int* off = nullptr;
   const int* meta = nullptr;
+  const int* srow = nullptr;
   int compact = 0;
 };
 
@@ -31,8 +32,8 @@
                           const int32_t* verb2roles, int n_verbs, int B, int R, int D, RowMap rm, int feat_rep,
                           float* h32, bf16* hb_hi, bf16* hb_mid, bf16* hb_lo, cudaStream_t s);
 int launch_aggregate_rows(const float* h32, RowMap rm, int B, int R, int D, bf16* a_hi, bf16* a_mid, bf16* a_lo,
-                          cudaStream_t s);
-int launch_aggregate_t_rows(const bf16* da, const bf16* e, RowMap rm, int B, int R, int D, bf16* ada, cudaStream_t s);
+                          bf16* S, cudaStream_t s);
+int launch_row_sums(const bf16* x, int64_t ld, RowMap rm, int B, int R, int cols, bf16* Sd, cudaStream_t s);
 int launch_aggregate_t(const bf16* da, const bf16* e, const float* mask, const bf16* h, int B, int R, int D,
                        bf16* ada, float* dmask, cudaStream_t s);
 int launch_classifier_input(const float* h32, RowMap rm, int R, int64_t rows, int D, DropSpec ds, bf16* x_hi,
@@ -62,6 +63,9 @@
   int64_t ld_dst;
   int64_t col_off;
   int rows, rows_pad, part;
+  float scale = 1.f;
+  const float* add = nullptr;
+  float add_scale = 0.f;
 };
 constexpr int kMaxPackJobs = 48;
 int launch_pack_weight_multi(const PackJob* jobs, int n_jobs, int cols, cudaStream_t s);
diff --git a/situation_recognition_b200/csrc/epilogue_pipe.cuh b/situation_recognition_b200/csrc/epilogue_pipe.cuh
--- a/situation_recognition_b200/csrc/epilogue_pipe.cuh
+++ b/situation_recognition_b200/csrc/epilogue_pipe.cuh
@@ -72,19 +72,25 @@
   }
 }
 
+__device__ __forceinline__ float gsum_at(const uint4 (&gv)[4], int g, int i) {
+  const uint32_t w = (i >> 1) == 0 ? gv[g].x : (i >> 1) == 1 ? gv[g].y : (i >> 1) == 2 ? gv[g].z : gv[g].w;
+  return (i & 1) ? bf16_hi_f(w) : bf16_lo_f(w);
+}
 template <int EPI>
 __device__ __forceinline__ void pipe_compute(const PipeCtx& c, uint32_t s, const float (&acc)[32],
-                                             const float (&breg)[8], int cc, bool r_tile) {
+                                             const float (&breg)[8], const uint4 (&gv)[4], int cc, bool r_tile) {
   const GemmArgs& a = *c.args;
   const int lane = c.lane;
   const uint32_t sf = s + c.ew * kF32Warp;
   auto sb = [&](int region_off) -> uint32_t { return s + region_off + c.ew * kB16Warp; };
   if constexpr (EPI == EPI_ZR) {
     float b[4][8];
+    const bool gs = (a.flags & FLAG_GSUM) != 0;
 #pragma unroll
     for (int g = 0; g < 4; ++g)
 #pragma unroll
-      for (int i = 0; i < 8; ++i) b[g][i] = __shfl_sync(0xffffffffu, breg[i], cc * 4 + g);
+      for (int i = 0; i < 8; ++i)
+        b[g][i] = __shfl_sync(0xffffffffu, breg[i], cc * 4 + g) + (gs ? gsum_at(gv, g, i) : 0.f);
     if (!r_tile) {
 #pragma unroll
       for (int g = 0; g < 4; ++g) {
@@ -152,6 +158,10 @@
         if (has_add) {
 #pragma unroll
           for (int i = 0; i < 8; ++i) dh[j][i] += ad[j][i];
+        }
+        if (a.flags & FLAG_GSUM) {
+#pragma unroll
+          for (int i = 0; i < 8; ++i) dh[j][i] += gsum_at(gv, g, i);
         }
         if (next) {
           float dz[8], dc[8];
diff --git a/situation_recognition_b200/csrc/gemm.cuh b/situation_recognition_b200/csrc/gemm.cuh
--- a/situation_recognition_b200/csrc/gemm.cuh
+++ b/situation_recognition_b200/csrc/gemm.cuh
@@ -23,7 +23,7 @@
   EPI_DH = 6,
 };
 
-enum : int { FLAG_LO = 1, FLAG_STASH = 2, FLAG_REDUCE = 4, FLAG_NEXT = 8, FLAG_ADD = 16, FLAG_BK_A = 32 };
+enum : int { FLAG_LO = 1, FLAG_STASH = 2, FLAG_REDUCE = 4, FLAG_NEXT = 8, FLAG_ADD = 16, FLAG_BK_A = 32, FLAG_GSUM = 64 };
 
 struct GemmMaps {
   CUtensorMap a[kMaxAMaps];
@@ -48,6 +48,8 @@
   int n_split;
   int n_valid;
   float* stats;
+  const __nv_bfloat16* gsum;
+  const int* gsum_row;
   int flags;
   unsigned long long b_hint;
 #ifdef SRG_EPI_TIMING
@@ -429,6 +431,16 @@
             }
             const bool pre = nvalid && needs_in(n0_of(nw));
             SRG_T(c0);
+            uint4 gv[4] = {};
+            if constexpr (EPI == EPI_DH || EPI == EPI_ZR) {
+              if (args.flags & FLAG_GSUM) {
+                const int row = row0 + ew * 32 + lane;
+                const uint4* gp = reinterpret_cast<const uint4*>(
+                    args.gsum + static_cast<int64_t>(__ldg(args.gsum_row + row)) * args.N + n0 + cc * 32);
+#pragma unroll
+                for (int q = 0; q < 4; ++q) gv[q] = __ldg(gp + q);
+              }
+            }
             if (leader && tin && !issued) {
               ptx::tma_wait_group_read<0>();
               pipe_issue<EPI>(ctx, sp, &bar2[set], n0, cc, row0);
@@ -458,7 +470,7 @@
             float accv[32];
             ptx::tmem_ld_32x32(tacc + cc * 32, accv);
             ptx::tmem_ld_wait();
-            pipe_compute<EPI>(ctx, ptx::smem_u32(sp), accv, breg, cc, r_tile);
+            pipe_compute<EPI>(ctx, ptx::smem_u32(sp), accv, breg, gv, cc, r_tile);
             ptx::fence_proxy_async_smem();
             epi_sync();
             SRG_T(c5);
diff --git a/situation_recognition_b200/csrc/gemm_launch.cuh b/situation_recognition_b200/csrc/gemm_launch.cuh
--- a/situation_recognition_b200/csrc/gemm_launch.cuh
+++ b/situation_recognition_b200/csrc/gemm_launch.cuh
@@ -205,6 +205,11 @@
   args.n_split = p.n_split;
   args.n_valid = p.n_valid;
   args.stats = p.stats;
+  SRG_CHECK(!(p.flags & FLAG_GSUM) ||
+                ((p.epi == EPI_DH || p.epi == EPI_ZR) && !p.f32 && p.gsum != nullptr && p.gsum_row != nullptr),
+            "gemm: FLAG_GSUM needs a bf16 EPI_DH / EPI_ZR kernel, gsum and gsum_row");
+  args.gsum = p.gsum;
+  args.gsum_row = p.gsum_row;
   args.flags = p.flags;
   static const bool b_evict_last = [] { const char* v = getenv("SRG_B_EVICT_LAST"); return !(v && v[0] == '0'); }();
   args.b_hint = (b_evict_last && !(p.a_mn && p.b_mn)) ? 0x14F0000000000000ull : 0ull;
diff --git a/situation_recognition_b200/csrc/host.cuh b/situation_recognition_b200/csrc/host.cuh
--- a/situation_recognition_b200/csrc/host.cuh
+++ b/situation_recognition_b200/csrc/host.cuh
@@ -156,6 +156,8 @@
   float bias_scale = 1.f;
   int n_split = 0, n_valid = 0;
   float* stats = nullptr;
+  const __nv_bfloat16* gsum = nullptr;
+  const int* gsum_row = nullptr;
   int flags = 0;
   int k_splits = 1;
   int corr_seg_begin = -1;
diff --git a/situation_recognition_b200/csrc/kernels_elementwise.cu b/situation_recognition_b200/csrc/kernels_elementwise.cu
--- a/situation_recognition_b200/csrc/kernels_elementwise.cu
+++ b/situation_recognition_b200/csrc/kernels_elementwise.cu
@@ -113,14 +113,17 @@
   }
 }
 
+constexpr int kSelfRows = 256;
+
 __global__ void __launch_bounds__(1024)
 k_prep_rows(const int32_t* __restrict__ role_count, int n_verbs, int R, const int64_t* __restrict__ verb, int B,
-            int compact, int* __restrict__ cnt, int* __restrict__ off, int* __restrict__ meta, int* __restrict__ bad) {
-  __shared__ int s_part[1024];
+            int compact, int* __restrict__ cnt, int* __restrict__ off, int* __restrict__ meta, int* __restrict__ srow,
+            int* __restrict__ bad) {
+  __shared__ int s_part[1024], s_pad[1024];
   const int tid = threadIdx.x;
   const int per = (B + 1023) / 1024;
   const int b0 = min(B, tid * per), b1 = min(B, b0 + per);
-  int sum = 0;
+  int sum = 0, pads = 0;
   for (int b = b0; b < b1; ++b) {
     int64_t v = verb[b];
     if (v < 0 || v >= n_verbs) {
@@ -130,31 +133,44 @@
     const int n = role_count[v];
     cnt[b] = n;
     sum += compact ? n : R;
+    pads += compact ? 0 : R - n;
   }
   s_part[tid] = sum;
+  s_pad[tid] = pads;
   __syncthreads();
   for (int o = 1; o < 1024; o <<= 1) {
     const int v = (tid >= o) ? s_part[tid - o] : 0;
+    const int p = (tid >= o) ? s_pad[tid - o] : 0;
     __syncthreads();
     s_part[tid] += v;
+    s_pad[tid] += p;
     __syncthreads();
   }
-  int run = s_part[tid] - sum;
+  int run = s_part[tid] - sum, pad_run = B + s_pad[tid] - pads;
   for (int b = b0; b < b1; ++b) {
     off[b] = run;
-    run += compact ? cnt[b] : R;
-  }
+    const int n = cnt[b], L = compact ? n : R;
+    if (!compact)
+      for (int r = 0; r < L; ++r) srow[run + r] = (r < n) ? b : pad_run++;
+    run += L;
+  }
+  if (compact) {
+    __syncthreads();
+    for (int b = tid; b < B; b += 1024)
+      for (int r = 0, o = off[b], n = cnt[b]; r < n; ++r) srow[o + r] = b;
+  }
+  const int n_real = s_part[1023];
+  const int rows_touched = (n_real + 1 + 255) / 256 * 256;
+  const int tail0 = B + s_pad[1023];
+  if (tid < kSelfRows && n_real + tid < rows_touched) srow[n_real + tid] = tail0 + tid;
   if (tid == 1023) {
-    const int n_real = s_part[1023];
     off[B] = n_real;
     meta[0] = n_real + 1;
     meta[1] = n_real;
-    meta[2] = (n_real + 1 + 255) / 256 * 256;
-    meta[3] = 0;
-  }
-}
-
-constexpr int kSelfRows = 256;
+    meta[2] = rows_touched;
+    meta[3] = tail0 + rows_touched - n_real;
+  }
+}
 
 __device__ __forceinline__ void store8_split(bf16* hi, Parts parts, int64_t idx, float4 a, float4 b) {
   store4_split(hi, parts, idx, a);
@@ -204,7 +220,7 @@
 }
 
 __global__ void k_aggregate_rows(const float* __restrict__ h32, RowMap rm, int B, int R, int D, bf16* __restrict__ a_hi,
-                                 Parts a_lo) {
+                                 Parts a_lo, bf16* __restrict__ S) {
   const int D4 = D / 4;
   const int64_t total = static_cast<int64_t>(B + kSelfRows) * D4;
   for (int64_t t = blockIdx.x * static_cast<int64_t>(blockDim.x) + threadIdx.x; t < total;
@@ -215,7 +231,11 @@
       const int row = rm.meta[1] + (u - B);
       if (row < rm.meta[2]) {
         const int64_t off = static_cast<int64_t>(row) * D + d;
-        store4_split(a_hi, a_lo, off, *reinterpret_cast<const float4*>(h32 + off));
+        const float4 v = *reinterpret_cast<const float4*>(h32 + off);
+        store4_split(a_hi, a_lo, off, v);
+        if (S != nullptr)
+          *reinterpret_cast<uint2*>(S + static_cast<int64_t>(rm.srow[row]) * D + d) =
+              pack4_bf16(2.f * v.x, 2.f * v.y, 2.f * v.z, 2.f * v.w);
       }
       continue;
     }
@@ -226,6 +246,22 @@
 #pragma unroll
     for (int j = 0; j < kMaxR; ++j)
       if (j < L) h[j] = *reinterpret_cast<const float4*>(h32 + base + static_cast<int64_t>(j) * D);
+    if (S != nullptr) {
+      float4 sum = make_float4(0.f, 0.f, 0.f, 0.f);
+#pragma unroll
+      for (int j = 0; j < kMaxR; ++j) {
+        if (j < n) {
+          sum.x += h[j].x; sum.y += h[j].y; sum.z += h[j].z; sum.w += h[j].w;
+        }
+      }
+      *reinterpret_cast<uint2*>(S + static_cast<int64_t>(u) * D + d) = pack4_bf16(sum.x, sum.y, sum.z, sum.w);
+#pragma unroll
+      for (int j = 0; j < kMaxR; ++j) {
+        if (j >= n && j < L)
+          *reinterpret_cast<uint2*>(S + static_cast<int64_t>(rm.srow[rm.off[u] + j]) * D + d) =
+              pack4_bf16(2.f * h[j].x, 2.f * h[j].y, 2.f * h[j].z, 2.f * h[j].w);
+      }
+    }
 #pragma unroll
     for (int i = 0; i < kMaxR; ++i) {
       if (i < L) {
@@ -415,7 +451,15 @@
     const int r = static_cast<int>(t / c4);
     const int c = static_cast<int>(t % c4) * 4;
     float4 v = make_float4(0.f, 0.f, 0.f, 0.f);
-    if (r < job.rows) v = *reinterpret_cast<const float4*>(job.src + static_cast<int64_t>(r) * cols + c);
+    if (r < job.rows) {
+      const int64_t o = static_cast<int64_t>(r) * cols + c;
+      v = *reinterpret_cast<const float4*>(job.src + o);
+      v.x *= job.scale; v.y *= job.scale; v.z *= job.scale; v.w *= job.scale;
+      if (job.add != nullptr) {
+        const float4 w = *reinterpret_cast<const float4*>(job.add + o);
+        v.x += job.add_scale * w.x; v.y += job.add_scale * w.y; v.z += job.add_scale * w.z; v.w += job.add_scale * w.w;
+      }
+    }
     for (int k = 0; k < job.part; ++k) {
       v.x -= bf16_round(v.x); v.y -= bf16_round(v.y); v.z -= bf16_round(v.z); v.w -= bf16_round(v.w);
     }
@@ -728,52 +772,53 @@
 }
 
 __global__ void __launch_bounds__(kThreads, 4)
-k_aggregate_t_rows(const bf16* __restrict__ da, const bf16* __restrict__ e, RowMap rm, int B, int R, int D,
-                   bf16* __restrict__ ada) {
-  const int D8 = D / 8;
-  const bool rows_only = (rm.cnt == nullptr);
-  const int64_t total = static_cast<int64_t>(rows_only ? B : B + kSelfRows) * D8;
+k_row_sums(const bf16* __restrict__ x, int64_t ld, RowMap rm, int B, int R, int cols, bf16* __restrict__ Sd) {
+  const int C8 = cols / 8;
+  const int64_t total = static_cast<int64_t>(B + kSelfRows) * C8;
+  auto put = [&](int64_t srow, int c, const float (&a)[8]) {
+    uint4 o;
+    const uint2 lo = pack4_bf16(a[0], a[1], a[2], a[3]), hi = pack4_bf16(a[4], a[5], a[6], a[7]);
+    o.x = lo.x; o.y = lo.y; o.z = hi.x; o.w = hi.y;
+    *reinterpret_cast<uint4*>(Sd + srow * cols + c) = o;
+  };
+  auto twice = [&](const uint4 g, float (&a)[8]) {
+    a[0] = 2.f * bf16_lo_f(g.x); a[1] = 2.f * bf16_hi_f(g.x); a[2] = 2.f * bf16_lo_f(g.y); a[3] = 2.f * bf16_hi_f(g.y);
+    a[4] = 2.f * bf16_lo_f(g.z); a[5] = 2.f * bf16_hi_f(g.z); a[6] = 2.f * bf16_lo_f(g.w); a[7] = 2.f * bf16_hi_f(g.w);
+  };
   for (int64_t t = blockIdx.x * static_cast<int64_t>(blockDim.x) + threadIdx.x; t < total;
        t += static_cast<int64_t>(gridDim.x) * blockDim.x) {
-    const int u = static_cast<int>(t / D8);
-    const int d = static_cast<int>(t % D8) * 8;
-    int n = 0, L = 1;
-    int64_t base;
-    if (rows_only) {
-      base = static_cast<int64_t>(u) * D + d;
-    } else if (u >= B) {
+    const int u = static_cast<int>(t / C8);
+    const int c = static_cast<int>(t % C8) * 8;
+    float a[8];
+    if (u >= B) {
       const int row = rm.meta[1] + (u - B);
       if (row >= rm.meta[2]) continue;
-      base = static_cast<int64_t>(row) * D + d;
-    } else {
-      n = rm.cnt[u];
-      L = rm.compact ? n : R;
-      base = static_cast<int64_t>(rm.off[u]) * D + d;
-    }
+      twice(*reinterpret_cast<const uint4*>(x + row * ld + c), a);
+      put(rm.srow[row], c, a);
+      continue;
+    }
+    const int n = rm.cnt[u];
+    const int L = rm.compact ? n : R;
+    const int64_t base = rm.off[u];
     uint4 g[kMaxR];
 #pragma unroll
     for (int i = 0; i < kMaxR; ++i)
-      if (i < L) g[i] = *reinterpret_cast<const uint4*>(da + base + static_cast<int64_t>(i) * D);
-#pragma unroll
-    for (int j = 0; j < kMaxR; ++j) {
-      if (j < L) {
-        const uint4 ad = *reinterpret_cast<const uint4*>(e + base + static_cast<int64_t>(j) * D);
-        float a[8] = {bf16_lo_f(ad.x), bf16_hi_f(ad.x), bf16_lo_f(ad.y), bf16_hi_f(ad.y),
-                      bf16_lo_f(ad.z), bf16_hi_f(ad.z), bf16_lo_f(ad.w), bf16_hi_f(ad.w)};
-#pragma unroll
-        for (int i = 0; i < kMaxR; ++i) {
-          const bool on = (j < n) ? (i < n && i != j) : (i == j);
-          if (i < L && on) {
-            a[0] += bf16_lo_f(g[i].x); a[1] += bf16_hi_f(g[i].x);
-            a[2] += bf16_lo_f(g[i].y); a[3] += bf16_hi_f(g[i].y);
-            a[4] += bf16_lo_f(g[i].z); a[5] += bf16_hi_f(g[i].z);
-            a[6] += bf16_lo_f(g[i].w); a[7] += bf16_hi_f(g[i].w);
-          }
-        }
-        uint4 o;
-        const uint2 lo = pack4_bf16(a[0], a[1], a[2], a[3]), hi = pack4_bf16(a[4], a[5], a[6], a[7]);
-        o.x = lo.x; o.y = lo.y; o.z = hi.x; o.w = hi.y;
-        *reinterpret_cast<uint4*>(ada + base + static_cast<int64_t>(j) * D) = o;
+      if (i < L) g[i] = *reinterpret_cast<const uint4*>(x + (base + i) * ld + c);
+#pragma unroll
+    for (int i = 0; i < 8; ++i) a[i] = 0.f;
+#pragma unroll
+    for (int i = 0; i < kMaxR; ++i) {
+      if (i < n) {
+        a[0] += bf16_lo_f(g[i].x); a[1] += bf16_hi_f(g[i].x); a[2] += bf16_lo_f(g[i].y); a[3] += bf16_hi_f(g[i].y);
+        a[4] += bf16_lo_f(g[i].z); a[5] += bf16_hi_f(g[i].z); a[6] += bf16_lo_f(g[i].w); a[7] += bf16_hi_f(g[i].w);
+      }
+    }
+    put(u, c, a);
+#pragma unroll
+    for (int i = 0; i < kMaxR; ++i) {
+      if (i >= n && i < L) {
+        twice(g[i], a);
+        put(rm.srow[base + i], c, a);
       }
     }
   }
@@ -1367,7 +1412,7 @@
                      RowMap rm, int* bad, cudaStream_t s) {
   if (B <= 0) return SRG_OK;
   k_prep_rows<<<1, 1024, 0, s>>>(role_count, n_verbs, R, verb, B, compact, const_cast<int*>(rm.cnt),
-                                 const_cast<int*>(rm.off), const_cast<int*>(rm.meta), bad);
+                                 const_cast<int*>(rm.off), const_cast<int*>(rm.meta), const_cast<int*>(rm.srow), bad);
   SRG_LAUNCH_CHECK();
   return SRG_OK;
 }
@@ -1385,20 +1430,21 @@
 }
 
 int launch_aggregate_rows(const float* h32, RowMap rm, int B, int R, int D, bf16* a_hi, bf16* a_mid, bf16* a_lo,
-                          cudaStream_t s) {
+                          bf16* S, cudaStream_t s) {
   if (B <= 0) return SRG_OK;
   if (R > kMaxR) return set_error(SRG_ERR_UNSUPPORTED, "max_role_count %d > %d", R, kMaxR);
   k_aggregate_rows<<<grid_for(static_cast<int64_t>(B + kSelfRows) * D / 4), kThreads, 0, s>>>(h32, rm, B, R, D, a_hi,
-                                                                                            Parts{a_mid, a_lo});
-  SRG_LAUNCH_CHECK();
-  return SRG_OK;
-}
-
-int launch_aggregate_t_rows(const bf16* da, const bf16* e, RowMap rm, int B, int R, int D, bf16* ada, cudaStream_t s) {
+                                                                                            Parts{a_mid, a_lo}, S);
+  SRG_LAUNCH_CHECK();
+  return SRG_OK;
+}
+
+int launch_row_sums(const bf16* x, int64_t ld, RowMap rm, int B, int R, int cols, bf16* Sd, cudaStream_t s) {
   if (B <= 0) return SRG_OK;
   if (R > kMaxR) return set_error(SRG_ERR_UNSUPPORTED, "max_role_count %d > %d", R, kMaxR);
-  const int64_t units = (rm.cnt == nullptr) ? B : B + kSelfRows;
-  k_aggregate_t_rows<<<grid_for(units * D / 8), kThreads, 0, s>>>(da, e, rm, B, R, D, ada);
+  if (cols % 8 != 0 || ld % 8 != 0) return set_error(SRG_ERR_ARG, "row_sums: cols %d / ld %lld not multiples of 8", cols,
+                                                     (long long)ld);
+  k_row_sums<<<grid_for(static_cast<int64_t>(B + kSelfRows) * cols / 8), kThreads, 0, s>>>(x, ld, rm, B, R, cols, Sd);
   SRG_LAUNCH_CHECK();
   return SRG_OK;
 }
```
